# ZhaoyangLyu/Point_Diffusion_Refinement

Hardware: AMD Instinct MI355X
Metric: DDPM reverse steps/sec (T=1000, N=2048) (higher is better)
Workload: dtype f32; 1 GPU; BASELINE configs[1]: B=32/GPU, N=2048, 3072-pt mirrored condition, T=1000 DDPM reverse sampling, random-init dual-path PointNet++ (9.76 M params), cached condition step; global_batch=32, parallelism=dp1, launch=hipGraph replay, noise=device Philox, execution=fused channel-last HIP

## Files before the change

### include/pdr_hip.h

```cpp
#ifndef PDR_HIP_H
#define PDR_HIP_H

#include <stddef.h>
#include <stdint.h>

#ifdef __cplusplus
extern "C" {
#endif

#define PDR_OK 0
#define PDR_EINVAL (-1)
#define PDR_EUNSUPPORTED (-2)
#define PDR_ELAUNCH (-3)

typedef void *pdr_stream_t;

int pdr_version(void);
const char *pdr_last_error(void);
int pdr_set_option(const char *name, int value);
int pdr_get_option(const char *name, int *value);
const char *pdr_option_name(int index);

int pdr_opt_n_threads(int work_size);

// ... 142 lines not shown
int pdr_knn_build(const float *feats_y, int C, const float *x, const float *y,
                  const long long *idx, const float *d2, int B, int n1, int n2, int K,
                  float *out, int ldo, pdr_stream_t stream);
int pdr_attention_pool(const float *scores, int lds, const float *values, int ldv,
                       const float *vscale, const float *vshift, int v_relu, const int *counts,
                       int B, int npoint, int K, int D, float *out, pdr_stream_t stream);
int pdr_gather_add(const float *U, int ldu, int n_src, const float *V, const float *V0, int ldv,
                   const int *idx, const int *counts, const float *s1, const float *r1,
                   const float *s2, const float *r2, int B, int rows_per_batch, int K, int Cout,
                   float *Y, int ldy, float *partial, int relu_col0, int ycol0, int ycols,
                   pdr_stream_t stream);

int pdr_dedup_plan(const int *idx, const int *counts, int B, int m, int K, int *idx0, float *row_w,
                   unsigned char *tile_valid, int *tile_list, int *n_tiles, pdr_stream_t stream);
int pdr_dedup_prepare(const int *idx, const int *counts, const float *xyz, int B, int m, int K, int *perm, int *inv,
                      int *perm_rows, int *idx_s, int *counts_s, float *xyz_s, int *idx0, float *row_w,
                      unsigned char *tile_valid, int *tile_list, int *n_tiles, int *nvalid, int *probe_acc,
                      pdr_stream_t stream);
int pdr_dedup_probe(const int *counts, int B, int m, int K, int *probe_acc, pdr_stream_t stream);
int pdr_dedup_sort(const int *counts, int B, int m, int *perm, int *inv, int *perm_rows, pdr_stream_t stream);
int pdr_gather_add_tiles(const float *U, int ldu, int n_src, const float *V, const float *V0, int ldv,
                         const int *idx, const int *counts, const float *s1, const float *r1,
                         const float *s2, const float *r2, int B, int rows_per_batch, int K, int Cout,
                         float *Y, int ldy, float *partial, int relu_col0, int ycol0, int ycols,
                         const unsigned char *tile_valid, int partial_tpb, pdr_stream_t stream);
int pdr_gather_add_tiles_twin(const float *U, int ldu, int n_src, const float *V, const float *V0, int ldv,
                              const int *idx, const int *counts, int B, int rows_per_batch, int K, int Cout, float *Y,
                              int ldy, float *partial, int relu_col0, int ycol0, int ycols,
                              const unsigned char *tile_valid, int partial_tpb, const int *idx0, float *Yd, int ldyd,
                              const int *wrow0, float wmul, pdr_stream_t stream);
int pdr_weighted_moments(const float *Y, int ldy, int B, int rpb, int C, int relu_col0, const float *row_w,
                         float *partial, int ptpb, int tpb_full, const unsigned char *tile_valid,
                         pdr_stream_t stream);
int pdr_patch_rows(const float *V, int ldv, const float *vscale, const float *vshift, int v_relu,
                   const float *row_w, int B, int rpb, int D, float *out, int ldo, const int *out_rows,
                   pdr_stream_t stream);
int pdr_gather_rows(const float *src, const int *idx, int B, int n, int C, int m, float *out,
                    pdr_stream_t stream);


int pdr_reverse_update(float *x, const float *eps, int ld_eps, const float *z, const float *tab_a,
                       const float *tab_b, const float *tab_c, const long long *t_dev, long npoints,
                       int mode, pdr_stream_t stream);
int pdr_reverse_step(float *x, const float *eps, int ld_eps, const float *z, const float *tab_a,
                     const float *tab_b, const float *tab_c, long long *t_dev, const float *ts_table,
                     float *ts_out, unsigned long long *rng_state, int *ticket, long npoints, int mode,
                     int *probe_acc, int *probe_out, pdr_stream_t stream);
int pdr_embed_select(const float *table, int ldt, int T, const long long *t_dev, int B, int W, float *out, int ldo,
                     pdr_stream_t stream);
int pdr_embed_linear(const float *x, int ldx, const float *ts, int ts_stride, const float *freq, int half,
                     const float *W, const float *bias, int B, int K, int N, int act, float *out, int ldo,
                     pdr_stream_t stream);
typedef struct {
  const float *ptr;
  int C, ld;
} pdr_chain_seg_t;
typedef struct {
  const float *Wt;
  const float *bias;
  int ldw, Cin, Cout, main_cols;
  const float *gamma;
  const float *beta;
  int groups, Cn;
  float eps;
  int relu_pre, relu_post;
  const float *add;
  int add_ld;
  int reserved_;
} pdr_chain_layer_t;
typedef struct {
  int n_layers, n_seg;
  pdr_chain_seg_t seg[3];
  pdr_chain_layer_t layer[4];
  int residual, ldo;
  float *out;
  float *scratch;
  int *sync;
} pdr_point_chain_t;
int pdr_point_chain_plan(const pdr_point_chain_t *chain, int B, int n, long *out);
int pdr_point_chain(const pdr_point_chain_t *chain, int B, int n, pdr_stream_t stream);
int pdr_gather_rows2(const float *src0, int C0, const float *src1, int C1, const int *idx, int B, int n, int m,
                     float *out, pdr_stream_t stream);
int pdr_pad_rows(const float *src, long rows, int C, float *out, int ldo, pdr_stream_t stream);
int pdr_mark_time(unsigned long long *slot, pdr_stream_t stream);

#ifdef __cplusplus
}
#endif
#endif
```

### point_diffusion_refinement_amd/_lib.py

```python
import ctypes
import os

_HERE = os.path.dirname(os.path.abspath(__file__))
LIB_PATH = os.path.join(_HERE, "libpdr_hip.so")

PDR_OK, PDR_EINVAL, PDR_EUNSUPPORTED, PDR_ELAUNCH = 0, -1, -2, -3
_ERR = {PDR_EINVAL: "invalid argument", PDR_EUNSUPPORTED: "unsupported size", PDR_ELAUNCH: "kernel launch failed"}

_c = ctypes
_P, _I, _F, _Z = _c.c_void_p, _c.c_int, _c.c_float, _c.c_size_t

SIGNATURES = {
    "pdr_version": (_I, []),
    "pdr_last_error": (_c.c_char_p, []),
    "pdr_set_option": (_I, [_c.c_char_p, _I]),
    "pdr_get_option": (_I, [_c.c_char_p, _P]),
    "pdr_option_name": (_c.c_char_p, [_I]),
    "pdr_opt_n_threads": (_I, [_I]),
    "pdr_fps_workspace_bytes": (_Z, [_I, _I]),
    "pdr_furthest_point_sampling": (_I, [_P, _I, _I, _I, _P, _P, _P]),
    "pdr_gather_points": (_I, [_P, _P, _I, _I, _I, _I, _P, _P]),
    "pdr_gather_points_grad": (_I, [_P, _P, _I, _I, _I, _I, _P, _P]),
    "pdr_ball_query": (_I, [_P, _P, _I, _I, _I, _F, _I, _P, _P, _P]),
    "pdr_group_points": (_I, [_P, _P, _I, _I, _I, _I, _I, _P, _P]),
    "pdr_group_points_grad": (_I, [_P, _P, _I, _I, _I, _I, _I, _P, _P]),
    "pdr_three_nn": (_I, [_P, _P, _I, _I, _I, _P, _P, _P]),
    "pdr_three_interpolate": (_I, [_P, _P, _P, _I, _I, _I, _I, _P, _P]),
    "pdr_three_interpolate_grad": (_I, [_P, _P, _P, _I, _I, _I, _I, _P, _P]),
    "pdr_knn_points": (_I, [_P, _P, _I, _I, _I, _I, _P, _P, _P, _P]),
    "pdr_knn_points_ragged": (_I, [_P, _P, _P, _P, _I, _I, _I, _I, _P, _P, _P, _P]),
    "pdr_chamfer_nn": (_I, [_P, _P, _I, _I, _I, _P, _P, _P, _P, _P]),
    "pdr_chamfer_nn_ragged": (_I, [_P, _P, _P, _P, _I, _I, _I, _P, _P, _P, _P, _P]),
    "pdr_knn_group": (_I, [_P, _P, _I, _I, _I, _I, _P, _P, _P, _P]),
    "pdr_knn_points_grad": (_I, [_P, _P, _P, _P, _I, _I, _I, _I, _P, _P, _P]),
    "pdr_emd_workspace_bytes": (_Z, [_I, _I, _I]),
    "pdr_matchcost_workspace_bytes": (_Z, [_I, _I, _I]),
    "pdr_approxmatch": (_I, [_P, _P, _I, _I, _I, _P, _P, _P]),
    "pdr_matchcost": (_I, [_P, _P, _P, _I, _I, _I, _P, _P, _P]),
    "pdr_matchcost_grad": (_I, [_P, _P, _P, _P, _I, _I, _I, _P, _P, _P]),
    "pdr_emd_cost": (_I, [_P, _P, _I, _I, _I, _P, _P, _P]),
    "pdr_fused_layer_tile_rows": (_I, [_I, _I]),
    "pdr_fused_layer_variant": (_I, [_I, _I]),
    "pdr_fused_layer_plan": (_I, [_P, _c.c_long, _I, _P, _I, _I, _P, _I, _P]),
    "pdr_fused_layer": (_I, [_P, _c.c_long, _I, _P, _I, _P, _I, _P, _I, _P, _I, _P]),
    "pdr_fused_layer_pair": (_I, [_P, _c.c_long, _P, _c.c_long, _I, _P, _I, _P, _I, _P, _I, _P, _I, _P, _P, _I, _P]),
    "pdr_fused_layer_f16x3": (_I, [_P, _c.c_long, _I, _P, _I, _P, _I, _P, _I, _P, _I, _P]),
    "pdr_fused_layer_pool": (_I, [_P, _c.c_long, _I, _P, _I, _P, _I, _P, _I, _P, _P, _I, _P, _I, _P, _I, _P]),
    "pdr_fused_layer_pool_f16x3": (_I, [_P, _c.c_long, _I, _P, _I, _P, _I, _P, _I, _P, _P, _I, _P, _I, _P, _I, _P]),
    "pdr_gn_reduce": (_I, [_P, _I, _I, _I, _I, _c.c_double, _P, _I, _I, _P]),
    "pdr_apply_act": (_I, [_P, _c.c_long, _I, _P, _I, _P]),
    "pdr_act_colmax": (_I, [_P, _c.c_long, _I, _P, _P]),
    "pdr_gn_fold": (_I, [_P, _I, _I, _I, _c.c_double, _P, _I, _I, _I, _c.c_double, _I, _I, _I, _c.c_double, _F,
                         _P, _P, _P, _P, _P, _I, _P, _I, _P]),
    "pdr_gn_finalize": (_I, [_P, _I, _I, _I, _I, _c.c_double, _F, _P, _P, _P, _P, _P]),
    "pdr_group_build": (_I, [_P, _I, _P, _P, _P, _P, _I, _I, _I, _I, _I, _I, _I, _P, _I, _P]),
    "pdr_knn_build": (_I, [_P, _I, _P, _P, _P, _P, _I, _I, _I, _I, _P, _I, _P]),
    "pdr_attention_pool": (_I, [_P, _I, _P, _I, _P, _P, _I, _P, _I, _I, _I, _I, _P, _P]),
    "pdr_gather_rows": (_I, [_P, _P, _I, _I, _I, _I, _P, _P]),
    "pdr_reverse_update": (_I, [_P, _P, _I, _P, _P, _P, _P, _P, _c.c_long, _I, _P]),
    "pdr_reverse_step": (_I, [_P, _P, _I, _P, _P, _P, _P, _P, _P, _P, _P, _P, _c.c_long, _I, _P, _P, _P]),
    "pdr_embed_select": (_I, [_P, _I, _I, _P, _I, _I, _P, _I, _P]),
    "pdr_dedup_prepare": (_I, [_P, _P, _P, _I, _I, _I, _P, _P, _P, _P, _P, _P, _P, _P, _P, _P, _P, _P, _P, _P]),
    "pdr_dedup_probe": (_I, [_P, _I, _I, _I, _P, _P]),
    "pdr_gather_add_tiles_twin": (_I, [_P, _I, _I, _P, _P, _I, _P, _P, _I, _I, _I, _I, _P, _I, _P, _I, _I, _I, _P, _I,
                                       _P, _P, _I, _P, _F, _P]),
    "pdr_gather_rows2": (_I, [_P, _I, _P, _I, _P, _I, _I, _I, _P, _P]),
    "pdr_pad_rows": (_I, [_P, _c.c_long, _I, _P, _I, _P]),
    "pdr_mark_time": (_I, [_P, _P]),
    "pdr_embed_linear": (_I, [_P, _I, _P, _I, _P, _I, _P, _P, _I, _I, _I, _I, _P, _I, _P]),
    "pdr_gather_add": (_I, [_P, _I, _I, _P, _P, _I, _P, _P, _P, _P, _P, _P, _I, _I, _I, _I, _P, _I, _P, _I, _I, _I, _P]),
    "pdr_gather_add_tiles": (_I, [_P, _I, _I, _P, _P, _I, _P, _P, _P, _P, _P, _P, _I, _I, _I, _I, _P, _I, _P, _I, _I, _I,
                                  _P, _I, _P]),
    "pdr_dedup_plan": (_I, [_P, _P, _I, _I, _I, _P, _P, _P, _P, _P, _P]),
    "pdr_dedup_sort": (_I, [_P, _I, _I, _P, _P, _P, _P]),
    "pdr_weighted_moments": (_I, [_P, _I, _I, _I, _I, _I, _P, _P, _I, _I, _P, _P]),
    "pdr_patch_rows": (_I, [_P, _I, _P, _P, _I, _P, _I, _I, _I, _P, _I, _P, _P]),
    "pdr_point_chain_plan": (_I, [_P, _I, _I, _P]),
    "pdr_point_chain": (_I, [_P, _I, _I, _P]),
}


class Seg(_c.Structure):
    _fields_ = [("ptr", _P), ("C", _I), ("ld", _I), ("row_div", _I), ("gV", _P), ("gV0", _P), ("g_ldv", _I),
                ("g_nsrc", _I), ("g_zrow", _I), ("g_reserved", _I), ("g_r1", _P), ("g_r2", _P)]


class LayerIn(_c.Structure):
    _fields_ = [("n_seg", _I), ("seg", Seg * 4), ("scale", _P), ("shift", _P), ("add", _P), ("rseg", Seg),
                ("add_ld", _I), ("pre_relu", _I), ("post_relu", _I), ("rows_per_batch", _I), ("gidx", _P),
                ("gcnt", _P), ("gK", _I), ("ss_ld", _I), ("oadd", _P), ("oadd_ld", _I), ("oadd_div", _I), ("oadd_rows", _P),
                ("gs1", _P), ("gs2", _P), ("tile_list", _P), ("n_tiles", _P), ("out_rows", _P), ("partial_tpb", _I),
                ("wmul", _F), ("wrow0", _P), ("patch_values", _P), ("patch_w", _P), ("patch_ld", _I),
                ("walk_reverse", _I)]
class ChainSeg(_c.Structure):
    _fields_ = [("ptr", _P), ("C", _I), ("ld", _I)]


class ChainLayer(_c.Structure):
    _fields_ = [("Wt", _P), ("bias", _P), ("ldw", _I), ("Cin", _I), ("Cout", _I), ("main_cols", _I), ("gamma", _P),
                ("beta", _P), ("groups", _I), ("Cn", _I), ("eps", _F), ("relu_pre", _I), ("relu_post", _I), ("add", _P),
                ("add_ld", _I), ("reserved_", _I)]


class PointChain(_c.Structure):
    _fields_ = [("n_layers", _I), ("n_seg", _I), ("seg", ChainSeg * 3), ("layer", ChainLayer * 4), ("residual", _I),
                ("ldo", _I), ("out", _P), ("scratch", _P), ("sync", _P)]


_lib = None
ABI_VERSION = 200


def load():
    global _lib
    if _lib is None:
        if not os.path.exists(LIB_PATH):
            raise ImportError(
                "point_diffusion_refinement_amd: %s not found. Build it with "
                "`python -c 'import __graft_entry__ as g; g.build()'` or `make -C %s/csrc`. "
                "There is no CPU fallback." % (LIB_PATH, _HERE))
        lib = ctypes.CDLL(LIB_PATH)
        for name, (res, args) in SIGNATURES.items():
            fn = getattr(lib, name)
            fn.restype, fn.argtypes = res, args
        if lib.pdr_version() != ABI_VERSION:
            raise ImportError("point_diffusion_refinement_amd: %s is ABI %d, this binding needs %d -- rebuild it "
                              "(`make -C %s/csrc`)" % (LIB_PATH, lib.pdr_version(), ABI_VERSION, _HERE))
        _lib = lib
        _apply_env_options()
    return _lib


def set_option(name, value):
    check(load().pdr_set_option(name.encode(), int(value)), "set_option(%s=%r)" % (name, value))


def get_option(name):
    v = _c.c_int(0)
    check(load().pdr_get_option(name.encode(), _c.byref(v)), "get_option(%s)" % name)
    return v.value


def option_names():
    lib, out, i = load(), [], 0
    while True:
        n = lib.pdr_option_name(i)
        if n is None:
            return out
        out.append(n.decode())
        i += 1


def _apply_env_options():
    for item in filter(None, (t.strip() for t in os.environ.get("PDR_OPTIONS", "").split(","))):
        name, _, val = item.partition("=")
        set_option(name.strip(), int(val))
    for name in option_names():
        val = os.environ.get("PDR_" + name.upper())
        if val is not None and val.strip().lstrip("-").isdigit():
            set_option(name, int(val))


def check(rc, what):
    if rc != PDR_OK:
        detail = ""
        if rc == PDR_ELAUNCH:
            detail = ": " + (load().pdr_last_error() or b"").decode()
        raise RuntimeError("%s failed: %s%s" % (what, _ERR.get(rc, "code %d" % rc), detail))
```

### point_diffusion_refinement_amd/csrc/ball_query.hip

```cpp
#include "pdr_common.h"

namespace {

template <int NCH, bool RESIDENT>
__global__ __launch_bounds__(256) void ball_query_kernel(
    const float* __restrict__ new_xyz, const float* __restrict__ xyz, int n, int m,
    float radius2, int nsample, int qpw, int* __restrict__ idx,
    int* __restrict__ counts) {
  const int b = blockIdx.y;
  const int lane = threadIdx.x & 63;
  const int wave = __builtin_amdgcn_readfirstlane(threadIdx.x >> 6);
  const float* p = xyz + static_cast<size_t>(b) * n * 3;
  const float* q = new_xyz + static_cast<size_t>(b) * m * 3;
  int* oi = idx + static_cast<size_t>(b) * m * nsample;
  int* oc = counts + static_cast<size_t>(b) * m;

  const int nch = RESIDENT ? NCH : (n + 63) / 64;
  float px[NCH], py[NCH], pz[NCH];
  if constexpr (RESIDENT) {
    if constexpr (NCH <= 32) {
#pragma unroll
      for (int c = 0; c < NCH; ++c) {
        const int k = min(c * 64 + lane, n - 1);
        px[c] = p[k * 3 + 0];
        py[c] = p[k * 3 + 1];
        pz[c] = p[k * 3 + 2];
      }
#pragma unroll
      for (int c = 0; c < NCH; ++c) {
        const bool ok = c * 64 + lane < n;
        px[c] = ok ? px[c] : __builtin_inff();
        py[c] = ok ? py[c] : __builtin_inff();
        pz[c] = ok ? pz[c] : __builtin_inff();
      }
    } else {
#pragma unroll
      for (int c = 0; c < NCH; ++c) {
        const int k = c * 64 + lane;
        const bool ok = k < n;
        px[c] = ok ? p[k * 3 + 0] : __builtin_inff();
        py[c] = ok ? p[k * 3 + 1] : __builtin_inff();
        pz[c] = ok ? p[k * 3 + 2] : __builtin_inff();
      }
    }
    __builtin_amdgcn_s_waitcnt(0x0F70);
  }

  const int j0 = (blockIdx.x * 4 + wave) * qpw;
  const int jf = min(j0, m - 1);
  float nqx = q[jf * 3 + 0], nqy = q[jf * 3 + 1], nqz = q[jf * 3 + 2];
  for (int jj = 0; jj < qpw; ++jj) {
    const int j = j0 + jj;
    if (j >= m) break;
    const float qx = nqx, qy = nqy, qz = nqz;
    {
      const int jn = min(j + 1, m - 1);
      nqx = q[jn * 3 + 0], nqy = q[jn * 3 + 1], nqz = q[jn * 3 + 2];
    }
    int* row = oi + static_cast<size_t>(j) * nsample;
    int cnt = 0;
    int first = 0;
    auto scan = [&](int c, float x, float y, float z) {
      const float dx = qx - x, dy = qy - y, dz = qz - z;
      const float d2 = PDR_SUM3(dx, dy, dz);
      const bool hit = d2 < radius2;
      const unsigned long long mask = __ballot(hit);
      if (mask != 0ull) {
        if (cnt == 0) first = c * 64 + __builtin_ctzll(mask);
        const int pos = cnt + __builtin_amdgcn_mbcnt_hi(
                                  static_cast<unsigned>(mask >> 32),
                                  __builtin_amdgcn_mbcnt_lo(static_cast<unsigned>(mask), 0u));
        if (hit && pos < nsample) row[pos] = c * 64 + lane;
        cnt += __builtin_popcountll(mask);
      }
    };
    if constexpr (RESIDENT) {
#pragma unroll
      for (int c = 0; c < NCH; ++c) {
        if (cnt < nsample) scan(c, px[c], py[c], pz[c]);
      }
    } else {
      for (int c = 0; c < nch && cnt < nsample; ++c) {
        const int k = c * 64 + lane;
        const bool ok = k < n;
        const int kc = ok ? k : n - 1;
        const float x = p[kc * 3 + 0], y = p[kc * 3 + 1], z = p[kc * 3 + 2];
        scan(c, ok ? x : __builtin_inff(), ok ? y : __builtin_inff(), ok ? z : __builtin_inff());
      }
    }
    const int filled = cnt < nsample ? cnt : nsample;
    for (int l = filled + lane; l < nsample; l += 64) row[l] = first;
    if (lane == 0) oc[j] = filled;
  }
}

template <int NCH, bool RESIDENT>
int launch(const float* new_xyz, const float* xyz, int B, int n, int m, float radius2,
           int nsample, int* idx, int* counts, hipStream_t s) {
  int qpw = 16;
  while (qpw > 1 && static_cast<long long>(B) * ((m + 4 * qpw - 1) / (4 * qpw)) < 1024) qpw >>= 1;
  dim3 grid((m + 4 * qpw - 1) / (4 * qpw), B);
  hipLaunchKernelGGL((ball_query_kernel<NCH, RESIDENT>), grid, dim3(256), 0, s, new_xyz, xyz, n,
                     m, radius2, nsample, qpw, idx, counts);
  return pdr::check_launch();
}

}

extern "C" int pdr_ball_query(const float* new_xyz, const float* xyz, int B, int n, int m,
                              float radius, int nsample, int* idx, int* counts,
                              pdr_stream_t stream) {
  if (B < 0 || n <= 0 || m < 0 || nsample <= 0) return PDR_EINVAL;
  if (B == 0 || m == 0) return PDR_OK;
  if (!new_xyz || !xyz || !idx || !counts) return PDR_EINVAL;
  hipStream_t s = pdr::as_stream(stream);
  const float radius2 = radius * radius;
#define PDR_BQ_CASE(NCH) \
  if (n <= 64 * (NCH))   \
  return launch<NCH, true>(new_xyz, xyz, B, n, m, radius2, nsample, idx, counts, s)
  PDR_BQ_CASE(1);
  PDR_BQ_CASE(2);
  PDR_BQ_CASE(4);
  PDR_BQ_CASE(8);
  PDR_BQ_CASE(16);
  PDR_BQ_CASE(32);
  PDR_BQ_CASE(48);
  PDR_BQ_CASE(64);
#undef PDR_BQ_CASE
  return launch<1, false>(new_xyz, xyz, B, n, m, radius2, nsample, idx, counts, s);
}
```

### point_diffusion_refinement_amd/csrc/dedup.hip

```cpp
#include "pdr_common.h"

__global__ __launch_bounds__(256) void dedup_flags_kernel(const int* __restrict__ idx, const int* __restrict__ counts,
                                                          int K, long nq, int qpt, int* __restrict__ idx0,
                                                          float* __restrict__ row_w,
                                                          unsigned char* __restrict__ tile_valid) {
  const long q = static_cast<long>(blockIdx.x) * 256 + threadIdx.x;
  if (q >= nq) return;
  const int cnt = counts[q];
  idx0[q] = idx[q * K];
  int v = cnt > 1 ? 1 : 0;
  for (int off = 1; off < qpt; off <<= 1) v |= __shfl_xor(v, off, 64);
  const bool valid = v != 0;
  row_w[q] = valid ? 0.0f : static_cast<float>(K);
  if ((q & (qpt - 1)) == 0) tile_valid[q / qpt] = valid ? 1 : 0;
}

__global__ __launch_bounds__(1024) void dedup_compact_kernel(const unsigned char* __restrict__ tile_valid, int ntiles,
                                                            int* __restrict__ tile_list, int* __restrict__ n_tiles) {
  __shared__ int wtot[16];
  __shared__ int base_s;
  const int tid = threadIdx.x, lane = tid & 63, wave = tid >> 6;
  if (tid == 0) base_s = 0;
  __syncthreads();
  for (int i0 = 0; i0 < ntiles; i0 += 1024) {
// ... 2 lines not shown
    const unsigned long long bal = __ballot(valid);
    const int before = __builtin_popcountll(bal & ((1ull << lane) - 1ull));
    if (lane == 0) wtot[wave] = __builtin_popcountll(bal);
    __syncthreads();
    int woff = 0, tot = 0;
    for (int w = 0; w < 16; ++w) {
      woff += w < wave ? wtot[w] : 0;
      tot += wtot[w];
    }
    const int base = base_s;
    if (valid) tile_list[base + woff + before] = i;
    __syncthreads();
    if (tid == 0) base_s = base + tot;
    __syncthreads();
  }
  if (tid == 0) *n_tiles = base_s;
}

__global__ __launch_bounds__(1024) void dedup_sort_kernel(const int* __restrict__ counts, int m,
                                                         int* __restrict__ perm, int* __restrict__ inv,
                                                         int* __restrict__ perm_rows) {
  __shared__ int wtot[16];
  __shared__ int base_s;
  const int tid = threadIdx.x, lane = tid & 63, wave = tid >> 6;
  const int* cb = counts + static_cast<long>(blockIdx.x) * m;
  int* pb = perm + static_cast<long>(blockIdx.x) * m;
  int* ib = inv + static_cast<long>(blockIdx.x) * m;
  if (tid == 0) base_s = 0;
  __syncthreads();
  for (int pass = 0; pass < 2; ++pass) {
    for (int i0 = 0; i0 < m; i0 += 1024) {
      const int i = i0 + tid;
      const bool take = i < m && ((cb[i] > 1) == (pass == 0));
      const unsigned long long bal = __ballot(take);
      const int before = __builtin_popcountll(bal & ((1ull << lane) - 1ull));
      if (lane == 0) wtot[wave] = __builtin_popcountll(bal);
      __syncthreads();
      int woff = 0, tot = 0;
      for (int w = 0; w < 16; ++w) {
        woff += w < wave ? wtot[w] : 0;
        tot += wtot[w];
      }
      const int base = base_s;
      if (take) {
        const int j = base + woff + before;
        pb[j] = i;
        ib[i] = j;
        if (perm_rows) perm_rows[static_cast<long>(blockIdx.x) * m + j] = static_cast<int>(blockIdx.x) * m + i;
      }
      __syncthreads();
      if (tid == 0) base_s = base + tot;
      __syncthreads();
    }
  }
}

extern "C" int pdr_dedup_sort(const int* counts, int B, int m, int* perm, int* inv, int* perm_rows,
                              pdr_stream_t stream) {
  if (!counts || !perm || !inv || B < 0 || m <= 0 || static_cast<long>(B) * m >= (1L << 31)) return PDR_EINVAL;
  if (B == 0) return PDR_OK;
  hipLaunchKernelGGL(dedup_sort_kernel, dim3(B), dim3(1024), 0, pdr::as_stream(stream), counts, m, perm, inv, perm_rows);
  return pdr::check_launch();
}

extern "C" int pdr_dedup_plan(const int* idx, const int* counts, int B, int m, int K, int* idx0, float* row_w,
                              unsigned char* tile_valid, int* tile_list, int* n_tiles, pdr_stream_t stream) {
  if (!idx || !counts || !idx0 || !row_w || !tile_valid || !tile_list || !n_tiles || B < 0 || m <= 0) return PDR_EINVAL;
  if (!(K == 8 || K == 16 || K == 32) || (static_cast<long>(m) * K) % 128 != 0) return PDR_EINVAL;
  if (B == 0) return PDR_OK;
  const int qpt = 128 / K;
  const long ntiles = static_cast<long>(B) * m / qpt;
  if (ntiles >= (1L << 30)) return PDR_EINVAL;
  const long nq = static_cast<long>(B) * m;
  hipLaunchKernelGGL(dedup_flags_kernel, dim3(pdr::blocks_for(nq)), dim3(256), 0, pdr::as_stream(stream), idx, counts, K,
                     nq, qpt, idx0, row_w, tile_valid);
  hipLaunchKernelGGL(dedup_compact_kernel, dim3(1), dim3(1024), 0, pdr::as_stream(stream), tile_valid,
                     static_cast<int>(ntiles), tile_list, n_tiles);
  return pdr::check_launch();
}

constexpr int kMaxPrepareClouds = 1024;
constexpr int kMaxPrepareQueries = 4096;

__global__ __launch_bounds__(1024) void dedup_prepare_kernel(
    const int* __restrict__ idx, const int* __restrict__ counts, const float* __restrict__ xyz, int m, int K, int nB,
    int* __restrict__ perm, int* __restrict__ inv, int* __restrict__ perm_rows, int* __restrict__ idx_s,
    int* __restrict__ counts_s, float* __restrict__ xyz_s, int* __restrict__ idx0, float* __restrict__ row_w,
    unsigned char* __restrict__ tile_valid, int* __restrict__ tile_list, int* __restrict__ n_tiles,
    int* __restrict__ nvalid, int* __restrict__ probe_acc) {
  __shared__ int nreal_s[kMaxPrepareClouds];
  __shared__ int perm_s[kMaxPrepareQueries];
  __shared__ int wtot[16];
  __shared__ int base_s, prefix_s;
  const int tid = threadIdx.x, lane = tid & 63, wave = tid >> 6;
  const int b = blockIdx.x;
  const int qpt = 128 / K, tpb = m / qpt;
  if (tid == 0) base_s = 0;
  const bool vec = (m & 3) == 0 && (reinterpret_cast<uintptr_t>(counts) & 15) == 0;
  for (int bb = wave; bb <= b; bb += 16) {
    const int* cb = counts + static_cast<long>(bb) * m;
    int c = 0;
    if (vec) {
      const int4* c4 = reinterpret_cast<const int4*>(cb);
      const int n4 = m >> 2;
      for (int i0 = 0; i0 < n4; i0 += 64 * 8) {
        int4 v[8];
#pragma unroll
        for (int u = 0; u < 8; ++u) {
          const int i = i0 + 64 * u + lane;
          v[u] = c4[i < n4 ? i : 0];
        }
#pragma unroll
        for (int u = 0; u < 8; ++u) {
          const bool ok = i0 + 64 * u + lane < n4;
          c += ok ? (v[u].x > 1) + (v[u].y > 1) + (v[u].z > 1) + (v[u].w > 1) : 0;
        }
      }
    } else {
      for (int i = lane; i < m; i += 64) c += cb[i] > 1 ? 1 : 0;
    }
#pragma unroll
    for (int off = 32; off >= 1; off >>= 1) c += __shfl_xor(c, off, 64);
    if (lane == 0) nreal_s[bb] = c;
  }
  __syncthreads();
  if (tid == 0) {
    int p = 0;
    for (int bb = 0; bb < b; ++bb) p += (nreal_s[bb] + qpt - 1) / qpt;
    prefix_s = p;
  }
  const int nv = (nreal_s[b] + qpt - 1) / qpt;
  const int q0 = nv * qpt;
  const int* cb = counts + static_cast<long>(b) * m;
  int* pb = perm + static_cast<long>(b) * m;
  int* ib = inv + static_cast<long>(b) * m;
  for (int pass = 0; pass < 2; ++pass) {
    for (int i0 = 0; i0 < m; i0 += 1024) {
      const int i = i0 + tid;
      const bool take = i < m && ((cb[i] > 1) == (pass == 0));
      const unsigned long long bal = __ballot(take);
      const int before = __builtin_popcountll(bal & ((1ull << lane) - 1ull));
      if (lane == 0) wtot[wave] = __builtin_popcountll(bal);
      __syncthreads();
      int woff = 0, tot = 0;
      for (int w = 0; w < 16; ++w) {
        woff += w < wave ? wtot[w] : 0;
        tot += wtot[w];
      }
      const int base = base_s;
      if (take) {
        const int j = base + woff + before;
        perm_s[j] = i;
        pb[j] = i;
        ib[i] = j;
        if (perm_rows) perm_rows[static_cast<long>(b) * m + j] = b * m + i;
      }
      __syncthreads();
      if (tid == 0) base_s = base + tot;
      __syncthreads();
    }
  }
  for (int j = tid; j < m; j += 1024) {
    const int src = perm_s[j];
    const long qs = static_cast<long>(b) * m + src, qd = static_cast<long>(b) * m + j;
    counts_s[qd] = cb[src];
    idx0[qd] = idx[qs * K];
    row_w[qd] = j >= q0 ? static_cast<float>(K) : 0.0f;
    if (xyz) {
      const float x = xyz[qs * 3 + 0], y = xyz[qs * 3 + 1], z = xyz[qs * 3 + 2];
      xyz_s[qd * 3 + 0] = x;
      xyz_s[qd * 3 + 1] = y;
      xyz_s[qd * 3 + 2] = z;
    }
  }
  const int k4 = K / 4, ksh4 = __builtin_ctz(k4);
  const int npiece = m * k4;
  const int4* src4 = reinterpret_cast<const int4*>(idx + static_cast<long>(b) * m * K);
  int4* dst4 = reinterpret_cast<int4*>(idx_s + static_cast<long>(b) * m * K);
  for (int e0 = 0; e0 < npiece; e0 += 4096) {
    int4 v[4];
#pragma unroll
    for (int u = 0; u < 4; ++u) {
      const int e = min(e0 + 1024 * u + tid, npiece - 1);
      v[u] = src4[(perm_s[e >> ksh4] << ksh4) + (e & (k4 - 1))];
    }
#pragma unroll
    for (int u = 0; u < 4; ++u) {
      const int e = e0 + 1024 * u + tid;
      if (e < npiece) dst4[e] = v[u];
    }
  }
  const int prefix = prefix_s;
  for (int t = tid; t < tpb; t += 1024) {
    tile_valid[static_cast<long>(b) * tpb + t] = t < nv ? 1 : 0;
    if (t < nv) tile_list[prefix + t] = b * tpb + t;
  }
  if (tid == 0) {
    nvalid[b] = nv;
    nvalid[nB + b] = q0;
    if (b == nB - 1) *n_tiles = prefix + nv;
    if (probe_acc) {
      atomicAdd(&probe_acc[0], nv);
      atomicAdd(&probe_acc[1], tpb);
    }
  }
}

__global__ __launch_bounds__(256) void dedup_probe_kernel(const int* __restrict__ counts, int m, int K,
                                                          int* __restrict__ probe_acc) {
  __shared__ int tot;
  if (threadIdx.x == 0) tot = 0;
  __syncthreads();
  const int* cb = counts + static_cast<long>(blockIdx.x) * m;
  int c = 0;
  for (int i = threadIdx.x; i < m; i += 256) c += cb[i] > 1 ? 1 : 0;
#pragma unroll
  for (int off = 32; off >= 1; off >>= 1) c += __shfl_xor(c, off, 64);
  if ((threadIdx.x & 63) == 0 && c) atomicAdd(&tot, c);
  __syncthreads();
  if (threadIdx.x == 0) {
    const int qpt = 128 / K;
    atomicAdd(&probe_acc[0], (tot + qpt - 1) / qpt);
    atomicAdd(&probe_acc[1], m / qpt);
  }
}

extern "C" int pdr_dedup_prepare(const int* idx, const int* counts, const float* xyz, int B, int m, int K, int* perm,
                                 int* inv, int* perm_rows, int* idx_s, int* counts_s, float* xyz_s, int* idx0,
                                 float* row_w, unsigned char* tile_valid, int* tile_list, int* n_tiles, int* nvalid,
                                 int* probe_acc, pdr_stream_t stream) {
  if (!idx || !counts || !perm || !inv || !idx_s || !counts_s || (xyz && !xyz_s) || !idx0 || !row_w || !tile_valid ||
      !tile_list || !n_tiles || !nvalid || B < 0 || m <= 0)
    return PDR_EINVAL;
  if (!(K == 8 || K == 16 || K == 32) || (static_cast<long>(m) * K) % 128 != 0) return PDR_EINVAL;
  if (static_cast<long>(B) * m * K >= (1L << 31)) return PDR_EINVAL;
  if (B > kMaxPrepareClouds || m > kMaxPrepareQueries) return PDR_EUNSUPPORTED;
  if ((reinterpret_cast<uintptr_t>(idx) | reinterpret_cast<uintptr_t>(idx_s)) % 16 != 0) return PDR_EINVAL;
  if (B == 0) return PDR_OK;
  hipLaunchKernelGGL(dedup_prepare_kernel, dim3(B), dim3(1024), 0, pdr::as_stream(stream), idx, counts, xyz, m, K, B,
                     perm, inv, perm_rows, idx_s, counts_s, xyz_s, idx0, row_w, tile_valid, tile_list, n_tiles, nvalid,
                     probe_acc);
  return pdr::check_launch();
}

extern "C" int pdr_dedup_probe(const int* counts, int B, int m, int K, int* probe_acc, pdr_stream_t stream) {
  if (!counts || !probe_acc || B < 0 || m <= 0) return PDR_EINVAL;
  if (!(K == 8 || K == 16 || K == 32) || (static_cast<long>(m) * K) % 128 != 0) return PDR_EINVAL;
  if (B == 0) return PDR_OK;
  hipLaunchKernelGGL(dedup_probe_kernel, dim3(B), dim3(256), 0, pdr::as_stream(stream), counts, m, K, probe_acc);
  return pdr::check_launch();
}

__global__ __launch_bounds__(256) void weighted_moments_kernel(const float* __restrict__ Y, int ldy, int C, int rpb,
                                                               int tpbd, int nB, int relu_col0,
                                                               const float* __restrict__ row_w,
                                                               float* __restrict__ partial, int ptpb, int tpb_full,
                                                               const unsigned char* __restrict__ tile_valid) {
  const int nmom = nB * tpbd;
  const int cl = threadIdx.x & 63, sl = threadIdx.x >> 6;
  const int c = blockIdx.y * 64 + cl;
  if (static_cast<int>(blockIdx.x) >= nmom) {
    const int t0 = (static_cast<int>(blockIdx.x) - nmom) * 16;
    for (int k = sl; k < 16; k += 4) {
      const int t = t0 + k;
      if (t < nB * tpb_full && !tile_valid[t] && c < C) {
        const int b = t / tpb_full, tb = t - b * tpb_full;
        float* o = partial + ((static_cast<long>(b) * ptpb + tb) * C + c) * 2;
        o[0] = 0.0f;
        o[1] = 0.0f;
      }
    }
    return;
  }
  __shared__ float red[4][64][2];
  const int b = blockIdx.x / tpbd, j = blockIdx.x - b * tpbd;
  const int r0 = j * 128 + sl * 32, r1 = min(r0 + 32, rpb);
  float s1 = 0.0f, s2 = 0.0f;
  if (c < C) {
    const float lo = c >= relu_col0 ? 0.0f : -__builtin_inff();
    const float* yp = Y + (static_cast<long>(b) * rpb) * ldy + c;
    const float* wp = row_w + static_cast<long>(b) * rpb;
    float w[32];
    bool any = false;
#pragma unroll
    for (int k = 0; k < 32; ++k) {
      w[k] = r0 + k < r1 ? wp[min(r0 + k, rpb - 1)] : 0.0f;
      any = any || w[k] > 0.0f;
    }
    if (any) {
#pragma unroll
      for (int k0 = 0; k0 < 32; k0 += 16) {
        float y[16];
#pragma unroll
        for (int k = 0; k < 16; ++k) y[k] = yp[static_cast<long>(min(r0 + k0 + k, rpb - 1)) * ldy];
#pragma unroll
        for (int k = 0; k < 16; ++k) {
          const float f = fmaxf(y[k], lo);
          s1 = __builtin_fmaf(w[k0 + k], f, s1);
          s2 = __builtin_fmaf(w[k0 + k] * f, f, s2);
        }
      }
    }
  }
  red[sl][cl][0] = s1;
  red[sl][cl][1] = s2;
  __syncthreads();
  if (sl == 0 && c < C) {
    float* o = partial + ((static_cast<long>(b) * ptpb + tpb_full + j) * C + c) * 2;
    o[0] = (red[0][cl][0] + red[1][cl][0]) + (red[2][cl][0] + red[3][cl][0]);
    o[1] = (red[0][cl][1] + red[1][cl][1]) + (red[2][cl][1] + red[3][cl][1]);
  }
}

extern "C" int pdr_weighted_moments(const float* Y, int ldy, int B, int rpb, int C, int relu_col0, const float* row_w,
                                    float* partial, int ptpb, int tpb_full, const unsigned char* tile_valid,
                                    pdr_stream_t stream) {
  if (!Y || !row_w || !partial || !tile_valid || B < 0 || rpb <= 0 || C <= 0 || ldy < C || tpb_full <= 0) return PDR_EINVAL;
  const int tpbd = (rpb + 127) / 128;
  if (ptpb < tpb_full + tpbd) return PDR_EINVAL;
  if (B == 0) return PDR_OK;
  const long nz = (static_cast<long>(B) * tpb_full + 15) / 16;
  const dim3 grid(static_cast<unsigned>(static_cast<long>(B) * tpbd + nz), static_cast<unsigned>((C + 63) / 64));
  hipLaunchKernelGGL(weighted_moments_kernel, grid, dim3(256), 0, pdr::as_stream(stream), Y, ldy, C, rpb, tpbd, B,
                     relu_col0, row_w, partial, ptpb, tpb_full, tile_valid);
// ... 34 lines not shown
```

### point_diffusion_refinement_amd/csrc/fused_gather.hip

```cpp
#include "pdr_common.h"

namespace {

template <int LPP>
__global__ __launch_bounds__(256) void group_build_kernel(
    const float* __restrict__ feats, int Cs, int n, const float* __restrict__ xyz,
    const float* __restrict__ new_xyz, const int* __restrict__ idx, const int* __restrict__ counts,
    int m, int K, int patch_empty, int with_abs, int with_centre, long npos, int Cout, int ldo,
    float* __restrict__ out) {
  constexpr int GPB = 256 / LPP;
  const int lane = threadIdx.x % LPP;
  const long g0 = static_cast<long>(blockIdx.x) * GPB + threadIdx.x / LPP;
  const long ngroups = static_cast<long>(gridDim.x) * GPB;
  for (long p = g0; p < npos; p += ngroups) {
    const long bj = p / K;
    const int b = static_cast<int>(bj / m);
    const int a = idx[p];
    const bool empty = patch_empty && counts[bj] <= 0;
    const float* frow = feats + (static_cast<long>(b) * n + a) * Cs;
    float* orow = out + p * ldo;
    for (int c = lane; c < Cs; c += LPP) orow[c] = empty ? 0.0f : frow[c];
    if (lane < ldo - Cout) orow[Cout + lane] = 0.0f;
    if (lane < Cout - Cs) {
      const int g = lane;
// ... 113 lines not shown
    int cnt = K;
    if (counts) {
      cnt = counts[row];
      cnt = cnt < 1 ? 1 : cnt;
    }
    const float4* s4 = reinterpret_cast<const float4*>(scores + row * K * D) + lane;
    const float4* v4 = reinterpret_cast<const float4*>(values + row * K * D) + lane;
    float4 sv[NL], vv[NL];
#pragma unroll
    for (int i = 0; i < NL; ++i) {
      const bool ok = k0 + i * kstep < K;
      sv[i] = ok ? s4[i * 64] : make_float4(0, 0, 0, 0);
      vv[i] = ok ? v4[i * 64] : make_float4(0, 0, 0, 0);
    }
    float4 sc = make_float4(1, 1, 1, 1), shv = make_float4(0, 0, 0, 0);
    if (vscale) sc = *reinterpret_cast<const float4*>(vscale + static_cast<long>(b) * D + 4 * c4);
    if (vshift) shv = *reinterpret_cast<const float4*>(vshift + static_cast<long>(b) * D + 4 * c4);
    float m[4] = {-__builtin_inff(), -__builtin_inff(), -__builtin_inff(), -__builtin_inff()};
    float se[NL][4];
#pragma unroll
    for (int i = 0; i < NL; ++i) {
      const int k = k0 + i * kstep;
      const float e[4] = {sv[i].x, sv[i].y, sv[i].z, sv[i].w};
#pragma unroll
      for (int j = 0; j < 4; ++j) {
        se[i][j] = k >= K ? -__builtin_inff() : (k >= cnt ? -1e9f : e[j]) * 1.44269504088896340736f;
        m[j] = fmaxf(m[j], se[i][j]);
      }
    }
#pragma unroll
    for (int j = 0; j < 4; ++j)
      for (int off = D4; off < 64; off <<= 1) m[j] = fmaxf(m[j], __shfl_xor(m[j], off, 64));
    float l[4] = {0, 0, 0, 0}, acc[4] = {0, 0, 0, 0};
    const float sce[4] = {sc.x, sc.y, sc.z, sc.w}, she[4] = {shv.x, shv.y, shv.z, shv.w};
#pragma unroll
    for (int i = 0; i < NL; ++i) {
      const float ve[4] = {vv[i].x, vv[i].y, vv[i].z, vv[i].w};
#pragma unroll
      for (int j = 0; j < 4; ++j) {
        const float w = __builtin_amdgcn_exp2f(se[i][j] - m[j]);
        const float val = fmaxf(__builtin_fmaf(ve[j], sce[j], she[j]), lo);
        l[j] += w;
        acc[j] = __builtin_fmaf(val, w, acc[j]);
      }
    }
#pragma unroll
    for (int j = 0; j < 4; ++j)
      for (int off = D4; off < 64; off <<= 1) {
        l[j] += __shfl_xor(l[j], off, 64);
        acc[j] += __shfl_xor(acc[j], off, 64);
      }
    if (lane < D4)
      *reinterpret_cast<float4*>(out + row * D + 4 * c4) =
          make_float4(acc[0] / l[0], acc[1] / l[1], acc[2] / l[2], acc[3] / l[3]);
  }
}

__global__ __launch_bounds__(256) void gather_rows_cl_kernel(const float* __restrict__ src, int n,
                                                             int C, const int* __restrict__ idx,
                                                             int m, long total,
                                                             float* __restrict__ out) {
  const long e = static_cast<long>(blockIdx.x) * 256 + threadIdx.x;
  if (e >= total) return;
  const long bj = e / C;
  const int c = static_cast<int>(e - bj * C);
  const int b = static_cast<int>(bj / m);
  out[e] = src[(static_cast<long>(b) * n + idx[bj]) * C + c];
}

__global__ __launch_bounds__(256) void gather_rows2_cl_kernel(const float* __restrict__ src0, int C0,
                                                              const float* __restrict__ src1, int C1, int n,
                                                              const int* __restrict__ idx, int m, long total,
                                                              float* __restrict__ out) {
  const long e = static_cast<long>(blockIdx.x) * 256 + threadIdx.x;
  if (e >= total) return;
  const int C = C0 + C1;
  const long bj = e / C;
  const int c = static_cast<int>(e - bj * C);
  const int b = static_cast<int>(bj / m);
  const long row = static_cast<long>(b) * n + idx[bj];
  out[e] = c < C0 ? src0[row * C0 + c] : src1[row * C1 + (c - C0)];
}

__global__ __launch_bounds__(256) void pad_rows_kernel(const float* __restrict__ src, int C, int ldo, long total,
                                                       float* __restrict__ out) {
  const long e = static_cast<long>(blockIdx.x) * 256 + threadIdx.x;
  if (e >= total) return;
  const long r = e / ldo;
  const int c = static_cast<int>(e - r * ldo);
  out[e] = c < C ? src[r * C + c] : 0.0f;
}

}

extern "C" int pdr_group_build(const float* feats, int Cs, const float* xyz, const float* new_xyz,
                               const int* idx, const int* counts, int B, int n, int m, int K,
                               int patch_empty, int with_abs, int with_centre, float* out, int ldo,
                               pdr_stream_t stream) {
  if (B < 0 || n <= 0 || m < 0 || K <= 0 || Cs < 0) return PDR_EINVAL;
  if (B == 0 || m == 0) return PDR_OK;
  if (!xyz || !new_xyz || !idx || !out || (Cs > 0 && !feats) || (patch_empty && !counts))
    return PDR_EINVAL;
  const int Cout = Cs + 3 + (with_abs ? 3 : 0) + (with_centre ? 3 : 0);
  if (ldo < Cout || ldo - Cout > 8) return PDR_EINVAL;
  const long npos = static_cast<long>(B) * m * K;
  hipStream_t s = pdr::as_stream(stream);
#define PDR_GB(LPP)                                                                                 \
  do {                                                                                              \
    const long nblk = (npos + 256 / LPP - 1) / (256 / LPP);                                         \
    hipLaunchKernelGGL(group_build_kernel<LPP>, dim3(static_cast<unsigned>(nblk < 32768 ? nblk : 32768)), \
                       dim3(256), 0, s, feats, Cs, n, xyz, new_xyz, idx, counts, m, K, patch_empty, \
                       with_abs, with_centre, npos, Cout, ldo, out);                                \
  } while (0)
  if (Cout <= 16) PDR_GB(16);
  else if (Cout <= 48) PDR_GB(32);
  else PDR_GB(64);
#undef PDR_GB
  return pdr::check_launch();
}

extern "C" int pdr_knn_build(const float* feats_y, int C, const float* x, const float* y,
                             const long long* idx, const float* d2, int B, int n1, int n2, int K,
                             float* out, int ldo, pdr_stream_t stream) {
  if (B < 0 || n1 < 0 || n2 <= 0 || K <= 0 || C < 0) return PDR_EINVAL;
  if (B == 0 || n1 == 0) return PDR_OK;
  if (!x || !y || !idx || !d2 || !out || (C > 0 && !feats_y)) return PDR_EINVAL;
  const int Cout = C + 11;
  if (ldo < Cout || ldo - Cout > 8) return PDR_EINVAL;
  const long npos = static_cast<long>(B) * n1 * K;
  hipStream_t s = pdr::as_stream(stream);
#define PDR_KB(LPP)                                                                                 \
  do {                                                                                              \
    const long nblk = (npos + 256 / LPP - 1) / (256 / LPP);                                         \
    hipLaunchKernelGGL(knn_build_kernel<LPP>, dim3(static_cast<unsigned>(nblk < 32768 ? nblk : 32768)), \
                       dim3(256), 0, s, feats_y, C, n2, x, y, idx, d2, n1, K, npos, Cout, ldo, out); \
  } while (0)
  if (Cout <= 16) PDR_KB(16);
  else if (Cout <= 48) PDR_KB(32);
  else PDR_KB(64);
#undef PDR_KB
  return pdr::check_launch();
}

extern "C" int pdr_attention_pool(const float* scores, int lds, const float* values, int ldv,
                                  const float* vscale, const float* vshift, int v_relu,
                                  const int* counts, int B, int npoint, int K, int D, float* out,
                                  pdr_stream_t stream) {
  if (B < 0 || npoint < 0 || K <= 0 || D <= 0) return PDR_EINVAL;
  if (B == 0 || npoint == 0) return PDR_OK;
  if (!scores || !values || !out) return PDR_EINVAL;
  const long rows = static_cast<long>(B) * npoint;
  if (D % 4 || lds % 4 || ldv % 4) return PDR_EUNSUPPORTED;
  {
    const int D4 = D / 4;
    const long per_query = static_cast<long>(K) * D4;
    const int kstep = D4 <= 64 ? 64 / (D4 ? D4 : 1) : 0;
    if (lds == D && ldv == D && D4 <= 64 && (D4 & (D4 - 1)) == 0 && per_query <= 512 && kstep > 0) {
      const int nl = static_cast<int>((K + kstep - 1) / kstep);
      long blocks = (rows + 3) / 4;
      if (blocks > 256L * 16) blocks = 256L * 16;
      const dim3 grid(static_cast<unsigned>(blocks));
      hipStream_t st = pdr::as_stream(stream);
#define PDR_AP(NL)                                                                                      \
  hipLaunchKernelGGL(attention_pool_wave_kernel<NL>, grid, dim3(256), 0, st, scores, values, vscale,    \
                     vshift, v_relu, counts, K, D, npoint, rows, out)
      if (nl <= 1) PDR_AP(1);
      else if (nl <= 2) PDR_AP(2);
      else if (nl <= 4) PDR_AP(4);
      else PDR_AP(8);
#undef PDR_AP
      return pdr::check_launch();
    }
  }
  hipLaunchKernelGGL(attention_pool_kernel, dim3(pdr::blocks_for(rows * (D / 4))), dim3(256), 0,
                     pdr::as_stream(stream), scores, lds, values, ldv, vscale, vshift, v_relu, counts, K,
                     D, npoint, rows, out);
  return pdr::check_launch();
}

extern "C" int pdr_gather_rows2(const float* src0, int C0, const float* src1, int C1, const int* idx, int B, int n,
                                int m, float* out, pdr_stream_t stream) {
  if (B < 0 || n <= 0 || C0 <= 0 || C1 <= 0 || m < 0) return PDR_EINVAL;
  if (B == 0 || m == 0) return PDR_OK;
  if (!src0 || !src1 || !idx || !out) return PDR_EINVAL;
  const long total = static_cast<long>(B) * m * (C0 + C1);
  hipLaunchKernelGGL(gather_rows2_cl_kernel, dim3(pdr::blocks_for(total)), dim3(256), 0, pdr::as_stream(stream), src0,
                     C0, src1, C1, n, idx, m, total, out);
  return pdr::check_launch();
}

extern "C" int pdr_pad_rows(const float* src, long rows, int C, float* out, int ldo, pdr_stream_t stream) {
  if (rows < 0 || C <= 0 || ldo < C) return PDR_EINVAL;
  if (rows == 0) return PDR_OK;
  if (!src || !out) return PDR_EINVAL;
  const long total = rows * ldo;
  hipLaunchKernelGGL(pad_rows_kernel, dim3(pdr::blocks_for(total)), dim3(256), 0, pdr::as_stream(stream), src, C, ldo,
                     total, out);
  return pdr::check_launch();
}

extern "C" int pdr_gather_rows(const float* src, const int* idx, int B, int n, int C, int m,
                               float* out, pdr_stream_t stream) {
  if (B < 0 || n <= 0 || C <= 0 || m < 0) return PDR_EINVAL;
  if (B == 0 || m == 0) return PDR_OK;
  if (!src || !idx || !out) return PDR_EINVAL;
  const long total = static_cast<long>(B) * m * C;
  hipLaunchKernelGGL(gather_rows_cl_kernel, dim3(pdr::blocks_for(total)), dim3(256), 0,
                     pdr::as_stream(stream), src, n, C, idx, m, total, out);
  return pdr::check_launch();
}

template <int LPR, bool KPOW2, bool HAS_S>
__global__ __launch_bounds__(256) void gather_add_kernel(
    const float* __restrict__ U, int ldu, int n_src, const float* __restrict__ V,
    const float* __restrict__ V0, int ldv, const int* __restrict__ idx, const int* __restrict__ counts,
    const float* __restrict__ s1, const float* __restrict__ r1, const float* __restrict__ s2,
    const float* __restrict__ r2, int rows_per_batch_, int K_, int Cout, float* __restrict__ Y_, int ldy_,
    float* __restrict__ partial, int relu_col0, int ycol0_, int ycol1_,
    const unsigned char* __restrict__ tile_valid, int partial_tpb, pdr::GatherTwin tw) {
  constexpr int TM = 128;
  const bool twin = static_cast<int>(blockIdx.x) >= tw.n_main && tw.n_main > 0;
  const int rows_per_batch = twin ? rows_per_batch_ / K_ : rows_per_batch_;
  const int K = twin ? 1 : K_;
  const int* __restrict__ idx_e = twin ? tw.idx0 : idx;
  float* __restrict__ Y = twin ? tw.Y : Y_;
  const int ldy = twin ? tw.ldy : ldy_;
  const int ycol0 = twin ? 0 : ycol0_, ycol1 = twin ? ((Cout + 3) & ~3) : ycol1_;
  constexpr int RPI = 64 / LPR;
  constexpr int DEPTH = 32 / RPI < 4 ? 32 / RPI : 4;
  constexpr int CW = 4 * LPR;
  __shared__ float red[4][CW][2];
  const int lane = threadIdx.x & 63, wave = threadIdx.x >> 6;
  const int sub = lane / LPR, cl = lane % LPR;
  const int tpb = (rows_per_batch + TM - 1) / TM;
  const int n_main = tw.n_main > 0 ? tw.n_main : static_cast<int>(gridDim.x);
  const int bid = twin ? static_cast<int>(blockIdx.x) - n_main : pdr::xcd_contiguous(blockIdx.x, n_main);
  const int b = bid / tpb, tb = bid - b * tpb;
  if (!twin && tile_valid && !tile_valid[bid]) return;
  const int tpb_main = (rows_per_batch_ + TM - 1) / TM;
  const long prow = static_cast<long>(b) * (partial_tpb > 0 ? partial_tpb : tpb) + (twin ? tpb_main : 0) + tb;
  const long row0 = static_cast<long>(b) * rows_per_batch + static_cast<long>(tb) * TM;
  const int nvalid = min(TM, rows_per_batch - tb * TM);
  const int wlo = twin ? min(max(tw.wrow0[b] - tb * TM, 0), TM) : 0;
  const float wmul = twin ? tw.wmul : 1.0f;
  const float* Ub = U + static_cast<long>(b) * n_src * ldu;
  const int wr0 = wave * 32;
  const int myr = min(wr0 + (lane & 31), nvalid - 1);
  const long myp = row0 + myr;
  const int my_idx = idx_e[myp];
  const int my_empty = (counts && counts[myp / K] <= 0) ? 1 : 0;
  const float my_s1 = s1 ? s1[myp] : 0.0f;
  const float my_s2 = s2 ? s2[myp] : 0.0f;
  const int nrows = max(0, min(32, nvalid - wr0));

  constexpr bool has_s = HAS_S;
  const bool has_em = counts != nullptr;
  const int ksh = KPOW2 ? __builtin_ctz(K) : -1;
  const long qbase = (row0 + wr0) / K;
  const float* Vq = V + qbase * ldv;
  const long v0d = has_em ? V0 - V : 0;
  for (int c0 = static_cast<int>(blockIdx.y) * CW; c0 < Cout; c0 += CW * static_cast<int>(gridDim.y)) {
    const int c = c0 + 4 * cl;
    const bool cok = c < Cout;
    const int cc = cok ? c : 0;
    float4 q1 = make_float4(0, 0, 0, 0), q2 = make_float4(0, 0, 0, 0);
    if (cok && r1) q1 = *reinterpret_cast<const float4*>(r1 + c);
    if (cok && r2) q2 = *reinterpret_cast<const float4*>(r2 + c);
    float lo[4];
#pragma unroll
    for (int j = 0; j < 4; ++j) lo[j] = (c + j >= relu_col0) ? 0.0f : -__builtin_inff();
    const bool ywin = Y && c >= ycol0 && c < ycol1;
    float a1[4] = {0, 0, 0, 0}, a2[4] = {0, 0, 0, 0};
    for (int r = 0; r < nrows; r += DEPTH * RPI) {
      float4 u[DEPTH], v[DEPTH];
      float t1[DEPTH], t2[DEPTH];
      int em[DEPTH], rr[DEPTH];
#pragma unroll
      for (int k = 0; k < DEPTH; ++k) {
        rr[k] = r + k * RPI + sub;
        const int rc = min(rr[k], nrows - 1);
// ... 162 lines not shown
```

### point_diffusion_refinement_amd/csrc/fused_layer.hip

```cpp
#include "layer_tiles.h"

#include <cstdlib>

namespace {

typedef float f32x16 __attribute__((ext_vector_type(16)));

using pdr::PoolArgs;

template <int RT, int CT, int WR, int WC, int KC, bool RADD, bool VEC, bool GATH, bool POOL = false, int KS = 1>
__global__ __launch_bounds__(256, 2) void fused_layer_kernel(
    pdr_layer_in_t in, int Cin, const float* __restrict__ Wt, int ldw,
    const float* __restrict__ bias, int Cout, float* __restrict__ Y, int ldy,
    float* __restrict__ partial, int relu_col0, int n_row_tiles, PoolArgs pool = PoolArgs()) {
  static_assert(WR * WC * KS == 4, "4 waves per workgroup");
  static_assert(KS == 1 || !POOL, "pooled epilogue: no K split");
  constexpr int TM = WR * RT * 32, TN = WC * CT * 32;
  constexpr int APT = TM * KC / 256;
  constexpr int RSTEP = 256 / KC;
  constexpr int C4 = KC / 4;
  constexpr int VSTEP = 256 / C4;
  constexpr int APT4 = TM / VSTEP;
  constexpr int TN4 = TN / 4;
  constexpr int WPT4 = (KC * TN4 + 255) / 256;
// ... 339 lines not shown
      const int col = n0 + cl;
      const bool colok = col < Cout;
      const float bv = bias_r[j];
      const bool relu_stat = col >= relu_col0;
      float s1 = 0.0f, s2 = 0.0f;
      float* ybase = Y + row0 * ldy + col;
      if (colok && in.oadd) {
        const int osh = __builtin_ctz(in.oadd_div);
        const float* ob = in.oadd + col;
#pragma unroll
        for (int i = 0; i < RT; ++i) {
#pragma unroll
          for (int r = 0; r < 16; ++r) {
            const int rl = min((wr * RT + i) * 32 + (r & 3) + 8 * (r >> 2) + 4 * hi, nvalid - 1);
            const long oq = (row0 + rl) >> osh;
            acc[i][j][r] += ob[(in.oadd_rows ? static_cast<long>(in.oadd_rows[oq]) : oq) * in.oadd_ld];
          }
        }
      }
      if (colok) {
        if (rows_full) {
#pragma unroll
          for (int i = 0; i < RT; ++i) {
#pragma unroll
            for (int r = 0; r < 16; ++r) {
              const int rl = (wr * RT + i) * 32 + (r & 3) + 8 * (r >> 2) + 4 * hi;
              const float y = acc[i][j][r] + bv;
              ybase[rl * ldy] = y;
              const float f = relu_stat ? fmaxf(y, 0.0f) : y;
              s1 += f;
              s2 = __builtin_fmaf(f, f, s2);
            }
          }
        } else {
#pragma unroll
          for (int i = 0; i < RT; ++i) {
#pragma unroll
            for (int r = 0; r < 16; ++r) {
              const int rl = (wr * RT + i) * 32 + (r & 3) + 8 * (r >> 2) + 4 * hi;
              const float y = acc[i][j][r] + bv;
              if (rl < nvalid) {
                ybase[rl * ldy] = y;
                if (rl >= wlo) {
                  const float f = relu_stat ? fmaxf(y, 0.0f) : y;
                  s1 += f;
                  s2 = __builtin_fmaf(f, f, s2);
                }
              }
            }
          }
        }
      }
      if (partial) {
        s1 += __shfl_xor(s1, 32, 64);
        s2 += __shfl_xor(s2, 32, 64);
        if (in.wrow0) {
          s1 *= in.wmul;
          s2 *= in.wmul;
        }
        if (hi == 0) {
          red[wr][cl][0] = s1;
          red[wr][cl][1] = s2;
        }
      }
    }
    if (partial) {
      __syncthreads();
      if (tid < TN && n0 + tid < Cout) {
        float s1 = 0.0f, s2 = 0.0f;
#pragma unroll
        for (int w = 0; w < WR; ++w) {
          s1 += red[w][tid][0];
          s2 += red[w][tid][1];
        }
        const long prow = static_cast<long>(b) * (in.partial_tpb > 0 ? in.partial_tpb : tpb) + tb;
        float* o = partial + (prow * Cout + n0 + tid) * 2;
        o[0] = s1;
        o[1] = s2;
      }
    }
  }
}

__global__ __launch_bounds__(256) void fused_layer_thin_kernel(const float* __restrict__ X, int ldx, int shift,
                                                               int Cin, const float* __restrict__ Wt, int ldw,
                                                               const float* __restrict__ bias, int Cout,
                                                               float* __restrict__ Y, int ldy, long P, int qshift) {
  constexpr int kThinIters = 8;
  const int ql = 1 << qshift;
  const int cq = threadIdx.x & (ql - 1), rl = threadIdx.x >> qshift;
  const int c0 = 4 * (static_cast<int>(blockIdx.y) * ql + cq);
  if (c0 >= Cout) return;
  const int rpp = 256 >> qshift;
  float4 w[4];
  float b4[4];
#pragma unroll
  for (int k = 0; k < 4; ++k)
    w[k] = k < Cin ? *reinterpret_cast<const float4*>(Wt + static_cast<long>(k) * ldw + c0) : make_float4(0, 0, 0, 0);
#pragma unroll
  for (int j = 0; j < 4; ++j) b4[j] = (bias && c0 + j < Cout) ? bias[c0 + j] : 0.0f;
  const long r0 = static_cast<long>(blockIdx.x) * (rpp * kThinIters) + rl;
  float4 xr[kThinIters];
#pragma unroll
  for (int it = 0; it < kThinIters; ++it) {
    const long row = r0 + static_cast<long>(it) * rpp;
    xr[it] = *reinterpret_cast<const float4*>(X + ((row < P ? row : P - 1) >> shift) * ldx);
  }
#pragma unroll
  for (int it = 0; it < kThinIters; ++it) {
    const long row = r0 + static_cast<long>(it) * rpp;
    if (row < P) {
      const float4 x = xr[it];
      const float xs[4] = {x.x, x.y, x.z, x.w};
      float acc[4] = {b4[0], b4[1], b4[2], b4[3]};
#pragma unroll
      for (int o = 0; o < 4; ++o) {
        const int k = ((o & 1) << 1) | (o >> 1);
        if (k < Cin) {
          acc[0] = __builtin_fmaf(xs[k], w[k].x, acc[0]);
          acc[1] = __builtin_fmaf(xs[k], w[k].y, acc[1]);
          acc[2] = __builtin_fmaf(xs[k], w[k].z, acc[2]);
          acc[3] = __builtin_fmaf(xs[k], w[k].w, acc[3]);
        }
      }
      *reinterpret_cast<float4*>(Y + row * ldy + c0) = make_float4(acc[0], acc[1], acc[2], acc[3]);
    }
  }
}

using pdr::LayerSource;
using pdr::Tile;

inline bool narrow_kc32() { return pdr::option(pdr::OPT_NARROW_KC32) != 0; }
inline int pick_tile(int rows_per_batch, int Cout) {
  if (narrow_kc32() && rows_per_batch >= 128 && Cout <= 32) return 7;
  if (narrow_kc32() && rows_per_batch >= 128 && Cout <= 64) return 8;
  if (rows_per_batch >= 256 && Cout <= 32) return 0;
  if (rows_per_batch >= 256 && Cout <= 64) return 1;
  if (rows_per_batch >= 128 && Cout <= 96) return 2;
  if (rows_per_batch >= 128 && Cout > 128 && Cout <= 160) return 3;
  if (rows_per_batch >= 128) return 4;
  if (rows_per_batch >= 64) return 5;
  return 6;
}
}

extern "C" int pdr_fused_layer_tile_rows(int rows_per_batch, int Cout) {
  if (rows_per_batch <= 0 || Cout <= 0) return 0;
  return pdr::tile_tm(pick_tile(rows_per_batch, Cout));
}

extern "C" int pdr_fused_layer_variant(int rows_per_batch, int Cout) {
  if (rows_per_batch <= 0 || Cout <= 0) return -1;
  return pick_tile(rows_per_batch, Cout);
}

namespace {
enum class Family {
  Thin,
  DeepSplitK,
  Deep,
  Ws,
  Uniform
};

struct LayerPlan {
  Family family;
  int id, tm;
  LayerSource src;
  bool vec;
  bool ws;
  bool thin;
  long ntiles;
  int ncol;
  int deep;
  int deep_tn;
};

bool deep_chunks() { return pdr::option(pdr::OPT_DEEP_CHUNKS) != 0; }

bool use_ws_kernels() { return pdr::option(pdr::OPT_FUSED_WS) != 0; }

int plan_layer(const pdr_layer_in_t* in, long P, int Cin, const float* Wt, int ldw, int Cout, const float* Y,
               int ldy, bool has_partial, LayerPlan* pl) {
  if (!in || !Wt || P < 0 || Cin <= 0 || Cout <= 0 || in->n_seg < 1 || in->n_seg > 4 || ldw < Cout ||
      (Y && ldy < Cout))
    return PDR_EINVAL;
  if (ldw % 4 != 0 || reinterpret_cast<uintptr_t>(Wt) % 16 != 0) return PDR_EINVAL;
  int ctot = 0;
  for (int s = 0; s < in->n_seg; ++s) {
    if (!in->seg[s].ptr || in->seg[s].C <= 0 || in->seg[s].row_div < 1) return PDR_EINVAL;
    if (in->seg[s].row_div & (in->seg[s].row_div - 1)) return PDR_EUNSUPPORTED;
    ctot += in->seg[s].C;
  }
  if (ctot != Cin || in->rows_per_batch <= 0 || P % in->rows_per_batch != 0) return PDR_EINVAL;
  if (in->oadd && (in->oadd_div < 1 || (in->oadd_div & (in->oadd_div - 1)) || in->oadd_ld < Cout))
    return PDR_EINVAL;
  if (in->ss_ld != 0 && in->ss_ld < Cin) return PDR_EINVAL;
  const int id = pick_tile(in->rows_per_batch, Cout), tm = pdr::tile_tm(id);
  for (int sg = 0; sg < in->n_seg; ++sg) {
    const int d = in->seg[sg].row_div;
    if (in->rows_per_batch % d != 0 || (in->rows_per_batch > tm && tm % d != 0)) return PDR_EUNSUPPORTED;
  }
  const long nb = P / in->rows_per_batch;
  if (in->partial_tpb > 0 && in->partial_tpb < (in->rows_per_batch + tm - 1) / tm) return PDR_EINVAL;
  pl->id = id;
  pl->tm = tm;
  pl->ntiles = nb * ((in->rows_per_batch + tm - 1) / tm);
  pl->ncol = (Cout + pdr::tile_tn(id) - 1) / pdr::tile_tn(id);
  const LayerSource src = pdr::layer_source(*in);
// ... 38 lines not shown
             !in->pre_relu && !in->post_relu && !in->oadd && Y && ldy % 4 == 0 &&
             reinterpret_cast<uintptr_t>(Y) % 16 == 0 && ldw >= ((Cout + 3) & ~3) && ldy >= ((Cout + 3) & ~3) &&
             P < (1L << 31);
  if (src.knn_marked && !pl->ws) return PDR_EUNSUPPORTED;
  if (in->tile_list && (!in->n_tiles || !pl->ws || tm != 128)) return PDR_EUNSUPPORTED;
  pl->family = pl->thin && !has_partial && !in->tile_list ? Family::Thin
               : split_k                                   ? Family::DeepSplitK
               : pl->deep                                  ? Family::Deep
               : pl->ws                                    ? Family::Ws
                                                           : Family::Uniform;
  return PDR_OK;
}

struct LayerArgs {
  hipStream_t s; const pdr_layer_in_t& in; int Cin; const float* Wt; int ldw; const float* bias; int Cout;
  float* Y; int ldy; float* partial; int relu_col0, n_row_tiles; PoolArgs pool;
};

template <class T, bool RADD, bool VEC, bool GATH, bool POOL = false, int KS = 1>
void launch_k(dim3 grid, const LayerArgs& a) {
  hipLaunchKernelGGL((fused_layer_kernel<T::RT, T::CT, T::WR, T::WC, T::KC, RADD, VEC, GATH, POOL, KS>), grid,
                     dim3(256), 0, a.s, a.in, a.Cin, a.Wt, a.ldw, a.bias, a.Cout, a.Y, a.ldy, a.partial, a.relu_col0,
                     a.n_row_tiles, a.pool);
}

template <class T>
void launch_form(dim3 grid, const LayerArgs& a, const LayerPlan& pl) {
  if (pl.src.radd) {
    if (pl.src.gath) launch_k<T, true, true, true>(grid, a);
    else if (pl.vec) launch_k<T, true, true, false>(grid, a);
    else launch_k<T, true, false, false>(grid, a);
  } else {
    if (pl.src.gath) launch_k<T, false, true, true>(grid, a);
    else if (pl.vec) launch_k<T, false, true, false>(grid, a);
    else launch_k<T, false, false, false>(grid, a);
  }
}

template <class T, int KS = 1>
void launch_plain(dim3 grid, const LayerArgs& a, bool radd) {
  if (radd) launch_k<T, true, true, false, false, KS>(grid, a);
  else launch_k<T, false, true, false, false, KS>(grid, a);
}

dim3 uniform_grid(long ntiles, int ncol) {
  const long cap = (256L * 6 + ncol - 1) / ncol;
  return dim3(static_cast<unsigned>(ntiles > cap ? cap : ntiles), static_cast<unsigned>(ncol));
}
}

extern "C" int pdr_fused_layer_plan(const pdr_layer_in_t* in, long P, int Cin, const float* Wt, int ldw, int Cout,
                                    const float* Y, int ldy, int* out) {
  if (!out) return PDR_EINVAL;
  LayerPlan pl;
  const int rc = plan_layer(in, P, Cin, Wt, ldw, Cout, Y, ldy, true, &pl);
  if (rc != PDR_OK) return rc;
  out[0] = pl.family == Family::Ws;
  out[1] = pl.id;
  out[2] = pl.src.radd;
  out[3] = pl.src.gath ? (pl.src.knn_marked ? 2 : 1) : 0;
  out[4] = pl.vec;
  out[5] = 0;
  out[6] = pl.thin;
  out[7] = pl.deep ? 128 : 0;
  return PDR_OK;
}

extern "C" int pdr_fused_layer(const pdr_layer_in_t* in, long P, int Cin, const float* Wt, int ldw,
                               const float* bias, int Cout, float* Y, int ldy, float* partial,
                               int relu_col0, pdr_stream_t stream) {
  if (!Y) return PDR_EINVAL;
  LayerPlan pl;
  const int prc = plan_layer(in, P, Cin, Wt, ldw, Cout, Y, ldy, partial != nullptr, &pl);
  if (prc != PDR_OK) return prc;
  if (P == 0) return PDR_OK;
  hipStream_t s = pdr::as_stream(stream);
  const int nt = static_cast<int>(pl.ntiles);
  const LayerArgs a{s, *in, Cin, Wt, ldw, bias, Cout, Y, ldy, partial, relu_col0, nt, PoolArgs()};
  auto deep_grid = [&] {
    return dim3(static_cast<unsigned>(pl.ntiles), static_cast<unsigned>((Cout + pl.deep_tn - 1) / pl.deep_tn));
  };
  switch (pl.family) {
    case Family::Thin: {
      const int c4n = (Cout + 3) / 4;
      int qshift = 3;
      while (qshift < 6 && (1 << qshift) < c4n) ++qshift;
      const int ql = 1 << qshift, rows_per_block = (256 >> qshift) * 8;
      const dim3 tgrid(static_cast<unsigned>((P + rows_per_block - 1) / rows_per_block),
                       static_cast<unsigned>((c4n + ql - 1) / ql));
      hipLaunchKernelGGL(fused_layer_thin_kernel, tgrid, dim3(256), 0, s, in->seg[0].ptr, in->seg[0].ld,
                         __builtin_ctz(in->seg[0].row_div), Cin, Wt, ldw, bias, Cout, Y, ldy, P, qshift);
      break;
    }
    case Family::DeepSplitK:
      if (pl.deep == 6) launch_plain<Tile<1, 1, 1, 1, 128>, 4>(deep_grid(), a, pl.src.radd);
      else launch_plain<Tile<1, 1, 2, 1, 128>, 2>(deep_grid(), a, pl.src.radd);
      break;
    case Family::Deep:
      if (pl.deep == 6) launch_form<Tile<1, 1, 1, 4, 128>>(uniform_grid(pl.ntiles, pl.ncol), a, pl);
      else if (pl.deep == 5) launch_plain<Tile<1, 1, 2, 2, 128>>(deep_grid(), a, pl.src.radd);
      else launch_plain<Tile<2, 1, 2, 2, 128>>(deep_grid(), a, pl.src.radd);
      break;
    case Family::Ws:
      pdr::launch_fused_layer_ws(pl.id, pl.src, *in, Cin, Wt, ldw, bias, Cout, Y, ldy, partial, relu_col0, nt, pl.ncol,
                                 s);
      break;
    case Family::Uniform:
      pdr::with_tile(pl.id, [&](auto t) { launch_form<decltype(t)>(uniform_grid(pl.ntiles, pl.ncol), a, pl); });
      break;
  }
  return pdr::check_launch();
}

extern "C" int pdr_fused_layer_pair(const pdr_layer_in_t* in, long P, const pdr_layer_in_t* in2, long P2, int Cin,
                                    const float* Wt, int ldw, const float* bias, int Cout, float* Y, int ldy,
                                    float* Y2, int ldy2, float* partial, float* partial2, int relu_col0,
                                    pdr_stream_t stream) {
  if (!Y || !Y2 || !in || !in2) return PDR_EINVAL;
  LayerPlan pl, pl2;
  int rc = plan_layer(in, P, Cin, Wt, ldw, Cout, Y, ldy, partial != nullptr, &pl);
  if (rc != PDR_OK) return rc;
  rc = plan_layer(in2, P2, Cin, Wt, ldw, Cout, Y2, ldy2, partial2 != nullptr, &pl2);
  if (rc != PDR_OK) return rc;
  if (P == 0 || P2 == 0) return PDR_EUNSUPPORTED;
  if ((partial == nullptr) != (partial2 == nullptr)) return PDR_EINVAL;
  if (!in->tile_list || !pl.ws || !pdr::tile_has_pair(pl.id) || !pl.vec || !pl2.vec || pl.src.radd || pl2.src.radd ||
      pl2.src.gath || pl.src.knn_marked || in2->tile_list)
    return PDR_EUNSUPPORTED;
  const int tpb2 = (in2->rows_per_batch + pl.tm - 1) / pl.tm;
  if (in2->partial_tpb > 0 && in2->partial_tpb < tpb2) return PDR_EINVAL;
  for (int sg = 0; sg < in2->n_seg; ++sg)
    if (in2->seg[sg].row_div != 1) return PDR_EUNSUPPORTED;
  if (in2->gidx || !pdr::fused_layer_ws_supported(pl.id, pl2.src, *in2, Cin)) return PDR_EUNSUPPORTED;
  pdr::WsTwin tw;
  tw.in[1] = *in2;
  tw.Y[1] = Y2;
  tw.partial[1] = partial2;
  tw.ldy[1] = ldy2;
  tw.n_row_tiles[1] = static_cast<int>((P2 / in2->rows_per_batch) * tpb2);
  tw.gx = 0;
  pdr::launch_fused_layer_ws_pair(pl.id, pl.src.gath, *in, Cin, Wt, ldw, bias, Cout, Y, ldy, partial, relu_col0,
                                  static_cast<int>(pl.ntiles), pl.ncol, tw, pdr::as_stream(stream));
  return pdr::check_launch();
}

extern "C" int pdr_fused_layer_f16x3(const pdr_layer_in_t* in, long P, int Cin, const void* Wp, int nchunks,
                                     const float* bias, int Cout, float* Y, int ldy, float* partial,
                                     int relu_col0, pdr_stream_t stream) {
  if (!Y || !Wp || nchunks <= 0 || reinterpret_cast<uintptr_t>(Wp) % 16 != 0) return PDR_EINVAL;
  LayerPlan pl;
  const int prc = plan_layer(in, P, Cin, reinterpret_cast<const float*>(Wp), (Cout + 3) & ~3, Cout, Y, ldy,
                             partial != nullptr, &pl);
  if (prc != PDR_OK) return prc;
  if (P == 0) return PDR_OK;
  if (!pl.ws || !pdr::tile_has_split(pl.id)) return PDR_EUNSUPPORTED;
  int nch = 0;
  for (int s = 0; s < in->n_seg; ++s) nch += (in->seg[s].C + 31) / 32;
  if (nch != nchunks) return PDR_EINVAL;
  pdr::launch_fused_layer_ws(pl.id, pl.src, *in, Cin, reinterpret_cast<const float*>(Wp), nchunks, bias, Cout, Y, ldy,
                             partial, relu_col0, static_cast<int>(pl.ntiles), pl.ncol, pdr::as_stream(stream), true);
  return pdr::check_launch();
}

namespace {
bool pool_patch_args_ok(const pdr_layer_in_t& in, int D, const float* out, int ldo) {
  if (!in.patch_values) return true;
  return in.patch_w != nullptr && in.patch_ld >= D && D % 4 == 0 && in.patch_ld % 4 == 0 && ldo % 4 == 0 &&
         reinterpret_cast<uintptr_t>(in.patch_values) % 16 == 0 && reinterpret_cast<uintptr_t>(out) % 16 == 0;
}

struct PoolPlan {
  int id, tm, ncol, nch;
  long ntiles;
  bool vec;
};
int plan_pool(const pdr_layer_in_t* in, long P, int Cin, bool weights_ok, int D, const float* values, int ldv, int K,
              const float* out, int ldo, PoolPlan* pp) {
  if (!in || !weights_ok || !values || !out || P <= 0 || Cin <= 0 || D <= 0 || in->n_seg < 1 || in->n_seg > 4 ||
      ldv < D || ldo < D)
    return PDR_EINVAL;
  if (!pool_patch_args_ok(*in, D, out, ldo)) return PDR_EINVAL;
  if (!(K == 8 || K == 16 || K == 32)) return PDR_EUNSUPPORTED;
  if (in->rseg.ptr || in->oadd) return PDR_EUNSUPPORTED;
  int ctot = 0;
  pp->nch = 0;
  pp->vec = true;
  for (int s = 0; s < in->n_seg; ++s) {
    const pdr_seg_t& g = in->seg[s];
    if (!g.ptr || g.C <= 0 || g.row_div != 1 || g.gV) return PDR_EUNSUPPORTED;
    pp->vec = pp->vec && reinterpret_cast<uintptr_t>(g.ptr) % 16 == 0 && g.ld % 4 == 0 && g.ld >= ((g.C + 3) & ~3);
    ctot += g.C;
    pp->nch += (g.C + 31) / 32;
  }
// ... 56 lines not shown
```

### point_diffusion_refinement_amd/csrc/neighbors.hip

```cpp
#include <cstdlib>

#include "pdr_common.h"

namespace {

constexpr int kTile = 1024;

enum DistModel { kSum3 = 0, kAcc3 = 1 };

__device__ __forceinline__ int cloud_len(const int64_t* __restrict__ len, int b, int n) {
  if (!len) return n;
  const int64_t v = len[b];
  return v < 0 ? 0 : (v > n ? n : static_cast<int>(v));
}

template <int K, int MODEL, typename IdxT, bool KNN_PAD, bool RAGGED = false>
__global__ __launch_bounds__(256) void nn_search_kernel(const float* __restrict__ queries,
                                                        const float* __restrict__ cloud, int nq,
                                                        int nc, int Kout,
                                                        float* __restrict__ dists,
                                                        IdxT* __restrict__ idx,
                                                        float* __restrict__ nn,
                                                        float* __restrict__ wgt = nullptr,
                                                        const int64_t* __restrict__ len_q = nullptr,
                                                        const int64_t* __restrict__ len_c = nullptr) {
  static_assert(KNN_PAD || !RAGGED, "the ragged search pads with (0, -1)");
  __shared__ float4 tile[kTile];
  const int b = blockIdx.y;
  const int j = blockIdx.x * 256 + threadIdx.x;
  const bool active = j < nq;
  const int nqe = RAGGED ? cloud_len(len_q, b, nq) : nq;
  const int nce = !RAGGED ? nc : (static_cast<int>(blockIdx.x) * 256 < nqe ? cloud_len(len_c, b, nc) : 0);
  const bool searching = RAGGED ? j < nqe : active;
  const float* q = queries + (static_cast<size_t>(b) * nq + (active ? j : 0)) * 3;
  const float* c = cloud + static_cast<size_t>(b) * nc * 3;
  const float qx = q[0], qy = q[1], qz = q[2];

  float bd[K];
  int bi[K];
#pragma unroll
  for (int t = 0; t < K; ++t) {
    bd[t] = __builtin_inff();
    bi[t] = KNN_PAD ? -1 : 0;
  }

  for (int k0 = 0; k0 < nce; k0 += kTile) {
    const int kn = (nce - k0) < kTile ? (nce - k0) : kTile;
    __syncthreads();
    for (int t = threadIdx.x; t < kn; t += 256) {
      const float* s = c + static_cast<size_t>(k0 + t) * 3;
      tile[t] = make_float4(s[0], s[1], s[2], 0.0f);
    }
    __syncthreads();
    if (searching) {
      for (int t = 0; t < kn; ++t) {
        const float4 pt = tile[t];
        const float dx = qx - pt.x, dy = qy - pt.y, dz = qz - pt.z;
        const float d = MODEL == kSum3 ? PDR_SUM3(dx, dy, dz) : PDR_ACC3(dx, dy, dz);
        if (d < bd[K - 1]) {
          const int k = k0 + t;
#pragma unroll
          for (int s = K - 1; s >= 1; --s) {
            const bool shift = bd[s - 1] > d;
            const bool here = bd[s] > d;
            bd[s] = shift ? bd[s - 1] : (here ? d : bd[s]);
            bi[s] = shift ? bi[s - 1] : (here ? k : bi[s]);
          }
          if (bd[0] > d) {
            bd[0] = d;
            bi[0] = k;
          }
        }
      }
    }
  }
  if (!active) return;
  float* od = dists + (static_cast<size_t>(b) * nq + j) * Kout;
  IdxT* oi = idx + (static_cast<size_t>(b) * nq + j) * Kout;
  if (wgt) {
    float* ow = wgt + (static_cast<size_t>(b) * nq + j) * Kout;
    float norm = 0.0f;
#pragma unroll
    for (int t = 0; t < K; ++t)
      if (t < Kout) norm += 1.0f / ((KNN_PAD && bi[t] < 0 ? 0.0f : bd[t]) + 1e-8f);
#pragma unroll
    for (int t = 0; t < K; ++t)
      if (t < Kout) ow[t] = (1.0f / ((KNN_PAD && bi[t] < 0 ? 0.0f : bd[t]) + 1e-8f)) / norm;
  }
#pragma unroll
  for (int t = 0; t < K; ++t) {
    if (t < Kout) {
      const bool empty = KNN_PAD && bi[t] < 0;
      od[t] = empty ? 0.0f : bd[t];
      oi[t] = static_cast<IdxT>(bi[t]);
      if (nn) {
        float* on = nn + ((static_cast<size_t>(b) * nq + j) * Kout + t) * 3;
        const int a = empty ? 0 : bi[t];
        on[0] = empty ? 0.0f : c[a * 3 + 0];
        on[1] = empty ? 0.0f : c[a * 3 + 1];
        on[2] = empty ? 0.0f : c[a * 3 + 2];
      }
    }
  }
}

template <int NCH, typename IdxT, bool RAGGED = false>
__global__ __launch_bounds__(256) void knn_wave_kernel(const float* __restrict__ queries,
                                                       const float* __restrict__ cloud, int nq, int nc, int K,
                                                       int qpw, float* __restrict__ dists, IdxT* __restrict__ idx,
                                                       float* __restrict__ nn, float* __restrict__ wgt,
                                                       const int64_t* __restrict__ len_q = nullptr,
                                                       const int64_t* __restrict__ len_c = nullptr) {
  __shared__ unsigned long long cand[4][64];
  __shared__ float outd[4][8];
  __shared__ int outi[4][8];
  __shared__ float outr[4][8];
  const int b = blockIdx.y;
  const int lane = threadIdx.x & 63;
  const int wave = __builtin_amdgcn_readfirstlane(threadIdx.x >> 6);
  const float* c = cloud + static_cast<size_t>(b) * nc * 3;
  const float* q = queries + static_cast<size_t>(b) * nq * 3;
  const int nqe = RAGGED ? cloud_len(len_q, b, nq) : nq;
  const int nce = RAGGED ? cloud_len(len_c, b, nc) : nc;
  float px[NCH], py[NCH], pz[NCH];
#pragma unroll
  for (int ch = 0; ch < NCH; ++ch) {
    const int k = min(ch * 64 + lane, nc - 1);
    px[ch] = c[k * 3 + 0];
    py[ch] = c[k * 3 + 1];
    pz[ch] = c[k * 3 + 2];
  }
#pragma unroll
  for (int ch = 0; ch < NCH; ++ch) {
    const bool ok = ch * 64 + lane < nce;
    px[ch] = ok ? px[ch] : __builtin_inff();
    py[ch] = ok ? py[ch] : __builtin_inff();
    pz[ch] = ok ? pz[ch] : __builtin_inff();
  }
  const int j0 = (blockIdx.x * 4 + wave) * qpw;
  __builtin_amdgcn_s_waitcnt(0x0F70);
  const int jf = min(j0, nq - 1);
  float nqx = q[jf * 3 + 0], nqy = q[jf * 3 + 1], nqz = q[jf * 3 + 2];
  for (int jj = 0; jj < qpw; ++jj) {
    const int j = j0 + jj;
    if (j >= nq) break;
    const float qx = nqx, qy = nqy, qz = nqz;
    {
      const int jn = min(j + 1, nq - 1);
      nqx = q[jn * 3 + 0], nqy = q[jn * 3 + 1], nqz = q[jn * 3 + 2];
    }
    if (RAGGED && j >= nqe) {
      if (lane < K) {
        const size_t o = (static_cast<size_t>(b) * nq + j) * K + lane;
        dists[o] = 0.0f;
        idx[o] = static_cast<IdxT>(-1);
        if (nn) nn[o * 3 + 0] = nn[o * 3 + 1] = nn[o * 3 + 2] = 0.0f;
      }
      continue;
    }
    float d[NCH];
    float m = __builtin_inff();
    if constexpr (NCH % 2 == 0) {
      typedef float f2 __attribute__((ext_vector_type(2)));
      const f2 qx2 = {qx, qx}, qy2 = {qy, qy}, qz2 = {qz, qz};
#pragma unroll
      for (int ch = 0; ch < NCH; ch += 2) {
        const f2 dx = qx2 - f2{px[ch], px[ch + 1]}, dy = qy2 - f2{py[ch], py[ch + 1]},
                 dz = qz2 - f2{pz[ch], pz[ch + 1]};
        const f2 dd = __builtin_elementwise_fma(dz, dz, __builtin_elementwise_fma(dy, dy, dx * dx));
        d[ch] = dd.x;
        d[ch + 1] = dd.y;
        m = fminf(m, fminf(dd.x, dd.y));
      }
    } else {
#pragma unroll
      for (int ch = 0; ch < NCH; ++ch) {
        const float dx = qx - px[ch], dy = qy - py[ch], dz = qz - pz[ch];
        d[ch] = PDR_ACC3(dx, dy, dz);
        m = fminf(m, d[ch]);
      }
    }
    unsigned g = __float_as_uint(m);
    {
      unsigned o = __builtin_amdgcn_update_dpp(0u, g, 0xB1, 0xf, 0xf, false);
      g = o < g ? o : g;
      o = __builtin_amdgcn_update_dpp(0u, g, 0x4E, 0xf, 0xf, false);
      g = o < g ? o : g;
      o = __builtin_amdgcn_update_dpp(0u, g, 0x141, 0xf, 0xf, false);
      g = o < g ? o : g;
    }
    const unsigned T = pdr::wave_max_u32(g);
    int base = 0;
#pragma unroll
    for (int ch = 0; ch < NCH; ++ch) {
      const unsigned bits = __float_as_uint(d[ch]);
      const bool hit = bits <= T && (!RAGGED || ch * 64 + lane < nce);
      const unsigned long long mask = __ballot(hit);
      if (mask != 0ull) {
        const int pos = base + __builtin_amdgcn_mbcnt_hi(static_cast<unsigned>(mask >> 32),
                                                         __builtin_amdgcn_mbcnt_lo(static_cast<unsigned>(mask), 0u));
        if (hit && pos < 64) cand[wave][pos] = pdr::u64_from(bits, static_cast<unsigned>(ch * 64 + lane));
        base += __builtin_popcountll(mask);
      }
    }
    __builtin_amdgcn_wave_barrier();
    if (base >= K && base <= 64) {
      const unsigned long long key = lane < base ? cand[wave][lane] : ~0ull;
      const unsigned klo = static_cast<unsigned>(key), khi = static_cast<unsigned>(key >> 32);
      int rank = 0;
      for (int r = 0; r < base; ++r) {
        const unsigned long long kr =
            pdr::u64_from(__builtin_amdgcn_readlane(khi, r), __builtin_amdgcn_readlane(klo, r));
        rank += kr < key ? 1 : 0;
      }
      if (lane < base && rank < K) {
        outd[wave][rank] = __uint_as_float(khi);
        outi[wave][rank] = static_cast<int>(klo);
      }
    } else {
      unsigned long long last = 0ull;
      for (int r = 0; r < K; ++r) {
        unsigned long long best = ~0ull;
#pragma unroll
        for (int ch = 0; ch < NCH; ++ch) {
          const unsigned long long key =
              ch * 64 + lane < nce ? pdr::u64_from(__float_as_uint(d[ch]), static_cast<unsigned>(ch * 64 + lane))
                                  : ~0ull;
          if ((r == 0 || key > last) && key < best) best = key;
        }
        best = ~pdr::wave_max_u64(~best);
        if (lane == 0) {
          outd[wave][r] = __uint_as_float(static_cast<unsigned>(best >> 32));
          outi[wave][r] = static_cast<int>(static_cast<unsigned>(best));
        }
        last = best;
      }
    }
    __builtin_amdgcn_wave_barrier();
    if (lane < K) {
      const bool empty = RAGGED && static_cast<unsigned>(outi[wave][lane]) >= static_cast<unsigned>(nce);
      const float dk = empty ? 0.0f : outd[wave][lane];
      const int ik = empty ? -1 : outi[wave][lane];
      const size_t o = (static_cast<size_t>(b) * nq + j) * K + lane;
      dists[o] = dk;
      idx[o] = static_cast<IdxT>(ik);
      if (nn) {
        const int a = empty ? 0 : ik;
        nn[o * 3 + 0] = empty ? 0.0f : c[a * 3 + 0];
        nn[o * 3 + 1] = empty ? 0.0f : c[a * 3 + 1];
        nn[o * 3 + 2] = empty ? 0.0f : c[a * 3 + 2];
      }
      if (wgt) {
        const float rk = 1.0f / (dk + 1e-8f);
        outr[wave][lane] = rk;
        __builtin_amdgcn_wave_barrier();
        float norm = 0.0f;
        for (int t = 0; t < K; ++t) norm += outr[wave][t];
        wgt[o] = rk / norm;
      }
    }
    __builtin_amdgcn_wave_barrier();
  }
}

template <typename IdxT, bool RAGGED = false>
bool launch_knn_wave(const float* x, const float* y, int B, int n1, int n2, int K, float* dists, IdxT* idx, float* nn,
                     float* wgt, hipStream_t s, const int64_t* len1 = nullptr, const int64_t* len2 = nullptr) {
  const bool on = pdr::option(pdr::OPT_KNN_WAVE) != 0;
  if (!on || K > 8 || n2 < 64 || n2 > 1024) return false;
  int qpw = 16;
  while (qpw > 1 && static_cast<long long>(B) * ((n1 + 4 * qpw - 1) / (4 * qpw)) < 1024) qpw >>= 1;
  const dim3 grid((n1 + 4 * qpw - 1) / (4 * qpw), B);
#define PDR_KW(NCH)                                                                                                  \
  hipLaunchKernelGGL((knn_wave_kernel<NCH, IdxT, RAGGED>), grid, dim3(256), 0, s, x, y, n1, n2, K, qpw, dists, idx, nn, \
                     wgt, len1, len2)
  if (n2 <= 64) PDR_KW(1);
  else if (n2 <= 128) PDR_KW(2);
  else if (n2 <= 256) PDR_KW(4);
  else if (n2 <= 512) PDR_KW(8);
  else PDR_KW(16);
#undef PDR_KW
  return true;
}

typedef float f32x2 __attribute__((ext_vector_type(2)));

template <int QP, typename IdxT, bool RAGGED = false>
__global__ __launch_bounds__(256) void nn1_kernel(const float* __restrict__ xa, const float* __restrict__ xb,
                                                  int na, int nb, float* __restrict__ da,
                                                  IdxT* __restrict__ ia, float* __restrict__ db,
                                                  IdxT* __restrict__ ib,
                                                  const int64_t* __restrict__ len_a = nullptr,
                                                  const int64_t* __restrict__ len_b = nullptr, int pad_idx = -1) {
  constexpr int CH = 8;
  constexpr int NQ = 2 * QP;
  __shared__ float4 tile[kTile];
  const int dir = blockIdx.z;
  const float* queries = dir ? xb : xa;
  const float* cloud = dir ? xa : xb;
  const int nq = dir ? nb : na, nc = dir ? na : nb;
  float* dists = dir ? db : da;
  IdxT* idx = dir ? ib : ia;
  if (static_cast<int>(blockIdx.x) * 256 * NQ >= nq) return;
  const int b = blockIdx.y;
  const float* c = cloud + static_cast<size_t>(b) * nc * 3;
  const int q0 = blockIdx.x * 256 * NQ + threadIdx.x;
  const int nqe = RAGGED ? cloud_len(dir ? len_b : len_a, b, nq) : nq;
  const int nce =
      !RAGGED ? nc : (static_cast<int>(blockIdx.x) * 256 * NQ < nqe ? cloud_len(dir ? len_a : len_b, b, nc) : 0);
  f32x2 qx[QP], qy[QP], qz[QP], best[QP];
  int bchunk[NQ];
#pragma unroll
  for (int p = 0; p < QP; ++p) {
#pragma unroll
    for (int h = 0; h < 2; ++h) {
      const int j = min(q0 + 256 * (2 * p + h), nq - 1);
      const float* q = queries + (static_cast<size_t>(b) * nq + j) * 3;
      qx[p][h] = q[0];
      qy[p][h] = q[1];
      qz[p][h] = q[2];
      bchunk[2 * p + h] = 0;
    }
    best[p] = f32x2{__builtin_inff(), __builtin_inff()};
  }
  for (int k0 = 0; k0 < nce; k0 += kTile) {
    const int kn = (nce - k0) < kTile ? (nce - k0) : kTile;
    const int kpad = (kn + CH - 1) / CH * CH;
    __syncthreads();
    for (int t = threadIdx.x; t < kpad; t += 256) {
      const float* s = c + static_cast<size_t>(k0 + min(t, kn - 1)) * 3;
      tile[t] = t < kn ? make_float4(s[0], s[1], s[2], 0.0f)
                       : make_float4(__builtin_inff(), __builtin_inff(), __builtin_inff(), 0.0f);
    }
    __syncthreads();
    for (int t0 = 0; t0 < kpad; t0 += CH) {
      f32x2 cm[QP];
#pragma unroll
      for (int p = 0; p < QP; ++p) cm[p] = f32x2{__builtin_inff(), __builtin_inff()};
#pragma unroll
      for (int u = 0; u < CH; ++u) {
        const float4 pt = tile[t0 + u];
#pragma unroll
        for (int p = 0; p < QP; ++p) {
          const f32x2 dx = qx[p] - pt.x, dy = qy[p] - pt.y, dz = qz[p] - pt.z;
// ... 67 lines not shown
    constexpr int QPB = 256 * 2 * PDR_NN1_QP;
    hipLaunchKernelGGL((nn1_kernel<PDR_NN1_QP, int64_t, RAGGED>), dim3((n1 + QPB - 1) / QPB, B, 1), dim3(256), 0, s, x,
                       y, n1, n2, dists, idx, static_cast<float*>(nullptr), static_cast<int64_t*>(nullptr), len1, len2,
                       -1);
    return pdr::check_launch();
  }
  if (K == 1) return launch_knn<1, RAGGED>(x, y, len1, len2, B, n1, n2, K, dists, idx, nn, s);
  if (K <= n2 && launch_knn_wave<int64_t, RAGGED>(x, y, B, n1, n2, K, dists, idx, nn, nullptr, s, len1, len2))
    return pdr::check_launch();
  if (K <= 4) return launch_knn<4, RAGGED>(x, y, len1, len2, B, n1, n2, K, dists, idx, nn, s);
  if (K <= 8) return launch_knn<8, RAGGED>(x, y, len1, len2, B, n1, n2, K, dists, idx, nn, s);
  if (K <= 16) return launch_knn<16, RAGGED>(x, y, len1, len2, B, n1, n2, K, dists, idx, nn, s);
  return launch_knn<32, RAGGED>(x, y, len1, len2, B, n1, n2, K, dists, idx, nn, s);
}

template <bool RAGGED>
int chamfer_nn(const float* x, const float* y, const int64_t* len1, const int64_t* len2, int B, int n1, int n2,
               float* dist_xy, int64_t* idx_xy, float* dist_yx, int64_t* idx_yx, pdr_stream_t stream) {
  if (B < 0 || n1 <= 0 || n2 <= 0) return PDR_EINVAL;
  if (B == 0) return PDR_OK;
  if (!x || !y || !dist_xy || !idx_xy || !dist_yx || !idx_yx) return PDR_EINVAL;
  const int nmax = n1 > n2 ? n1 : n2;
  constexpr int QPB = 256 * 2 * PDR_NN1_QP;
  hipLaunchKernelGGL((nn1_kernel<PDR_NN1_QP, int64_t, RAGGED>), dim3((nmax + QPB - 1) / QPB, B, 2), dim3(256), 0,
                     pdr::as_stream(stream), x, y, n1, n2, dist_xy, idx_xy, dist_yx, idx_yx, len1, len2, 0);
  return pdr::check_launch();
}

}

extern "C" int pdr_three_nn(const float* unknown, const float* known, int B, int n, int m,
                            float* dist2, int* idx, pdr_stream_t stream) {
  if (B < 0 || n < 0 || m < 0) return PDR_EINVAL;
  if (B == 0 || n == 0) return PDR_OK;
  if (!unknown || !dist2 || !idx || (m > 0 && !known)) return PDR_EINVAL;
  dim3 grid((n + 255) / 256, B);
  hipLaunchKernelGGL((nn_search_kernel<3, kSum3, int, false>), grid, dim3(256), 0,
                     pdr::as_stream(stream), unknown, known, n, m, 3, dist2, idx,
                     static_cast<float*>(nullptr));
  return pdr::check_launch();
}

extern "C" int pdr_knn_points(const float* x, const float* y, int B, int n1, int n2, int K,
                              float* dists, int64_t* idx, float* nn, pdr_stream_t stream) {
  return knn_points<false>(x, y, nullptr, nullptr, B, n1, n2, K, dists, idx, nn, stream);
}

extern "C" int pdr_knn_points_ragged(const float* x, const float* y, const int64_t* lengths1, const int64_t* lengths2,
                                     int B, int n1, int n2, int K, float* dists, int64_t* idx, float* nn,
                                     pdr_stream_t stream) {
  if (!lengths1 && !lengths2) return knn_points<false>(x, y, nullptr, nullptr, B, n1, n2, K, dists, idx, nn, stream);
  return knn_points<true>(x, y, lengths1, lengths2, B, n1, n2, K, dists, idx, nn, stream);
}

extern "C" int pdr_chamfer_nn(const float* x, const float* y, int B, int n1, int n2, float* dist_xy,
                              int64_t* idx_xy, float* dist_yx, int64_t* idx_yx, pdr_stream_t stream) {
  return chamfer_nn<false>(x, y, nullptr, nullptr, B, n1, n2, dist_xy, idx_xy, dist_yx, idx_yx, stream);
}

extern "C" int pdr_chamfer_nn_ragged(const float* x, const float* y, const int64_t* lengths1, const int64_t* lengths2,
                                     int B, int n1, int n2, float* dist_xy, int64_t* idx_xy, float* dist_yx,
                                     int64_t* idx_yx, pdr_stream_t stream) {
  if (!lengths1 && !lengths2)
    return chamfer_nn<false>(x, y, nullptr, nullptr, B, n1, n2, dist_xy, idx_xy, dist_yx, idx_yx, stream);
  return chamfer_nn<true>(x, y, lengths1, lengths2, B, n1, n2, dist_xy, idx_xy, dist_yx, idx_yx, stream);
}

extern "C" int pdr_knn_group(const float* x, const float* y, int B, int n1, int n2, int K, float* dists,
                             int* idx, float* weights, pdr_stream_t stream) {
  if (B < 0 || n1 < 0 || n2 <= 0 || K <= 0 || K > n2) return PDR_EINVAL;
  if (K > 16) return PDR_EUNSUPPORTED;
  if (B == 0 || n1 == 0) return PDR_OK;
  if (!x || !y || !dists || !idx || !weights) return PDR_EINVAL;
  hipStream_t s = pdr::as_stream(stream);
  if (launch_knn_wave<int>(x, y, B, n1, n2, K, dists, idx, nullptr, weights, s)) return pdr::check_launch();
  const dim3 grid((n1 + 255) / 256, B);
#define PDR_KG(KK)                                                                                      \
  hipLaunchKernelGGL((nn_search_kernel<KK, kAcc3, int, false>), grid, dim3(256), 0, s, x, y, n1, n2, K,  \
                     dists, idx, static_cast<float*>(nullptr), weights)
  if (K <= 4) PDR_KG(4);
  else if (K <= 8) PDR_KG(8);
  else PDR_KG(16);
#undef PDR_KG
  return pdr::check_launch();
}

namespace {
__global__ __launch_bounds__(256) void knn_grad_kernel(const float* __restrict__ x,
                                                       const float* __restrict__ y,
                                                       const int64_t* __restrict__ idx,
                                                       const float* __restrict__ gd, int n1, int n2, int K,
                                                       float* __restrict__ gx, float* __restrict__ gy) {
  const int b = blockIdx.y;
  const int j = blockIdx.x * 256 + threadIdx.x;
  if (j >= n1) return;
  const float* q = x + (static_cast<size_t>(b) * n1 + j) * 3;
  const float* p = y + static_cast<size_t>(b) * n2 * 3;
  float* gp = gy + static_cast<size_t>(b) * n2 * 3;
  const float qx = q[0], qy = q[1], qz = q[2];
  float ax = 0.0f, ay = 0.0f, az = 0.0f;
  for (int t = 0; t < K; ++t) {
    const int64_t k = idx[(static_cast<size_t>(b) * n1 + j) * K + t];
    if (k < 0) continue;
    const float g = 2.0f * gd[(static_cast<size_t>(b) * n1 + j) * K + t];
    const float dx = g * (qx - p[k * 3 + 0]);
    const float dy = g * (qy - p[k * 3 + 1]);
    const float dz = g * (qz - p[k * 3 + 2]);
    ax += dx;
    ay += dy;
    az += dz;
    atomicAdd(gp + k * 3 + 0, -dx);
    atomicAdd(gp + k * 3 + 1, -dy);
    atomicAdd(gp + k * 3 + 2, -dz);
  }
  float* o = gx + (static_cast<size_t>(b) * n1 + j) * 3;
  o[0] = ax;
  o[1] = ay;
  o[2] = az;
}
}

extern "C" int pdr_knn_points_grad(const float* x, const float* y, const int64_t* idx,
                                   const float* grad_dists, int B, int n1, int n2, int K, float* grad_x,
                                   float* grad_y, pdr_stream_t stream) {
  if (B < 0 || n1 < 0 || n2 < 0 || K <= 0) return PDR_EINVAL;
  if (B == 0) return PDR_OK;
  hipStream_t s = pdr::as_stream(stream);
  if (n2 > 0) {
    if (!grad_y) return PDR_EINVAL;
    if (hipMemsetAsync(grad_y, 0, sizeof(float) * static_cast<size_t>(B) * n2 * 3, s) != hipSuccess)
      return PDR_ELAUNCH;
  }
  if (n1 == 0) return PDR_OK;
  if (!x || !idx || !grad_dists || !grad_x || (n2 > 0 && !y)) return PDR_EINVAL;
  hipLaunchKernelGGL(knn_grad_kernel, dim3((n1 + 255) / 256, B), dim3(256), 0, s, x, y, idx, grad_dists, n1, n2,
                     K, grad_x, grad_y);
  return pdr::check_launch();
}
```

### point_diffusion_refinement_amd/csrc/pdr_common.h

```cpp
#pragma once
#include <hip/hip_runtime.h>
#include <stdint.h>

#include "../../include/pdr_hip.h"

#define PDR_SUM3(a, b, c) __builtin_fmaf((c), (c), __builtin_fmaf((a), (a), (b) * (b)))
#define PDR_ACC3(a, b, c) __builtin_fmaf((c), (c), __builtin_fmaf((b), (b), (a) * (a)))

#define PDR_WAVE 64

namespace pdr {

void set_last_error(hipError_t e);

inline int check_launch() {
  hipError_t e = hipGetLastError();
  if (e != hipSuccess) {
    set_last_error(e);
    return PDR_ELAUNCH;
  }
  return PDR_OK;
}

inline hipStream_t as_stream(pdr_stream_t s) { return reinterpret_cast<hipStream_t>(s); }

inline unsigned blocks_for(long total) { return static_cast<unsigned>((total + 255) / 256); }

enum Opt {
  OPT_FUSED_WS, OPT_NARROW_KC32, OPT_FPS_WAVE, OPT_FPS_LEAN, OPT_KNN_WAVE, OPT_GN_FOLD_SMALL, OPT_WS_NARROW3,
  OPT_WS_XCD_ORDER, OPT_DEEP_CHUNKS, OPT_DEEP_KS, OPT_DEEP_JOBS32, OPT_DEEP_JOBS64, OPT_COUNT
};
int option(Opt o);

struct PoolArgs {
  const float* values;
  const float* vscale;
  const float* vshift;
  const int* counts;
  float* out;
  int ldv, ldo, K, v_relu;
};

struct GatherTwin {
  const int* idx0;
  float* Y;
  const int* wrow0;
  int ldy, n_main;
  float wmul;
};

struct WsTwin {
  pdr_layer_in_t in[2];
  float* Y[2];
  float* partial[2];
  int ldy[2], n_row_tiles[2];
  int gx;
};

template <int CTRL>
__device__ __forceinline__ unsigned dpp_u32(unsigned v) {
  return __builtin_amdgcn_update_dpp(0u, v, CTRL, 0xf, 0xf, false);
}

__device__ __forceinline__ unsigned long long u64_from(unsigned hi, unsigned lo) {
  return (static_cast<unsigned long long>(hi) << 32) | lo;
}

template <int CTRL>
__device__ __forceinline__ unsigned long long dpp_max_step_u64(unsigned long long v) {
  const unsigned lo = dpp_u32<CTRL>(static_cast<unsigned>(v));
  const unsigned hi = dpp_u32<CTRL>(static_cast<unsigned>(v >> 32));
  const unsigned long long o = u64_from(hi, lo);
  return o > v ? o : v;
}

__device__ __forceinline__ unsigned long long wave_max_u64(unsigned long long v) {
  v = dpp_max_step_u64<0x111>(v);
  v = dpp_max_step_u64<0x112>(v);
  v = dpp_max_step_u64<0x114>(v);
  v = dpp_max_step_u64<0x118>(v);
  v = dpp_max_step_u64<0x142>(v);
  v = dpp_max_step_u64<0x143>(v);
  const unsigned lo = __builtin_amdgcn_readlane(static_cast<unsigned>(v), 63);
  const unsigned hi = __builtin_amdgcn_readlane(static_cast<unsigned>(v >> 32), 63);
  return u64_from(hi, lo);
}

template <int CTRL>
__device__ __forceinline__ unsigned dpp_max_step_u32(unsigned v) {
  const unsigned o = dpp_u32<CTRL>(v);
  return o > v ? o : v;
}
__device__ __forceinline__ unsigned wave_max_u32(unsigned v) {
  v = dpp_max_step_u32<0x111>(v);
  v = dpp_max_step_u32<0x112>(v);
  v = dpp_max_step_u32<0x114>(v);
  v = dpp_max_step_u32<0x118>(v);
  v = dpp_max_step_u32<0x142>(v);
  v = dpp_max_step_u32<0x143>(v);
  return __builtin_amdgcn_readlane(v, 63);
}

__device__ __forceinline__ float wave_sum_f32(float v) {
#pragma unroll
  for (int off = 32; off >= 1; off >>= 1) v += __shfl_xor(v, off, 64);
  return v;
}

__device__ __forceinline__ int lane_id() { return threadIdx.x & 63; }

__device__ __forceinline__ unsigned bitrev(unsigned v, int bits) {
  return bits == 0 ? 0u : (__brev(v) >> (32 - bits));
}

__device__ __forceinline__ int xcd_contiguous(int bid, int nb) {
// ... 8 lines not shown
```

### point_diffusion_refinement_amd/pointnet2/fused_network.py

```python
import contextlib
import ctypes
from collections import namedtuple

import torch
import torch.nn as nn
import torch.nn.functional as F

from .. import _lib
from ..pointnet2_ops import _ext
from ..pointnet2_ops.attention import MyGroupNorm
from .models.pointnet2_ssg_sem import calc_t_emb


USE_SPLIT_FIRST = True
SPLIT_QUERY_CONV = True
FUSE_SCORE_POOL = True
FUSE_CONDITION_BRANCH = True
USE_VIRTUAL_FIRST = True
USE_VIRTUAL_KNN = True
GATHER_RES = 4096
GATHER_RES_KNN = True
NATIVE_EMBED = True
STEP_TABLE = True
FUSE_GLOBAL_PNET = True
# ... 112 lines not shown
            seg.fill(li.seg[i])
        li.scale = self.scale.data_ptr() if self.scale is not None else None
        li.shift = self.shift.data_ptr() if self.shift is not None else None
        li.add = self.add.data_ptr() if self.add is not None else None
        li.add_ld = self.add_ld if self.add is not None else 0
        if self.radd is not None:
            self.radd.fill(li.rseg)
        li.pre_relu, li.post_relu, li.rows_per_batch = int(self.pre_relu), int(self.post_relu), self.rpb
        li.ss_ld = self.ss_ld
        if self.oadd is not None:
            li.oadd, li.oadd_ld, li.oadd_div = self.oadd[0].data_ptr(), self.oadd[0].shape[1], self.oadd[1]
            if self.oadd_rows is not None:
                li.oadd_rows = self.oadd_rows.data_ptr()
        if self.gidx is not None:
            li.gidx = self.gidx.data_ptr()
            li.gcnt = self.gcnt.data_ptr() if self.gcnt is not None else None
            li.gK = self.gK
            if self.gs1 is not None:
                li.gs1, li.gs2 = self.gs1.data_ptr(), self.gs2.data_ptr()
        li.partial_tpb = partial_tpb
        if self.dd is not None:
            li.tile_list, li.n_tiles = self.dd.tile_list.data_ptr(), self.dd.n_tiles.data_ptr()
            li.partial_tpb = partial_tpb or self.dd.ptpb
        if weighted and self.wrow0 is not None:
            li.wrow0, li.wmul = self.wrow0.data_ptr(), self.wmul
        if self.patch is not None:
            Vd, w = self.patch
            li.patch_values, li.patch_ld, li.patch_w = Vd.data_ptr(), Vd.shape[1], w.data_ptr()
        li.walk_reverse = self.walk()
        return li


_NET_DEDUP = [True]
_PROBE = [None]


def _dedup_on():
    return DEDUP and _NET_DEDUP[0]


def _probe_ptr():
    return _PROBE[0].data_ptr() if _PROBE[0] is not None else None


class Dedup:

    def __init__(self, idx, counts, B, m, K, prepared=None):
        dev = idx.device
        self.B, self.m, self.K = B, m, K
        self.tpb, self.tpbd = m * K // 128, (m + 127) // 128
        self.ptpb = self.tpb + self.tpbd
        nt = B * self.tpb
        self.idx0 = torch.empty((B, m), dtype=torch.int32, device=dev)
        self.row_w = torch.empty((B * m,), dtype=torch.float32, device=dev)
        self.tile_valid = torch.empty((nt,), dtype=torch.uint8, device=dev)
        self.tile_list = torch.empty((nt,), dtype=torch.int32, device=dev)
        self.n_tiles = torch.empty((1,), dtype=torch.int32, device=dev)
        self.nvalid = None
        if prepared is not None:
            prepared(self)
            return
        _lib.check(_lib.load().pdr_dedup_plan(idx.data_ptr(), counts.data_ptr(), B, m, K, self.idx0.data_ptr(),
                                              self.row_w.data_ptr(), self.tile_valid.data_ptr(),
                                              self.tile_list.data_ptr(), self.n_tiles.data_ptr(), _stream()),
                   "dedup_plan")
        nv = self.tile_valid.view(B, self.tpb).sum(1, dtype=torch.int32)
        self.nvalid = torch.stack([nv, nv * (128 // K)]).contiguous()
        if _PROBE[0] is not None:
            _PROBE[0][0:1] += self.n_tiles
            _PROBE[0][1:2] += nt

    @property
    def wrow0(self):
        return self.nvalid[1]

    def moments(self, Yd, C, relu_col0, partial):
        _lib.check(_lib.load().pdr_weighted_moments(Yd.data_ptr(), Yd.shape[1], self.B, self.m, C, relu_col0,
                                                    self.row_w.data_ptr(), partial.data_ptr(), self.ptpb, self.tpb,
                                                    self.tile_valid.data_ptr(), _stream()), "weighted_moments")


class SortedQueries:

    def __init__(self, idx, counts, new_xyz):
        B, m, K = idx.shape
        dev = idx.device
        lib = _lib.load()
        self.perm = torch.empty((B, m), dtype=torch.int32, device=dev)
        self.inv = torch.empty((B, m), dtype=torch.int32, device=dev)
        self.perm_rows = torch.empty((B, m), dtype=torch.int32, device=dev)
        self.plan = None
        if FUSED_PLAN and K in (8, 16, 32) and (m * K) % 128 == 0 and B <= 1024 and m <= 4096:
            new_xyz = new_xyz.contiguous()
            self.idx = torch.empty_like(idx)
            self.counts = torch.empty_like(counts)
            self.xyz = torch.empty_like(new_xyz)
            nvalid = torch.empty((2, B), dtype=torch.int32, device=dev)

            def prepared(dd):
                _lib.check(lib.pdr_dedup_prepare(
                    idx.data_ptr(), counts.data_ptr(), new_xyz.data_ptr(), B, m, K, self.perm.data_ptr(),
                    self.inv.data_ptr(), self.perm_rows.data_ptr(), self.idx.data_ptr(), self.counts.data_ptr(),
                    self.xyz.data_ptr(), dd.idx0.data_ptr(), dd.row_w.data_ptr(), dd.tile_valid.data_ptr(),
                    dd.tile_list.data_ptr(), dd.n_tiles.data_ptr(), nvalid.data_ptr(), _probe_ptr(), _stream()),
                    "dedup_prepare")
                dd.nvalid = nvalid
            self.plan = Dedup(self.idx, self.counts, B, m, K, prepared=prepared)
            return
        _lib.check(lib.pdr_dedup_sort(counts.data_ptr(), B, m, self.perm.data_ptr(), self.inv.data_ptr(),
                                      self.perm_rows.data_ptr(), _stream()), "dedup_sort")
        self.idx = gather_rows(idx.view(torch.float32), self.perm).view(torch.int32)
        self.counts = gather_rows(counts.view(B, m, 1).view(torch.float32), self.perm).view(torch.int32).view(B, m)
        self.xyz = gather_rows(new_xyz.contiguous(), self.perm)
        if K in (8, 16, 32) and (m * K) % 128 == 0:
            self.plan = Dedup(self.idx, self.counts, B, m, K)


Window = namedtuple("Window", "partial col0 C tpb mult sub", defaults=(1.0, None))


class Stats(namedtuple("Stats", "partial tpb sub", defaults=(None,))):
    __slots__ = ()

    def window(self, col0, C, mult=1.0):
        return Window(self.partial, col0, C, self.tpb, mult, self.sub)


class LayerOut:
    __slots__ = ("Y", "stats", "folded", "twin", "dd")

    def __init__(self, Y, stats, folded=None, twin=None, dd=None):
        self.Y, self.stats, self.folded, self.twin, self.dd = Y, stats, folded, twin, dd

    def __iter__(self):
        return iter((self.Y, self.stats.partial, self.stats.tpb))


Values = namedtuple("Values", "V scale shift twin")
Injected = namedtuple("Injected", "t off ld")
QueryTables = namedtuple("QueryTables", "V2 order", defaults=(None,))
Head = namedtuple("Head", "B m K counts first folded sq rows query q_ahead", defaults=(None,) * 5)
Prepared = namedtuple("Prepared", "head values event", defaults=(None,))


def _ready(x):
    return lambda: x


def act_from(lo, C, P, B, rpb, **kw):
    a = Act([Seg(lo.Y, 0, C, lo.Y.shape[1])], P, B, rpb, **kw)
    if lo.dd is not None:
        a.dd = lo.dd
        a.twin = _twin_act([Seg(lo.twin, 0, C, lo.twin.shape[1])], lo.dd, B, **kw)
    return a


def _twin_act(segs, dd, B, **kw):
    tw = Act(segs, dd.B * dd.m, B, dd.m, **kw)
    if TWIN_STATS:
        tw.wrow0, tw.wmul = dd.wrow0, float(dd.K)
    return tw


class FirstOut:

    def __init__(self, Y=None, stats=None, U=None, V2=None, ld=0, has_v0=False, idx=None, counts=None, K=0, nsrc=0,
                 zrow=-1, Yres=None, res_col0=0, res_cols=0, s1=None, s2=None, r1=None, r2=None, materialise=None):
        self.Y, self.stats, self.U, self.V2, self.ld, self.has_v0 = Y, stats, U, V2, ld, has_v0
        self.idx, self.counts, self.K, self.nsrc, self.zrow = idx, counts, K, nsrc, zrow
        self.Yres, self.res_col0, self.res_cols = Yres, res_col0, res_cols
        self.s1, self.s2, self.r1, self.r2 = s1, s2, r1, r2
        self.materialise = materialise
        self.dd, self.deg = None, None

    @property
    def virtual(self):
        return self.Y is None

    def seg(self, col0, C):
        if not self.virtual:
            return Seg(self.Y, col0, C, self.Y.shape[1])
        if self.Yres is not None and col0 >= self.res_col0 and col0 + C <= self.res_col0 + self.res_cols:
            return Seg(self.Yres, col0 - self.res_col0, C, self.Yres.shape[1])
        kNN = self.s1 is not None
        g = Gather(V=(self.V2, col0), V0=(self.V2, self.ld + col0) if self.has_v0 else None, ldv=self.V2.shape[1],
                   nsrc=self.nsrc, zrow=self.zrow, r1=(self.r1, col0) if kNN else None,
                   r2=(self.r2, col0) if kNN else None)
        return Seg(self.U, col0, C, self.U.shape[1], 1, g)

    def attach(self, act):
        if self.virtual:
            act.gidx, act.gcnt, act.gK = self.idx, self.counts, self.K
            act.gs1, act.gs2, act.first = self.s1, self.s2, self
        if self.dd is not None:
            dd, Yd = self.dd, self.deg
            if act.twin is None:
                if len(act.segs) != 1 or not act.segs[0].gathered:
                    raise NotImplementedError("deduplicated block: one gathered source per layer")
                sg = act.segs[0]
                tw = _twin_act([Seg(Yd, sg.off, sg.C, Yd.shape[1])], dd, act.B)
                for k in Act._SHARED:
                    object.__setattr__(tw, k, getattr(act, k))
                act.dd, act.twin = dd, tw
            if act.radd is not None and act.radd.gathered:
                act.twin.radd = Seg(Yd, act.radd.off, act.radd.C, Yd.shape[1])
        return act


def _pad4(c):
    return (c + 3) // 4 * 4


Padded = namedtuple("Padded", "src padded stream event")
_XYZ4 = {}
_GEOM = {}
_WALK = {}


def _new_forward():
    _XYZ4.clear()
    _GEOM.clear()
    _WALK.clear()


class Geom:
    __slots__ = ("tensor", "sorted", "probed")

    def __init__(self, tensor):
        self.tensor, self.sorted, self.probed = tensor, None, False


def _geom(idx, create=False):
    e = _GEOM.get(id(idx))
    if e is None and create:
        e = _GEOM[id(idx)] = Geom(idx)
    return e


def xyz4(t):
    if t.shape[-1] % 4 == 0:
        return t
    key = (t.data_ptr(), tuple(t.shape))
    hit = _XYZ4.get(key)
    if hit is None:
        C = t.shape[-1]
        stream = ev = None
        if t.is_cuda and t.dtype == torch.float32 and t.is_contiguous():
            padded = torch.empty(t.shape[:-1] + (_pad4(C),), dtype=torch.float32, device=t.device)
            _lib.check(_lib.load().pdr_pad_rows(t.data_ptr(), t.numel() // C, C, padded.data_ptr(), _pad4(C),
                                                _stream()), "pad_rows")
        else:
            padded = torch.nn.functional.pad(t, (0, -C % 4)).contiguous()
        if t.is_cuda:
            cur = torch.cuda.current_stream(t.device)
            stream, ev = cur.cuda_stream, torch.cuda.Event()
            ev.record(cur)
        hit = _XYZ4[key] = Padded(t, padded, stream, ev)
    elif hit.event is not None:
        cur = torch.cuda.current_stream(t.device)
        if cur.cuda_stream != hit.stream:
            cur.wait_event(hit.event)
    return hit.padded


def plain(t2d, B, rows_per_batch, row_div=1, C=None):
    rows, ld = t2d.shape
    C = ld if C is None else C
    return Act([Seg(t2d, 0, C, ld, row_div)], rows * row_div, B, rows_per_batch)


class Conv:

    def __init__(self, convs):
        convs = [c for c in convs if c is not None]
        ws = [c.weight.detach().reshape(c.weight.shape[0], -1) for c in convs]
        wt = torch.cat(ws, 0).t().contiguous()
        self.Cin, self.Cout = wt.shape
        dev = wt.device
        self.ldw = _pad4(self.Cout)
        self.Wt = torch.zeros((self.Cin, self.ldw), dtype=torch.float32, device=dev)
        self.Wt[:, :self.Cout] = wt
        self.bias = torch.cat([c.bias.detach() if c.bias is not None else torch.zeros(w.shape[0], device=dev)
                               for c, w in zip(convs, ws)]).contiguous()
        self.widths = [w.shape[0] for w in ws]
        self.f16x3 = {}
        self.pair_ok = {}

    def f16x3_image(self, seg_widths, TN):
        key = tuple(seg_widths) + (TN,)
        if key not in self.f16x3:
            self.f16x3[key] = pack_f16x3(self.Wt, self.Cout, key[:-1], TN)
        return self.f16x3[key]


SIDE_TABLES = True
FPS_STREAM = True
_PAR = {"stream": None}


def _on_aux(fn):
    aux = _PAR["stream"]
    if aux is None:
        return None
    main = torch.cuda.current_stream()
    ev = torch.cuda.Event()
    ev.record(main)
    aux.wait_event(ev)
    with torch.cuda.stream(aux):
        result = fn()
        done = torch.cuda.Event()
        done.record(aux)

    def join():
        main.wait_event(done)
        return result
    return join


@contextlib.contextmanager
def _single_stream():
    saved, _PAR["stream"] = _PAR["stream"], None
    try:
        yield
    finally:
        _PAR["stream"] = saved


_PRECISION = ["f32"]
SPLIT_VARIANTS = (4, 5, 8)
SPLIT_MIN_CIN = 64


def _apply_lab_opts():
    spec = __import__("os").environ.get("PDR_FUSED_OPTS", "")
    for item in filter(None, (t.strip() for t in spec.split(","))):
        name, _, val = item.partition("=")
        cur = globals().get(name)
        if name.startswith("_") or not isinstance(cur, (bool, int)):
            raise ValueError("PDR_FUSED_OPTS: unknown option %r" % name)
        globals()[name] = (val.lower() in ("1", "true", "on")) if isinstance(cur, bool) else int(val)


_apply_lab_opts()


def pack_f16x3(Wt, Cout, seg_widths, TN=128):
    KC = 32
    W = Wt[:, :Cout].float()
    half = torch.float16
    hi = W.to(half)
    if not bool(torch.isfinite(hi).all()):
        raise ValueError("split-f16 arithmetic: a weight is not finite or exceeds the f16 range (65504); use "
                         "precision='f32' for this network")
    lo = (W - hi.float()).to(half)
    chunks, k = [], 0
    for C in seg_widths:
        for ks in range(0, C, KC):
            chunks.append((k + ks, min(KC, C - ks)))
        k += C
    assert k == W.shape[0]
    ncb = (Cout + TN - 1) // TN
    img = torch.zeros((ncb, len(chunks), 2, TN, KC), dtype=half, device=Wt.device)
    for cb in range(ncb):
        n0 = cb * TN
        nn_ = min(TN, Cout - n0)
        for ci, (k0, km) in enumerate(chunks):
            img[cb, ci, 0, :nn_, :km] = hi[k0:k0 + km, n0:n0 + nn_].t()
            img[cb, ci, 1, :nn_, :km] = lo[k0:k0 + km, n0:n0 + nn_].t()
    img = img.view(ncb, len(chunks), 2, TN, 4, 8)
    n = torch.arange(TN, device=Wt.device)
    pos = torch.arange(4, device=Wt.device)[None, :] ^ ((n >> 2) & 3)[:, None]
    img = img.gather(4, pos[None, None, None, :, :, None].expand_as(img)).contiguous()
    return img.view(torch.int16).reshape(-1), len(chunks)


def _launch_split(lib, act, conv, li, y_ptr, ldy, partial_ptr, relu_col0, tiny_exact=True):
    if _PRECISION[0] != "split_f16" or conv.Cin < SPLIT_MIN_CIN:
        return False
    if torch.is_tensor(partial_ptr):
# ... 674 lines not shown
        self.device = a.device
        self._dense = None

    def dense(self):
        if self._dense is None:
            self._dense = torch.cat(self.parts, dim=2)
        return self._dense


def feature_segments(feats_cl):
    parts = feats_cl.parts if isinstance(feats_cl, Cat) else (feats_cl,)
    return [Seg(xyz4(t), 0, t.shape[2], _pad4(t.shape[2])) for t in parts]


def gather_rows(src_cl, idx):
    if isinstance(src_cl, Cat):
        a, b = src_cl.parts
        B, n, C = src_cl.shape
        m = idx.shape[1]
        out = torch.empty((B, m, C), dtype=torch.float32, device=a.device)
        _lib.check(_lib.load().pdr_gather_rows2(a.data_ptr(), a.shape[2], b.data_ptr(), b.shape[2], idx.data_ptr(), B, n,
                                                m, out.data_ptr(), _stream()), "gather_rows2")
        return out
    B, n, C = src_cl.shape
    m = idx.shape[1]
    out = torch.empty((B, m, C), dtype=torch.float32, device=src_cl.device)
    _lib.check(_lib.load().pdr_gather_rows(src_cl.data_ptr(), idx.data_ptr(), B, n, C, m, out.data_ptr(),
                                           _stream()), "gather_rows")
    return out


class FusedGroupedBlock:

    def __init__(self, grouper, mlp, att, bank):
        if grouper.neighbor_def != 'radius' or not grouper.use_xyz:
            raise NotImplementedError("fused path: radius neighbourhoods with xyz channels")
        self.radius, self.nsample = grouper.radius, grouper.nsample
        self.with_abs, self.with_centre = grouper.include_abs_coordinate, grouper.include_center_coordinate
        self.att = FusedAttention(att)
        self.mlp = FusedMlp(mlp, bank, extra_convs=[self.att.key_conv])
        self.split = None
        self.static_U = None
        self.dedup = False
        self._t128 = {}

    _WS_ON = []

    @staticmethod
    def _ws_kernels_on():
        if not FusedGroupedBlock._WS_ON:
            li = _lib.LayerIn()
            li.n_seg = 1
            li.seg[0].ptr, li.seg[0].C, li.seg[0].ld, li.seg[0].row_div = 0x1000, 64, 64, 1
            li.rows_per_batch = 8192
            plan = (ctypes.c_int * 8)()
            rc = _lib.load().pdr_fused_layer_plan(ctypes.byref(li), 8192, 64, 0x1000, 64, 64, 0x1000, 64, plan)
            FusedGroupedBlock._WS_ON.append(rc == 0 and plan[0] == 1)
        return FusedGroupedBlock._WS_ON[0]

    def _tiles_128(self, rpb):
        if rpb not in self._t128:
            tr = _lib.load().pdr_fused_layer_tile_rows
            couts = [c.Cout for c in self.mlp.rest] + [self.att.v.Cout, self.att.w1.Cout, self.att.w2.Cout]
            self._t128[rpb] = all(tr(rpb, c) == 128 for c in couts)
        return self._t128[rpb]

    def _plan(self, idx, counts, B, m, K, sq=None):
        if not self._eligible(idx, m, K):
            return None
        return sq.plan if (sq is not None and sq.idx is idx) else None

    def _shape_ok(self, idx, m, K):
        return (self.dedup and USE_SPLIT_FIRST and USE_VIRTUAL_FIRST and SPLIT_QUERY_CONV and
                K in (8, 16, 32) and m >= DEDUP_MIN_QUERIES and (m * K) % 128 == 0 and idx.dtype == torch.int32 and
                self._ws_kernels_on() and self._tiles_128(m * K))

    def _eligible(self, idx, m, K):
        return _dedup_on() and self._shape_ok(idx, m, K)

    def _sorted(self, idx):
        e = _geom(idx)
        return e.sorted if (e is not None and _dedup_on() and self.dedup) else None

    def plan_ahead(self, neigh, new_xyz):
        idx, counts = neigh
        B, m, K = idx.shape
        e = _geom(idx, create=True)
        if self._eligible(idx, m, K):
            if e.sorted is None:
                e.sorted = SortedQueries(idx, counts, new_xyz)
        elif _PROBE[0] is not None and self._shape_ok(idx, m, K) and not e.probed:
            _lib.check(_lib.load().pdr_dedup_probe(counts.data_ptr(), B, m, K, _probe_ptr(), _stream()), "dedup_probe")
            e.probed = True
        return neigh

    def side_tables(self, neigh, new_xyz, has_v0):
        sq = self._sorted(neigh[0])
        return QueryTables(self.split.query_tables(sq.xyz if sq is not None else new_xyz, has_v0=has_v0), sq)

    def _make_split(self, Cs):
        if self.split is None:
            self.split = SplitFirstConv(self.mlp.first, Cs, 'ball', self.with_abs, self.with_centre)
        return self.split

    @staticmethod
    def _in_place(K):
        return QUERIES_IN_PLACE and SPLIT_QUERY_CONV and K in (32, 64)

    def prepare_static_source(self, src_xyz, src_feats_cl):
        if not USE_SPLIT_FIRST:
            return
        U = self._make_split(src_feats_cl.shape[2]).source_table(src_feats_cl, src_xyz)
        if self.static_U is U:
            pass
        elif self.static_U is not None and self.static_U.shape == U.shape:
            self.static_U.copy_(U)
        else:
            self.static_U = U

    def neighbours(self, src_xyz, new_xyz):
        return _ext.ball_query(new_xyz, src_xyz, self.radius, self.nsample)

    @staticmethod
    def _ordered(query_feats_cl, sq, rows):
        return gather_rows(query_feats_cl, sq.perm) if (sq is not None and rows is None) else query_feats_cl

    def _head(self, src_xyz, src_feats_cl, new_xyz, subset, neigh, tables, U=None, query=None, q_ahead=None):
        B, m, _ = new_xyz.shape
        K = self.nsample
        idx, counts = neigh if neigh is not None else self.neighbours(src_xyz, new_xyz)
        sq, rows = self._sorted(idx), None
        if sq is not None:
            idx, counts, new_xyz = sq.idx, sq.counts, sq.xyz
            rows = sq.perm_rows if self._in_place(K) else None
        if query is not None:
            query = self._ordered(query, sq, rows)
            if q_ahead is not None and not (sq is None or rows is not None):
                q_ahead = None
            if q_ahead is None and QUERY_CONV_AHEAD and SPLIT_QUERY_CONV:
                qf = query.reshape(B * m, -1)
                q_ahead = _on_aux(lambda: self.att.query_conv(qf, B, m))
        first, folded = self._make_split(src_feats_cl.shape[2])(
            src_feats_cl, src_xyz, new_xyz, idx, None if subset else counts, K, self.mlp.extra_col0,
            virtual=USE_VIRTUAL_FIRST, U=U if U is not None else self.static_U,
            V2=tables.V2 if (tables is not None and tables.order is sq) else None,
            dd=self._plan(idx, counts, B, m, K, sq), **self.mlp.first_conv_args(m * K))
        return Head(B, m, K, counts, first, folded, sq, rows, query, q_ahead)

    def _values(self, hd, bank):
        h, _ = self.mlp.after_first(hd.first, hd.B * hd.m * hd.K, hd.B, hd.m * hd.K, bank, folded=hd.folded)
        return self.att.values(h, hd.B, hd.m, hd.K)

    def _pool(self, hd, query_feats_cl, values, q_ahead=None):
        out = self.att(query_feats_cl.reshape(hd.B * hd.m, -1), hd.first, self.mlp.extra_col0, hd.counts, hd.B, hd.m,
                       hd.K, values, sorted_q=hd.sq, query_rows=hd.rows, q_ahead=q_ahead)
        return out.view(hd.B, hd.m, -1)

    def prepare(self, src_xyz, src_feats_cl, new_xyz, bank, subset, neigh=None, V2=None):
        if USE_SPLIT_FIRST:
            hd = self._head(src_xyz, src_feats_cl, new_xyz, subset, neigh, V2)
            return Prepared(hd, _ready(self._values(hd, bank)))
        B, m, _ = new_xyz.shape
        idx, counts = neigh if neigh is not None else self.neighbours(src_xyz, new_xyz)
        K = self.nsample
        dense_feats = src_feats_cl.dense() if isinstance(src_feats_cl, Cat) else src_feats_cl
        G, Cg = group_build(dense_feats, src_xyz, new_xyz, idx, counts, not subset, self.with_abs, self.with_centre)
        h, first = self.mlp(plain(G, B, m * K, C=Cg), bank)
        return Prepared(Head(B, m, K, counts, first), _ready(self.att.values(h, B, m, K)))

    def finish(self, prep, query_feats_cl):
        hd = prep.head
        return self._pool(hd, self._ordered(query_feats_cl, hd.sq, hd.rows), prep.values)

    def __call__(self, src_xyz, src_feats_cl, new_xyz, query_feats_cl, bank, subset, neigh=None, V2=None, U=None,
                 q_ahead=None):
# ... 396 lines not shown
                l_xyz.append(gather_rows(l_xyz[i], sel))
                ev_fps[i] = event(fps_s)

        def transfer_level(lv, tables_for):
            with torch.cuda.stream(side):
                for blk in ([self.enc_map[lv]] if lv < nlev else []) + [self.dec_map[lv]]:
                    if fm_key(lv, blk) not in fm_neigh:
                        fm_neigh[fm_key(lv, blk)] = blk.plan_ahead(blk.neighbours(l_uvw[lv], l_xyz[lv]), l_xyz[lv])
                    if side_tables_on and blk.split is not None and blk in tables_for:
                        tables[id(blk)] = blk.side_tables(fm_neigh[fm_key(lv, blk)], l_xyz[lv], True)
                ev_fm[lv] = event(side)

        def group_level(i):
            sa = self.sa[i]
            if not fps_on:
                sample_level(i)
            with torch.cuda.stream(side):
                if fps_on:
                    side.wait_event(ev_fps[i])
                sa_neigh[i] = sa.plan_ahead(sa.neighbours(l_xyz[i], l_xyz[i + 1]), l_xyz[i + 1])
                xyz4(l_xyz[i + 1])
                if side_tables_on and sa.split is not None:
                    tables[id(sa)] = sa.side_tables(sa_neigh[i], l_xyz[i + 1], False)
                ev_sa[i] = event(side)

        with torch.cuda.stream(fps_s):
            mark("fps:begin")
        if fps_on:
            sample_level(0)
        transfer_level(0, (self.enc_map[0], self.dec_map[0]) if hoist0_main else (self.enc_map[0],))
        with torch.cuda.stream(side):
            mark("side:first_ball_query_done")
        if fps_on:
            for i in range(1, nlev):
                sample_level(i)

        mark("main:before_embeddings", detail=True)
        self._embeddings(ts, label)
        mark("main:embeddings_done")
        ev_emb = event(main)

        def transfer(blk, l, cl, query, V2=None, q_ahead=None):
            prep = prepared.get(id(blk))
            if prep is not None:
                if prep.event is not None:
                    main.wait_event(prep.event)
                return blk.finish(prep, query)
            return blk(l_uvw[l], cl[l], l_xyz[l], query, bank, subset=False, neigh=fm_neigh[fm_key(l, blk)], V2=V2,
                       q_ahead=q_ahead)

        prepared = {}
        hoist = AHEAD_DECODER_MAPS and USE_SPLIT_FIRST and self.two_streams
        hoisted = [False]
        hoist_enc = AHEAD_ENCODER_MAPS and hoist and (_dedup_on() or AHEAD_ENCODER_MAPS_WHOLE)

        def hoist_map(blk, cl, l):
            if tables.get(id(blk)) is None:
                return
            with torch.cuda.stream(side):
                if not hoisted[0]:
                    side.wait_event(ev_emb)
                    hoisted[0] = True
                with _single_stream():
                    prep = blk.prepare(l_uvw[l], cl[l], l_xyz[l], bank, subset=False, neigh=fm_neigh[fm_key(l, blk)],
                                       V2=tables[id(blk)])
                prepared[id(blk)] = prep._replace(event=event(side))

        def geometry_tail():
            with torch.cuda.stream(side):
                mark("side:encoder_geometry_done")
                if side_tables_on:
                    if self.dec_map[0].split is not None and id(self.dec_map[0]) not in tables:
                        tables[id(self.dec_map[0])] = self.dec_map[0].side_tables(fm_neigh[fm_key(0, self.dec_map[0])],
                                                                                  l_xyz[0], True)
                    for i in range(-1, -(len(self.fp) + 1), -1):
                        fp = self.fp[i]
                        if fp.split is not None:
                            tables[id(fp)] = QueryTables(fp.split.query_tables(l_xyz[i - 1], has_v0=False))
                for i in range(-1, -(len(self.fp) + 1), -1):
                    knn[i] = _ext.knn_group(l_xyz[i - 1], l_xyz[i], self.fp[i].K)
                mark("side:knn_done")
                return event(side)

        for k in range(nlev):
            group_level(k)
            lv = k + 1
            transfer_level(lv, (self.enc_map[lv],) if lv < nlev else (self.dec_map[lv],))
            if lv < nlev and hoist_enc:
                hoist_map(self.enc_map[lv], enc_cl, lv)
        if side_tables_on:
            with torch.cuda.stream(side):
                for l in range(1, nlev):
                    blk = self.dec_map[l]
                    if blk.split is not None and id(blk) not in tables:
                        tables[id(blk)] = blk.side_tables(fm_neigh[fm_key(l, blk)], l_xyz[l], True)
        ev_knn = geometry_tail()
        if hoist:
            for l in range(nlev, 0 if hoist0_main else -1, -1):
                hoist_map(self.dec_map[l], dec_cl, l)

        def table_early(split, Cm, early_feats, src_xyz):
            aux = _PAR["stream"]
            if not (SPLIT_SOURCE_TABLES and USE_SPLIT_FIRST and aux is not None) or early_feats.shape[2] % 4 != 0:
                return None
            aux.wait_event(event(main))
            with torch.cuda.stream(aux):
                part = split.source_table_early(Cm, early_feats, src_xyz)
                return part, event(aux)

        def table_late(split, pending, late_feats):
            if pending is None:
                return None
            main.wait_event(pending[1])
            return split.source_table_late(late_feats, pending[0])

        q0 = None
        if QUERY_CONV_AHEAD and SPLIT_QUERY_CONV and QUERIES_IN_PLACE and USE_SPLIT_FIRST and _PAR["stream"] is not None:
            q0 = _ready(self.enc_map[0].att.query_conv(feat0.reshape(B * N, -1), B, N))
        main.wait_event(ev_fm[0])
        mark("main:after_wait_first_ball_query")
        l_feat = [feat0]
        for i, sa in enumerate(self.sa):
            if i > 0:
                main.wait_event(ev_fm[i])
            Cm = self.enc_map[i].att.D
            pend = table_early(sa._make_split(Cm + l_feat[i].shape[2]), Cm, l_feat[i], l_xyz[i]) if i > 0 else None
            mapped = transfer(self.enc_map[i], i, enc_cl, l_feat[i], V2=tables.get(id(self.enc_map[i])),
                              q_ahead=q0 if i == 0 else None)
            mark("main:enc_map%d_done" % i)
            if i == 0 and hoist0_main and hoist and tables.get(id(self.dec_map[0])) is not None:
                with _single_stream():
                    prepared[id(self.dec_map[0])] = self.dec_map[0].prepare(
                        l_uvw[0], dec_cl[0], l_xyz[0], bank, subset=False, neigh=fm_neigh[fm_key(0, self.dec_map[0])],
                        V2=tables.get(id(self.dec_map[0])))
            sa_in = Cat(mapped, l_feat[i]) if USE_SPLIT_FIRST else torch.cat([mapped, l_feat[i]], dim=2)
            U_ahead = table_late(sa.split, pend, mapped)
            if i == 0 and SA0_TABLE_AHEAD and USE_SPLIT_FIRST and hoist0_main and _PAR["stream"] is not None:
                U_ahead = sa._make_split(sa_in.shape[2]).source_table(sa_in, l_xyz[i])
            main.wait_event(ev_sa[i])
            mark("main:after_wait_sa%d_geometry" % i)
            centre = gather_rows(sa_in, sels[i])
            l_feat.append(sa(l_xyz[i], sa_in, l_xyz[i + 1], centre, bank, subset=True, neigh=sa_neigh[i],
                             V2=tables.get(id(sa)), U=U_ahead))
            mark("main:sa%d_done" % i)
        main.wait_event(ev_knn)
        for i in range(-1, -(len(self.fp) + 1), -1):
            Cm = self.dec_map[i].att.D
            pend = table_early(self.fp[i]._make_split(Cm + l_feat[i].shape[2]), Cm, l_feat[i], l_xyz[i]) \
                if USE_SPLIT_FIRST else None
            mapped = transfer(self.dec_map[i], i % (nlev + 1), dec_cl, l_feat[i], V2=tables.get(id(self.dec_map[i])))
            fp_in = Cat(mapped, l_feat[i]) if USE_SPLIT_FIRST else torch.cat([mapped, l_feat[i]], dim=2)
            mark("main:dec_map%d_done" % (i % (nlev + 1)))
            l_feat[i - 1] = self.fp[i](l_xyz[i - 1], l_xyz[i], l_feat[i - 1], fp_in, bank, knn=knn[i],
                                       V2=tables.get(id(self.fp[i])), U=table_late(self.fp[i].split, pend, mapped))
            mark("main:fp%d_done" % (i % (nlev + 1)))
        mapped = transfer(self.dec_map[0], 0, dec_cl, l_feat[0], V2=tables.get(id(self.dec_map[0])))
        Cm, Cf = mapped.shape[2], l_feat[0].shape[2]
        head_in = Act([Seg(mapped, 0, Cm, Cm), Seg(l_feat[0], 0, Cf, Cf), Seg(xyz4(xyz), 0, 3, 4)], B * N, B, N)
        lo = run_layer(head_in, self.head1, fold=FoldReq(self.head_norm, self.head1.Cout, N))
        out = run_layer(act_from(lo, self.head1.Cout, B * N, B, N, scale=lo.folded[0], shift=lo.folded[1],
                                 post_relu=True), self.head2).Y
        mark("main:head_done")
        eps = out.view(B, N, out.shape[1])[:, :, :self.head2.Cout]
        return eps if self.return_strided_eps else eps.contiguous()

    __call__ = forward

    def reset_cond_features(self):
        self.net.reset_cond_features()
        self._synced = False
        self._label_key = None

    def parameters(self):
        return self.net.parameters()
```

### point_diffusion_refinement_amd/pointnet2_ops/_ext.py

```python
import torch

from .. import _lib


def _stream():
    return torch.cuda.current_stream().cuda_stream


def _req(t, name, dtype):
    if not isinstance(t, torch.Tensor):
        raise TypeError("%s must be a torch.Tensor" % name)
    if not t.is_cuda:
        raise RuntimeError("%s: CPU not supported" % name)
    if not t.is_contiguous():
        raise RuntimeError("%s must be a contiguous tensor" % name)
    if t.dtype != dtype:
        raise RuntimeError("%s must be a %s tensor" % (name, "float" if dtype == torch.float32 else "int"))


def _req_xyz(t, name):
    if t.dim() != 3 or t.shape[2] != 3:
        raise RuntimeError("%s must have shape (B, N, 3), got %s" % (name, tuple(t.shape)))


def _same_device(*ts):
    d = ts[0].device
    for t in ts[1:]:
        if t.device != d:
            raise RuntimeError("all tensors must live on the same device")


def furthest_point_sampling(points, nsamples):
    _req(points, "points", torch.float32)
    _req_xyz(points, "points")
    B, N, _ = points.shape
    lib = _lib.load()
    out = torch.empty((B, nsamples), dtype=torch.int32, device=points.device)
    ws = lib.pdr_fps_workspace_bytes(B, N)
    temp = torch.empty((ws // 4,), dtype=torch.float32, device=points.device) if ws else None
    with torch.cuda.device(points.device):
        _lib.check(lib.pdr_furthest_point_sampling(points.data_ptr(), B, N, int(nsamples),
                                                   temp.data_ptr() if temp is not None else None,
                                                   out.data_ptr(), _stream()), "furthest_point_sampling")
    return out


def gather_points(points, idx):
    _req(points, "points", torch.float32)
    _req(idx, "idx", torch.int32)
    _same_device(points, idx)
    B, C, N = points.shape
    m = idx.shape[1]
    out = torch.empty((B, C, m), dtype=torch.float32, device=points.device)
    with torch.cuda.device(points.device):
        _lib.check(_lib.load().pdr_gather_points(points.data_ptr(), idx.data_ptr(), B, C, N, m,
                                                 out.data_ptr(), _stream()), "gather_points")
    return out


def gather_points_grad(grad_out, idx, n):
    _req(grad_out, "grad_out", torch.float32)
    _req(idx, "idx", torch.int32)
    _same_device(grad_out, idx)
    B, C, m = grad_out.shape
    out = torch.empty((B, C, n), dtype=torch.float32, device=grad_out.device)
    with torch.cuda.device(grad_out.device):
        _lib.check(_lib.load().pdr_gather_points_grad(grad_out.data_ptr(), idx.data_ptr(), B, C, int(n), m,
                                                      out.data_ptr(), _stream()), "gather_points_grad")
    return out


def ball_query(new_xyz, xyz, radius, nsample):
    _req(new_xyz, "new_xyz", torch.float32)
    _req(xyz, "xyz", torch.float32)
    _req_xyz(new_xyz, "new_xyz")
    _req_xyz(xyz, "xyz")
    _same_device(new_xyz, xyz)
    if new_xyz.shape[0] != xyz.shape[0]:
        raise RuntimeError("new_xyz and xyz must have the same batch size")
    B, m, _ = new_xyz.shape
    n = xyz.shape[1]
    idx = torch.empty((B, m, nsample), dtype=torch.int32, device=xyz.device)
    counts = torch.empty((B, m), dtype=torch.int32, device=xyz.device)
    with torch.cuda.device(xyz.device):
        _lib.check(_lib.load().pdr_ball_query(new_xyz.data_ptr(), xyz.data_ptr(), B, n, m, float(radius),
                                              int(nsample), idx.data_ptr(), counts.data_ptr(), _stream()),
                   "ball_query")
    return idx, counts


def group_points(points, idx):
    _req(points, "points", torch.float32)
    _req(idx, "idx", torch.int32)
    _same_device(points, idx)
    B, C, N = points.shape
    _, npnt, ns = idx.shape
    out = torch.empty((B, C, npnt, ns), dtype=torch.float32, device=points.device)
    with torch.cuda.device(points.device):
        _lib.check(_lib.load().pdr_group_points(points.data_ptr(), idx.data_ptr(), B, C, N, npnt, ns,
                                                out.data_ptr(), _stream()), "group_points")
    return out


def group_points_grad(grad_out, idx, n):
    _req(grad_out, "grad_out", torch.float32)
    _req(idx, "idx", torch.int32)
    _same_device(grad_out, idx)
    B, C, npnt, ns = grad_out.shape
    out = torch.empty((B, C, n), dtype=torch.float32, device=grad_out.device)
    with torch.cuda.device(grad_out.device):
        _lib.check(_lib.load().pdr_group_points_grad(grad_out.data_ptr(), idx.data_ptr(), B, C, int(n), npnt, ns,
                                                     out.data_ptr(), _stream()), "group_points_grad")
    return out


def three_nn(unknowns, knows):
    _req(unknowns, "unknowns", torch.float32)
    _req(knows, "knows", torch.float32)
    _req_xyz(unknowns, "unknowns")
    _req_xyz(knows, "knows")
    _same_device(unknowns, knows)
    B, n, _ = unknowns.shape
    m = knows.shape[1]
    dist2 = torch.empty((B, n, 3), dtype=torch.float32, device=unknowns.device)
    idx = torch.empty((B, n, 3), dtype=torch.int32, device=unknowns.device)
    with torch.cuda.device(unknowns.device):
        _lib.check(_lib.load().pdr_three_nn(unknowns.data_ptr(), knows.data_ptr(), B, n, m, dist2.data_ptr(),
                                            idx.data_ptr(), _stream()), "three_nn")
    return [dist2, idx]


def three_interpolate(points, idx, weight):
    _req(points, "points", torch.float32)
    _req(idx, "idx", torch.int32)
    _req(weight, "weight", torch.float32)
    _same_device(points, idx, weight)
    B, C, m = points.shape
    n = idx.shape[1]
    out = torch.empty((B, C, n), dtype=torch.float32, device=points.device)
    with torch.cuda.device(points.device):
        _lib.check(_lib.load().pdr_three_interpolate(points.data_ptr(), idx.data_ptr(), weight.data_ptr(), B, C, m,
                                                     n, out.data_ptr(), _stream()), "three_interpolate")
    return out


def three_interpolate_grad(grad_out, idx, weight, m):
    _req(grad_out, "grad_out", torch.float32)
    _req(idx, "idx", torch.int32)
    _req(weight, "weight", torch.float32)
    _same_device(grad_out, idx, weight)
    B, C, n = grad_out.shape
    out = torch.empty((B, C, m), dtype=torch.float32, device=grad_out.device)
    with torch.cuda.device(grad_out.device):
        _lib.check(_lib.load().pdr_three_interpolate_grad(grad_out.data_ptr(), idx.data_ptr(), weight.data_ptr(), B,
                                                          C, n, int(m), out.data_ptr(), _stream()),
                   "three_interpolate_grad")
    return out


def _req_lengths(t, name, cloud):
    if t is None:
        return
    _req(t, name, torch.int64)
    if t.dim() != 1 or t.shape[0] != cloud.shape[0]:
        raise RuntimeError("%s must have shape (B,) = (%d,), got %s" % (name, cloud.shape[0], tuple(t.shape)))
    _same_device(cloud, t)


def _ptr(t):
    return t.data_ptr() if t is not None else None


def _knn_forward(p1, p2, K, return_nn, lengths1=None, lengths2=None):
    B, n1, _ = p1.shape
    n2 = p2.shape[1]
    dists = torch.empty((B, n1, K), dtype=torch.float32, device=p1.device)
    idx = torch.empty((B, n1, K), dtype=torch.int64, device=p1.device)
    nn = torch.empty((B, n1, K, 3), dtype=torch.float32, device=p1.device) if return_nn else None
    with torch.cuda.device(p1.device):
        if lengths1 is None and lengths2 is None:
            rc = _lib.load().pdr_knn_points(p1.data_ptr(), p2.data_ptr(), B, n1, n2, int(K), dists.data_ptr(),
                                            idx.data_ptr(), _ptr(nn), _stream())
        else:
            rc = _lib.load().pdr_knn_points_ragged(p1.data_ptr(), p2.data_ptr(), _ptr(lengths1), _ptr(lengths2), B,
                                                   n1, n2, int(K), dists.data_ptr(), idx.data_ptr(), _ptr(nn),
                                                   _stream())
        _lib.check(rc, "knn_points")
    return dists, idx, nn


def chamfer_nn(x, y, x_lengths=None, y_lengths=None):
    _req(x, "x", torch.float32)
    _req(y, "y", torch.float32)
    _same_device(x, y)
    if x.shape[2] != 3 or y.shape[2] != 3 or x.shape[0] != y.shape[0]:
        raise RuntimeError("chamfer_nn: (B,n,3) clouds with equal batch size")
    _req_lengths(x_lengths, "x_lengths", x)
    _req_lengths(y_lengths, "y_lengths", y)
    B, n1, _ = x.shape
    n2 = y.shape[1]
    dx = torch.empty((B, n1), dtype=torch.float32, device=x.device)
    dy = torch.empty((B, n2), dtype=torch.float32, device=x.device)
    ix = torch.empty((B, n1), dtype=torch.int64, device=x.device)
    iy = torch.empty((B, n2), dtype=torch.int64, device=x.device)
    with torch.cuda.device(x.device):
        if x_lengths is None and y_lengths is None:
            rc = _lib.load().pdr_chamfer_nn(x.data_ptr(), y.data_ptr(), B, n1, n2, dx.data_ptr(), ix.data_ptr(),
                                            dy.data_ptr(), iy.data_ptr(), _stream())
        else:
            rc = _lib.load().pdr_chamfer_nn_ragged(x.data_ptr(), y.data_ptr(), _ptr(x_lengths), _ptr(y_lengths), B,
                                                   n1, n2, dx.data_ptr(), ix.data_ptr(), dy.data_ptr(),
                                                   iy.data_ptr(), _stream())
        _lib.check(rc, "chamfer_nn")
    return dx, ix, dy, iy


def knn_group(x, y, K):
    _req(x, "x", torch.float32)
    _req(y, "y", torch.float32)
    _same_device(x, y)
    if x.dim() != 3 or y.dim() != 3 or x.shape[2] != 3 or y.shape[2] != 3 or x.shape[0] != y.shape[0]:
        raise RuntimeError("knn_group: x (B,n1,3) and y (B,n2,3) with equal batch size required, got %s and %s"
                           % (tuple(x.shape), tuple(y.shape)))
    B, n1, _ = x.shape
    n2 = y.shape[1]
    K = int(K)
    if K > min(n2, 16):
        d, i, _ = knn_points(x, y, K)
        w = 1.0 / (d + 1e-8)
        w = w / w.sum(dim=2, keepdim=True)
        return d, i.clamp(min=0).to(torch.int32), w
    d = torch.empty((B, n1, K), dtype=torch.float32, device=x.device)
    w = torch.empty((B, n1, K), dtype=torch.float32, device=x.device)
    i = torch.empty((B, n1, K), dtype=torch.int32, device=x.device)
    with torch.cuda.device(x.device):
        _lib.check(_lib.load().pdr_knn_group(x.data_ptr(), y.data_ptr(), B, n1, n2, int(K), d.data_ptr(),
                                             i.data_ptr(), w.data_ptr(), _stream()), "knn_group")
    return d, i, w


class _KnnDists(torch.autograd.Function):

    @staticmethod
    def forward(ctx, p1, p2, K, lengths1=None, lengths2=None):
        dists, idx, _ = _knn_forward(p1, p2, K, False, lengths1, lengths2)
        ctx.save_for_backward(p1, p2, idx)
        ctx.mark_non_differentiable(idx)
        return dists, idx

    @staticmethod
    def backward(ctx, grad_dists, _grad_idx):
        p1, p2, idx = ctx.saved_tensors
        B, n1, _ = p1.shape
        n2, K = p2.shape[1], idx.shape[2]
        g = grad_dists.contiguous().float()
        g1 = torch.empty_like(p1)
        g2 = torch.empty_like(p2)
        with torch.cuda.device(p1.device):
            _lib.check(_lib.load().pdr_knn_points_grad(p1.data_ptr(), p2.data_ptr(), idx.data_ptr(), g.data_ptr(), B,
                                                       n1, n2, K, g1.data_ptr(), g2.data_ptr(), _stream()),
                       "knn_points_grad")
        return g1, g2, None, None, None


def knn_points(p1, p2, K, return_nn=False, lengths1=None, lengths2=None):
    _req(p1, "p1", torch.float32)
    _req(p2, "p2", torch.float32)
    _same_device(p1, p2)
    if p1.shape[2] != 3 or p2.shape[2] != 3:
        raise RuntimeError("knn_points: only D=3 is built")
    _req_lengths(lengths1, "lengths1", p1)
    _req_lengths(lengths2, "lengths2", p2)
    if torch.is_grad_enabled() and (p1.requires_grad or p2.requires_grad):
        dists, idx = _KnnDists.apply(p1, p2, int(K), lengths1, lengths2)
        nn = None
        if return_nn:
            B, n1, _ = p1.shape
            safe = idx.clamp(min=0).reshape(B, n1 * int(K), 1).expand(-1, -1, 3)
            nn = p2.gather(1, safe).reshape(B, n1, int(K), 3) * (idx >= 0).unsqueeze(-1)
        return dists, idx, nn
    return _knn_forward(p1, p2, K, return_nn, lengths1, lengths2)
```

Baseline: 6012 cloud-steps/s.

## Batch per-level geometry kernels into multi-job grouped launches

Adds multi-job kernels for ball query, dedup prepare/probe, thin linear layers, kNN grouping and row padding. Each kernel takes a job table and maps blocks to jobs through a prefix search. The Python geometry stage is restructured to collect all levels' queries and launch them together on the side stream, replacing many small per-level launches. The goal is lower launch count and better GPU fill from tiny kernels, at the cost of heavier argument structs, runtime switch dispatch and a more complex scheduling path.

```diff
diff --git a/include/pdr_hip.h b/include/pdr_hip.h
--- a/include/pdr_hip.h
+++ b/include/pdr_hip.h
@@ -248,6 +248,66 @@
 int pdr_gather_rows2(const float *src0, int C0, const float *src1, int C1, const int *idx, int B, int n, int m,
                      float *out, pdr_stream_t stream);
 int pdr_pad_rows(const float *src, long rows, int C, float *out, int ldo, pdr_stream_t stream);
+#define PDR_MAX_JOBS 8
+typedef struct {
+  const float *new_xyz;
+  const float *xyz;
+  int n, m;
+  float radius;
+  int nsample;
+  int *idx;
+  int *counts;
+} pdr_ball_job_t;
+int pdr_ball_query_multi(const pdr_ball_job_t *jobs, int njobs, int B, pdr_stream_t stream);
+typedef struct {
+  const int *idx;
+  const int *counts;
+  const float *xyz;
+  int m, K;
+  int *perm, *inv, *perm_rows, *idx_s, *counts_s;
+  float *xyz_s;
+  int ld_xyz_s;
+  int probe_only;
+  int *idx0;
+  float *row_w;
+  unsigned char *tile_valid;
+  int *tile_list, *n_tiles, *nvalid;
+} pdr_prepare_job_t;
+int pdr_dedup_prepare_multi(const pdr_prepare_job_t *jobs, int njobs, int B, int *probe_acc, pdr_stream_t stream);
+int pdr_dedup_prepare_ld(const int *idx, const int *counts, const float *xyz, int B, int m, int K, int *perm, int *inv,
+                         int *perm_rows, int *idx_s, int *counts_s, float *xyz_s, int ld_xyz_s, int *idx0, float *row_w,
+                         unsigned char *tile_valid, int *tile_list, int *n_tiles, int *nvalid, int *probe_acc,
+                         pdr_stream_t stream);
+typedef struct {
+  const float *X;
+  int ldx, row_div;
+  long rows;
+  int Cin;
+  const float *Wt;
+  int ldw;
+  const float *bias;
+  int Cout;
+  float *Y;
+  int ldy;
+} pdr_thin_job_t;
+int pdr_thin_multi(const pdr_thin_job_t *jobs, int njobs, pdr_stream_t stream);
+typedef struct {
+  const float *x;
+  const float *y;
+  int n1, n2, K;
+  float *dists;
+  int *idx;
+  float *weights;
+} pdr_knn_job_t;
+int pdr_knn_group_multi(const pdr_knn_job_t *jobs, int njobs, int B, pdr_stream_t stream);
+typedef struct {
+  const float *src;
+  long rows;
+  int C;
+  float *out;
+  int ldo;
+} pdr_pad_job_t;
+int pdr_pad_rows_multi(const pdr_pad_job_t *jobs, int njobs, pdr_stream_t stream);
 int pdr_mark_time(unsigned long long *slot, pdr_stream_t stream);
 
 #ifdef __cplusplus
diff --git a/point_diffusion_refinement_amd/_lib.py b/point_diffusion_refinement_amd/_lib.py
--- a/point_diffusion_refinement_amd/_lib.py
+++ b/point_diffusion_refinement_amd/_lib.py
@@ -75,6 +75,12 @@
     "pdr_dedup_sort": (_I, [_P, _I, _I, _P, _P, _P, _P]),
     "pdr_weighted_moments": (_I, [_P, _I, _I, _I, _I, _I, _P, _P, _I, _I, _P, _P]),
     "pdr_patch_rows": (_I, [_P, _I, _P, _P, _I, _P, _I, _I, _I, _P, _I, _P, _P]),
+    "pdr_ball_query_multi": (_I, [_P, _I, _I, _P]),
+    "pdr_dedup_prepare_multi": (_I, [_P, _I, _I, _P, _P]),
+    "pdr_dedup_prepare_ld": (_I, [_P, _P, _P, _I, _I, _I, _P, _P, _P, _P, _P, _P, _I, _P, _P, _P, _P, _P, _P, _P, _P]),
+    "pdr_thin_multi": (_I, [_P, _I, _P]),
+    "pdr_knn_group_multi": (_I, [_P, _I, _I, _P]),
+    "pdr_pad_rows_multi": (_I, [_P, _I, _P]),
     "pdr_point_chain_plan": (_I, [_P, _I, _I, _P]),
     "pdr_point_chain": (_I, [_P, _I, _I, _P]),
 }
@@ -105,6 +111,37 @@
 class PointChain(_c.Structure):
     _fields_ = [("n_layers", _I), ("n_seg", _I), ("seg", ChainSeg * 3), ("layer", ChainLayer * 4), ("residual", _I),
                 ("ldo", _I), ("out", _P), ("scratch", _P), ("sync", _P)]
+
+
+MAX_JOBS = 8
+
+
+class BallJob(_c.Structure):
+    _fields_ = [("new_xyz", _P), ("xyz", _P), ("n", _I), ("m", _I), ("radius", _F), ("nsample", _I), ("idx", _P),
+                ("counts", _P)]
+
+
+class PrepareJob(_c.Structure):
+    _fields_ = [("idx", _P), ("counts", _P), ("xyz", _P), ("m", _I), ("K", _I), ("perm", _P), ("inv", _P),
+                ("perm_rows", _P), ("idx_s", _P), ("counts_s", _P), ("xyz_s", _P), ("ld_xyz_s", _I), ("probe_only", _I),
+                ("idx0", _P), ("row_w", _P), ("tile_valid", _P), ("tile_list", _P), ("n_tiles", _P), ("nvalid", _P)]
+
+
+class ThinJob(_c.Structure):
+    _fields_ = [("X", _P), ("ldx", _I), ("row_div", _I), ("rows", _c.c_long), ("Cin", _I), ("Wt", _P), ("ldw", _I),
+                ("bias", _P), ("Cout", _I), ("Y", _P), ("ldy", _I)]
+
+
+class KnnJob(_c.Structure):
+    _fields_ = [("x", _P), ("y", _P), ("n1", _I), ("n2", _I), ("K", _I), ("dists", _P), ("idx", _P), ("weights", _P)]
+
+
+class PadJob(_c.Structure):
+    _fields_ = [("src", _P), ("rows", _c.c_long), ("C", _I), ("out", _P), ("ldo", _I)]
+
+
+def job_array(jobs):
+    return (type(jobs[0]) * len(jobs))(*jobs)
 
 
 _lib = None
diff --git a/point_diffusion_refinement_amd/csrc/ball_query.hip b/point_diffusion_refinement_amd/csrc/ball_query.hip
--- a/point_diffusion_refinement_amd/csrc/ball_query.hip
+++ b/point_diffusion_refinement_amd/csrc/ball_query.hip
@@ -3,11 +3,10 @@
 namespace {
 
 template <int NCH, bool RESIDENT>
-__global__ __launch_bounds__(256) void ball_query_kernel(
+__device__ __forceinline__ void ball_query_body(
     const float* __restrict__ new_xyz, const float* __restrict__ xyz, int n, int m,
     float radius2, int nsample, int qpw, int* __restrict__ idx,
-    int* __restrict__ counts) {
-  const int b = blockIdx.y;
+    int* __restrict__ counts, int bx, int b) {
   const int lane = threadIdx.x & 63;
   const int wave = __builtin_amdgcn_readfirstlane(threadIdx.x >> 6);
   const float* p = xyz + static_cast<size_t>(b) * n * 3;
@@ -46,7 +45,7 @@
     __builtin_amdgcn_s_waitcnt(0x0F70);
   }
 
-  const int j0 = (blockIdx.x * 4 + wave) * qpw;
+  const int j0 = (bx * 4 + wave) * qpw;
   const int jf = min(j0, m - 1);
   float nqx = q[jf * 3 + 0], nqy = q[jf * 3 + 1], nqz = q[jf * 3 + 2];
   for (int jj = 0; jj < qpw; ++jj) {
@@ -95,6 +94,48 @@
 }
 
 template <int NCH, bool RESIDENT>
+__global__ __launch_bounds__(256) void ball_query_kernel(
+    const float* __restrict__ new_xyz, const float* __restrict__ xyz, int n, int m,
+    float radius2, int nsample, int qpw, int* __restrict__ idx,
+    int* __restrict__ counts) {
+  ball_query_body<NCH, RESIDENT>(new_xyz, xyz, n, m, radius2, nsample, qpw, idx, counts, blockIdx.x, blockIdx.y);
+}
+
+struct BallJob {
+  const float* new_xyz;
+  const float* xyz;
+  int* idx;
+  int* counts;
+  int n, m, nsample, gx, nch;
+  float radius2;
+};
+struct BallMulti {
+  pdr::JobPrefix pre;
+  BallJob job[PDR_MAX_JOBS];
+  int qpw;
+};
+
+__global__ __launch_bounds__(256) void ball_query_multi_kernel(const BallMulti a) {
+  const int j = pdr::find_job(a.pre, blockIdx.x);
+  const BallJob& J = a.job[j];
+  const int local = static_cast<int>(blockIdx.x - a.pre.first[j]);
+  const int b = local / J.gx, bx = local - b * J.gx;
+#define PDR_BQM(NCH)                                                                                              \
+  case NCH:                                                                                                       \
+    ball_query_body<NCH, true>(J.new_xyz, J.xyz, J.n, J.m, J.radius2, J.nsample, a.qpw, J.idx, J.counts, bx, b);  \
+    break
+  switch (J.nch) {
+    PDR_BQM(1);
+    PDR_BQM(2);
+    PDR_BQM(4);
+    PDR_BQM(8);
+    default:
+    PDR_BQM(16);
+  }
+#undef PDR_BQM
+}
+
+template <int NCH, bool RESIDENT>
 int launch(const float* new_xyz, const float* xyz, int B, int n, int m, float radius2,
            int nsample, int* idx, int* counts, hipStream_t s) {
   int qpw = 16;
@@ -129,3 +170,38 @@
 #undef PDR_BQ_CASE
   return launch<1, false>(new_xyz, xyz, B, n, m, radius2, nsample, idx, counts, s);
 }
+
+extern "C" int pdr_ball_query_multi(const pdr_ball_job_t* jobs, int njobs, int B, pdr_stream_t stream) {
+  if (!jobs || njobs < 1 || njobs > PDR_MAX_JOBS || B < 0) return PDR_EINVAL;
+  for (int j = 0; j < njobs; ++j) {
+    const pdr_ball_job_t& q = jobs[j];
+    if (q.n <= 0 || q.n > 1024 || q.m <= 0 || q.nsample <= 0 || !q.new_xyz || !q.xyz || !q.idx || !q.counts)
+      return PDR_EINVAL;
+    if (static_cast<long>(B) * q.m * q.nsample >= (1L << 31)) return PDR_EINVAL;
+  }
+  if (B == 0) return PDR_OK;
+  BallMulti a;
+  long wgs[PDR_MAX_JOBS];
+  int qpw = 32;
+  long tot;
+  do {
+    qpw >>= 1;
+    tot = 0;
+    for (int j = 0; j < njobs; ++j) tot += static_cast<long>(B) * ((jobs[j].m + 4 * qpw - 1) / (4 * qpw));
+  } while (qpw > 1 && tot < 1024);
+  a.qpw = qpw;
+  for (int j = 0; j < njobs; ++j) {
+    const pdr_ball_job_t& q = jobs[j];
+    BallJob& J = a.job[j];
+    J.new_xyz = q.new_xyz, J.xyz = q.xyz, J.idx = q.idx, J.counts = q.counts;
+    J.n = q.n, J.m = q.m, J.nsample = q.nsample;
+    J.gx = (q.m + 4 * qpw - 1) / (4 * qpw);
+    J.nch = q.n <= 64 ? 1 : q.n <= 128 ? 2 : q.n <= 256 ? 4 : q.n <= 512 ? 8 : 16;
+    J.radius2 = q.radius * q.radius;
+    wgs[j] = static_cast<long>(B) * J.gx;
+  }
+  for (int j = njobs; j < PDR_MAX_JOBS; ++j) a.job[j] = a.job[0];
+  if (!pdr::fill_prefix(&a.pre, wgs, njobs)) return PDR_EINVAL;
+  hipLaunchKernelGGL(ball_query_multi_kernel, dim3(a.pre.first[njobs]), dim3(256), 0, pdr::as_stream(stream), a);
+  return pdr::check_launch();
+}
diff --git a/point_diffusion_refinement_amd/csrc/dedup.hip b/point_diffusion_refinement_amd/csrc/dedup.hip
--- a/point_diffusion_refinement_amd/csrc/dedup.hip
+++ b/point_diffusion_refinement_amd/csrc/dedup.hip
@@ -108,10 +108,10 @@
 constexpr int kMaxPrepareClouds = 1024;
 constexpr int kMaxPrepareQueries = 4096;
 
-__global__ __launch_bounds__(1024) void dedup_prepare_kernel(
-    const int* __restrict__ idx, const int* __restrict__ counts, const float* __restrict__ xyz, int m, int K, int nB,
-    int* __restrict__ perm, int* __restrict__ inv, int* __restrict__ perm_rows, int* __restrict__ idx_s,
-    int* __restrict__ counts_s, float* __restrict__ xyz_s, int* __restrict__ idx0, float* __restrict__ row_w,
+__device__ __forceinline__ void dedup_prepare_body(
+    int b, const int* __restrict__ idx, const int* __restrict__ counts, const float* __restrict__ xyz, int m, int K,
+    int nB, int* __restrict__ perm, int* __restrict__ inv, int* __restrict__ perm_rows, int* __restrict__ idx_s,
+    int* __restrict__ counts_s, float* __restrict__ xyz_s, int ld_s, int* __restrict__ idx0, float* __restrict__ row_w,
     unsigned char* __restrict__ tile_valid, int* __restrict__ tile_list, int* __restrict__ n_tiles,
     int* __restrict__ nvalid, int* __restrict__ probe_acc) {
   __shared__ int nreal_s[kMaxPrepareClouds];
@@ -119,7 +119,6 @@
   __shared__ int wtot[16];
   __shared__ int base_s, prefix_s;
   const int tid = threadIdx.x, lane = tid & 63, wave = tid >> 6;
-  const int b = blockIdx.x;
   const int qpt = 128 / K, tpb = m / qpt;
   if (tid == 0) base_s = 0;
   const bool vec = (m & 3) == 0 && (reinterpret_cast<uintptr_t>(counts) & 15) == 0;
@@ -194,9 +193,10 @@
     row_w[qd] = j >= q0 ? static_cast<float>(K) : 0.0f;
     if (xyz) {
       const float x = xyz[qs * 3 + 0], y = xyz[qs * 3 + 1], z = xyz[qs * 3 + 2];
-      xyz_s[qd * 3 + 0] = x;
-      xyz_s[qd * 3 + 1] = y;
-      xyz_s[qd * 3 + 2] = z;
+      xyz_s[qd * ld_s + 0] = x;
+      xyz_s[qd * ld_s + 1] = y;
+      xyz_s[qd * ld_s + 2] = z;
+      if (ld_s == 4) xyz_s[qd * 4 + 3] = 0.0f;
     }
   }
   const int k4 = K / 4, ksh4 = __builtin_ctz(k4);
@@ -232,14 +232,25 @@
   }
 }
 
-__global__ __launch_bounds__(256) void dedup_probe_kernel(const int* __restrict__ counts, int m, int K,
-                                                          int* __restrict__ probe_acc) {
+__global__ __launch_bounds__(1024) void dedup_prepare_kernel(
+    const int* __restrict__ idx, const int* __restrict__ counts, const float* __restrict__ xyz, int m, int K, int nB,
+    int* __restrict__ perm, int* __restrict__ inv, int* __restrict__ perm_rows, int* __restrict__ idx_s,
+    int* __restrict__ counts_s, float* __restrict__ xyz_s, int ld_s, int* __restrict__ idx0, float* __restrict__ row_w,
+    unsigned char* __restrict__ tile_valid, int* __restrict__ tile_list, int* __restrict__ n_tiles,
+    int* __restrict__ nvalid, int* __restrict__ probe_acc) {
+  dedup_prepare_body(blockIdx.x, idx, counts, xyz, m, K, nB, perm, inv, perm_rows, idx_s, counts_s, xyz_s, ld_s, idx0,
+                     row_w, tile_valid, tile_list, n_tiles, nvalid, probe_acc);
+}
+
+template <int NT>
+__device__ __forceinline__ void dedup_probe_body(int b, const int* __restrict__ counts, int m, int K,
+                                                 int* __restrict__ probe_acc) {
   __shared__ int tot;
   if (threadIdx.x == 0) tot = 0;
   __syncthreads();
-  const int* cb = counts + static_cast<long>(blockIdx.x) * m;
+  const int* cb = counts + static_cast<long>(b) * m;
   int c = 0;
-  for (int i = threadIdx.x; i < m; i += 256) c += cb[i] > 1 ? 1 : 0;
+  for (int i = threadIdx.x; i < m; i += NT) c += cb[i] > 1 ? 1 : 0;
 #pragma unroll
   for (int off = 32; off >= 1; off >>= 1) c += __shfl_xor(c, off, 64);
   if ((threadIdx.x & 63) == 0 && c) atomicAdd(&tot, c);
@@ -251,21 +262,89 @@
   }
 }
 
+__global__ __launch_bounds__(256) void dedup_probe_kernel(const int* __restrict__ counts, int m, int K,
+                                                          int* __restrict__ probe_acc) {
+  dedup_probe_body<256>(blockIdx.x, counts, m, K, probe_acc);
+}
+
+struct PrepareMulti {
+  pdr::JobPrefix pre;
+  pdr_prepare_job_t job[PDR_MAX_JOBS];
+  int nB;
+  int* probe_acc;
+};
+
+__global__ __launch_bounds__(1024) void dedup_prepare_multi_kernel(const PrepareMulti a) {
+  const int j = pdr::find_job(a.pre, blockIdx.x);
+  const pdr_prepare_job_t& J = a.job[j];
+  const int b = static_cast<int>(blockIdx.x - a.pre.first[j]);
+  if (J.probe_only)
+    dedup_probe_body<1024>(b, J.counts, J.m, J.K, a.probe_acc);
+  else
+    dedup_prepare_body(b, J.idx, J.counts, J.xyz, J.m, J.K, a.nB, J.perm, J.inv, J.perm_rows, J.idx_s, J.counts_s,
+                       J.xyz_s, J.ld_xyz_s, J.idx0, J.row_w, J.tile_valid, J.tile_list, J.n_tiles, J.nvalid,
+                       a.probe_acc);
+}
+
+static int prepare_args_ok(const pdr_prepare_job_t& q, int B) {
+  if (!q.idx || !q.counts || !q.perm || !q.inv || !q.idx_s || !q.counts_s || (q.xyz && !q.xyz_s) || !q.idx0 || !q.row_w ||
+      !q.tile_valid || !q.tile_list || !q.n_tiles || !q.nvalid || B < 0 || q.m <= 0)
+    return PDR_EINVAL;
+  if (q.ld_xyz_s != 3 && q.ld_xyz_s != 4) return PDR_EINVAL;
+  if (!(q.K == 8 || q.K == 16 || q.K == 32) || (static_cast<long>(q.m) * q.K) % 128 != 0) return PDR_EINVAL;
+  if (static_cast<long>(B) * q.m * q.K >= (1L << 31)) return PDR_EINVAL;
+  if (B > kMaxPrepareClouds || q.m > kMaxPrepareQueries) return PDR_EUNSUPPORTED;
+  if ((reinterpret_cast<uintptr_t>(q.idx) | reinterpret_cast<uintptr_t>(q.idx_s)) % 16 != 0) return PDR_EINVAL;
+  return PDR_OK;
+}
+
+extern "C" int pdr_dedup_prepare_ld(const int* idx, const int* counts, const float* xyz, int B, int m, int K, int* perm,
+                                    int* inv, int* perm_rows, int* idx_s, int* counts_s, float* xyz_s, int ld_xyz_s,
+                                    int* idx0, float* row_w, unsigned char* tile_valid, int* tile_list, int* n_tiles,
+                                    int* nvalid, int* probe_acc, pdr_stream_t stream) {
+  const pdr_prepare_job_t q{idx, counts, xyz, m, K, perm, inv, perm_rows, idx_s, counts_s, xyz_s, ld_xyz_s, 0, idx0,
+                            row_w, tile_valid, tile_list, n_tiles, nvalid};
+  const int rc = prepare_args_ok(q, B);
+  if (rc != PDR_OK) return rc;
+  if (B == 0) return PDR_OK;
+  hipLaunchKernelGGL(dedup_prepare_kernel, dim3(B), dim3(1024), 0, pdr::as_stream(stream), idx, counts, xyz, m, K, B,
+                     perm, inv, perm_rows, idx_s, counts_s, xyz_s, ld_xyz_s, idx0, row_w, tile_valid, tile_list, n_tiles,
+                     nvalid, probe_acc);
+  return pdr::check_launch();
+}
+
 extern "C" int pdr_dedup_prepare(const int* idx, const int* counts, const float* xyz, int B, int m, int K, int* perm,
                                  int* inv, int* perm_rows, int* idx_s, int* counts_s, float* xyz_s, int* idx0,
                                  float* row_w, unsigned char* tile_valid, int* tile_list, int* n_tiles, int* nvalid,
                                  int* probe_acc, pdr_stream_t stream) {
-  if (!idx || !counts || !perm || !inv || !idx_s || !counts_s || (xyz && !xyz_s) || !idx0 || !row_w || !tile_valid ||
-      !tile_list || !n_tiles || !nvalid || B < 0 || m <= 0)
-    return PDR_EINVAL;
-  if (!(K == 8 || K == 16 || K == 32) || (static_cast<long>(m) * K) % 128 != 0) return PDR_EINVAL;
-  if (static_cast<long>(B) * m * K >= (1L << 31)) return PDR_EINVAL;
-  if (B > kMaxPrepareClouds || m > kMaxPrepareQueries) return PDR_EUNSUPPORTED;
-  if ((reinterpret_cast<uintptr_t>(idx) | reinterpret_cast<uintptr_t>(idx_s)) % 16 != 0) return PDR_EINVAL;
-  if (B == 0) return PDR_OK;
-  hipLaunchKernelGGL(dedup_prepare_kernel, dim3(B), dim3(1024), 0, pdr::as_stream(stream), idx, counts, xyz, m, K, B,
-                     perm, inv, perm_rows, idx_s, counts_s, xyz_s, idx0, row_w, tile_valid, tile_list, n_tiles, nvalid,
-                     probe_acc);
+  return pdr_dedup_prepare_ld(idx, counts, xyz, B, m, K, perm, inv, perm_rows, idx_s, counts_s, xyz_s, 3, idx0, row_w,
+                              tile_valid, tile_list, n_tiles, nvalid, probe_acc, stream);
+}
+
+extern "C" int pdr_dedup_prepare_multi(const pdr_prepare_job_t* jobs, int njobs, int B, int* probe_acc,
+                                       pdr_stream_t stream) {
+  if (!jobs || njobs < 1 || njobs > PDR_MAX_JOBS || B < 0) return PDR_EINVAL;
+  for (int j = 0; j < njobs; ++j) {
+    const pdr_prepare_job_t& q = jobs[j];
+    if (q.probe_only) {
+      if (!q.counts || !probe_acc || q.m <= 0) return PDR_EINVAL;
+      if (!(q.K == 8 || q.K == 16 || q.K == 32) || (static_cast<long>(q.m) * q.K) % 128 != 0) return PDR_EINVAL;
+    } else {
+      const int rc = prepare_args_ok(q, B);
+      if (rc != PDR_OK) return rc;
+    }
+  }
+  if (B == 0) return PDR_OK;
+  PrepareMulti a;
+  long wgs[PDR_MAX_JOBS];
+  for (int j = 0; j < PDR_MAX_JOBS; ++j) {
+    a.job[j] = jobs[j < njobs ? j : 0];
+    wgs[j] = B;
+  }
+  a.nB = B;
+  a.probe_acc = probe_acc;
+  if (!pdr::fill_prefix(&a.pre, wgs, njobs)) return PDR_EINVAL;
+  hipLaunchKernelGGL(dedup_prepare_multi_kernel, dim3(a.pre.first[njobs]), dim3(1024), 0, pdr::as_stream(stream), a);
   return pdr::check_launch();
 }
 
diff --git a/point_diffusion_refinement_amd/csrc/fused_gather.hip b/point_diffusion_refinement_amd/csrc/fused_gather.hip
--- a/point_diffusion_refinement_amd/csrc/fused_gather.hip
+++ b/point_diffusion_refinement_amd/csrc/fused_gather.hip
@@ -219,13 +219,29 @@
   out[e] = c < C0 ? src0[row * C0 + c] : src1[row * C1 + (c - C0)];
 }
 
-__global__ __launch_bounds__(256) void pad_rows_kernel(const float* __restrict__ src, int C, int ldo, long total,
-                                                       float* __restrict__ out) {
-  const long e = static_cast<long>(blockIdx.x) * 256 + threadIdx.x;
+__device__ __forceinline__ void pad_rows_body(long bx, const float* __restrict__ src, int C, int ldo, long total,
+                                              float* __restrict__ out) {
+  const long e = bx * 256 + threadIdx.x;
   if (e >= total) return;
   const long r = e / ldo;
   const int c = static_cast<int>(e - r * ldo);
   out[e] = c < C ? src[r * C + c] : 0.0f;
+}
+
+__global__ __launch_bounds__(256) void pad_rows_kernel(const float* __restrict__ src, int C, int ldo, long total,
+                                                       float* __restrict__ out) {
+  pad_rows_body(blockIdx.x, src, C, ldo, total, out);
+}
+
+struct PadMulti {
+  pdr::JobPrefix pre;
+  pdr_pad_job_t job[PDR_MAX_JOBS];
+};
+
+__global__ __launch_bounds__(256) void pad_rows_multi_kernel(const PadMulti a) {
+  const int j = pdr::find_job(a.pre, blockIdx.x);
+  const pdr_pad_job_t& J = a.job[j];
+  pad_rows_body(blockIdx.x - a.pre.first[j], J.src, J.C, J.ldo, J.rows * J.ldo, J.out);
 }
 
 }
@@ -333,6 +349,21 @@
   const long total = rows * ldo;
   hipLaunchKernelGGL(pad_rows_kernel, dim3(pdr::blocks_for(total)), dim3(256), 0, pdr::as_stream(stream), src, C, ldo,
                      total, out);
+  return pdr::check_launch();
+}
+
+extern "C" int pdr_pad_rows_multi(const pdr_pad_job_t* jobs, int njobs, pdr_stream_t stream) {
+  if (!jobs || njobs < 1 || njobs > PDR_MAX_JOBS) return PDR_EINVAL;
+  PadMulti a;
+  long wgs[PDR_MAX_JOBS];
+  for (int j = 0; j < njobs; ++j) {
+    const pdr_pad_job_t& q = jobs[j];
+    if (q.rows <= 0 || q.C <= 0 || q.ldo < q.C || !q.src || !q.out) return PDR_EINVAL;
+    wgs[j] = pdr::blocks_for(q.rows * q.ldo);
+  }
+  for (int j = 0; j < PDR_MAX_JOBS; ++j) a.job[j] = jobs[j < njobs ? j : 0];
+  if (!pdr::fill_prefix(&a.pre, wgs, njobs)) return PDR_EINVAL;
+  hipLaunchKernelGGL(pad_rows_multi_kernel, dim3(a.pre.first[njobs]), dim3(256), 0, pdr::as_stream(stream), a);
   return pdr::check_launch();
 }
 
diff --git a/point_diffusion_refinement_amd/csrc/fused_layer.hip b/point_diffusion_refinement_amd/csrc/fused_layer.hip
--- a/point_diffusion_refinement_amd/csrc/fused_layer.hip
+++ b/point_diffusion_refinement_amd/csrc/fused_layer.hip
@@ -445,14 +445,14 @@
   }
 }
 
-__global__ __launch_bounds__(256) void fused_layer_thin_kernel(const float* __restrict__ X, int ldx, int shift,
-                                                               int Cin, const float* __restrict__ Wt, int ldw,
-                                                               const float* __restrict__ bias, int Cout,
-                                                               float* __restrict__ Y, int ldy, long P, int qshift) {
+__device__ __forceinline__ void fused_layer_thin_body(int bx, int by, const float* __restrict__ X, int ldx, int shift,
+                                                      int Cin, const float* __restrict__ Wt, int ldw,
+                                                      const float* __restrict__ bias, int Cout,
+                                                      float* __restrict__ Y, int ldy, long P, int qshift) {
   constexpr int kThinIters = 8;
   const int ql = 1 << qshift;
   const int cq = threadIdx.x & (ql - 1), rl = threadIdx.x >> qshift;
-  const int c0 = 4 * (static_cast<int>(blockIdx.y) * ql + cq);
+  const int c0 = 4 * (by * ql + cq);
   if (c0 >= Cout) return;
   const int rpp = 256 >> qshift;
   float4 w[4];
@@ -462,7 +462,7 @@
     w[k] = k < Cin ? *reinterpret_cast<const float4*>(Wt + static_cast<long>(k) * ldw + c0) : make_float4(0, 0, 0, 0);
 #pragma unroll
   for (int j = 0; j < 4; ++j) b4[j] = (bias && c0 + j < Cout) ? bias[c0 + j] : 0.0f;
-  const long r0 = static_cast<long>(blockIdx.x) * (rpp * kThinIters) + rl;
+  const long r0 = static_cast<long>(bx) * (rpp * kThinIters) + rl;
   float4 xr[kThinIters];
 #pragma unroll
   for (int it = 0; it < kThinIters; ++it) {
@@ -489,6 +489,44 @@
       *reinterpret_cast<float4*>(Y + row * ldy + c0) = make_float4(acc[0], acc[1], acc[2], acc[3]);
     }
   }
+}
+
+__global__ __launch_bounds__(256) void fused_layer_thin_kernel(const float* __restrict__ X, int ldx, int shift,
+                                                               int Cin, const float* __restrict__ Wt, int ldw,
+                                                               const float* __restrict__ bias, int Cout,
+                                                               float* __restrict__ Y, int ldy, long P, int qshift) {
+  fused_layer_thin_body(blockIdx.x, blockIdx.y, X, ldx, shift, Cin, Wt, ldw, bias, Cout, Y, ldy, P, qshift);
+}
+
+struct ThinJob {
+  const float* X;
+  const float* Wt;
+  const float* bias;
+  float* Y;
+  long P;
+  int ldx, shift, Cin, ldw, Cout, ldy, qshift, gx;
+};
+struct ThinMulti {
+  pdr::JobPrefix pre;
+  ThinJob job[PDR_MAX_JOBS];
+};
+
+__global__ __launch_bounds__(256) void fused_layer_thin_multi_kernel(const ThinMulti a) {
+  const int j = pdr::find_job(a.pre, blockIdx.x);
+  const ThinJob& J = a.job[j];
+  const int local = static_cast<int>(blockIdx.x - a.pre.first[j]);
+  const int by = local / J.gx, bx = local - by * J.gx;
+  fused_layer_thin_body(bx, by, J.X, J.ldx, J.shift, J.Cin, J.Wt, J.ldw, J.bias, J.Cout, J.Y, J.ldy, J.P, J.qshift);
+}
+
+inline void thin_grid(long P, int Cout, unsigned* gx, unsigned* gy, int* qshift_out) {
+  const int c4n = (Cout + 3) / 4;
+  int qshift = 3;
+  while (qshift < 6 && (1 << qshift) < c4n) ++qshift;
+  const int ql = 1 << qshift, rows_per_block = (256 >> qshift) * 8;
+  *gx = static_cast<unsigned>((P + rows_per_block - 1) / rows_per_block);
+  *gy = static_cast<unsigned>((c4n + ql - 1) / ql);
+  *qshift_out = qshift;
 }
 
 using pdr::LayerSource;
@@ -693,12 +731,10 @@
   };
   switch (pl.family) {
     case Family::Thin: {
-      const int c4n = (Cout + 3) / 4;
-      int qshift = 3;
-      while (qshift < 6 && (1 << qshift) < c4n) ++qshift;
-      const int ql = 1 << qshift, rows_per_block = (256 >> qshift) * 8;
-      const dim3 tgrid(static_cast<unsigned>((P + rows_per_block - 1) / rows_per_block),
-                       static_cast<unsigned>((c4n + ql - 1) / ql));
+      unsigned gx, gy;
+      int qshift;
+      thin_grid(P, Cout, &gx, &gy, &qshift);
+      const dim3 tgrid(gx, gy);
       hipLaunchKernelGGL(fused_layer_thin_kernel, tgrid, dim3(256), 0, s, in->seg[0].ptr, in->seg[0].ld,
                          __builtin_ctz(in->seg[0].row_div), Cin, Wt, ldw, bias, Cout, Y, ldy, P, qshift);
       break;
@@ -720,6 +756,34 @@
       pdr::with_tile(pl.id, [&](auto t) { launch_form<decltype(t)>(uniform_grid(pl.ntiles, pl.ncol), a, pl); });
       break;
   }
+  return pdr::check_launch();
+}
+
+extern "C" int pdr_thin_multi(const pdr_thin_job_t* jobs, int njobs, pdr_stream_t stream) {
+  if (!jobs || njobs < 1 || njobs > PDR_MAX_JOBS) return PDR_EINVAL;
+  ThinMulti a;
+  long wgs[PDR_MAX_JOBS];
+  for (int j = 0; j < njobs; ++j) {
+    const pdr_thin_job_t& q = jobs[j];
+    if (!q.X || !q.Wt || !q.Y || q.rows <= 0 || q.Cin <= 0 || q.Cout <= 0) return PDR_EINVAL;
+    pdr_layer_in_t li = {};
+    li.n_seg = 1;
+    li.seg[0].ptr = q.X, li.seg[0].C = q.Cin, li.seg[0].ld = q.ldx, li.seg[0].row_div = q.row_div;
+    li.rows_per_batch = static_cast<int>(q.rows < (1L << 30) ? q.rows : 0);
+    LayerPlan pl;
+    const int rc = plan_layer(&li, q.rows, q.Cin, q.Wt, q.ldw, q.Cout, q.Y, q.ldy, false, &pl);
+    if (rc != PDR_OK || pl.family != Family::Thin) return PDR_EINVAL;
+    ThinJob& J = a.job[j];
+    unsigned gx, gy;
+    thin_grid(q.rows, q.Cout, &gx, &gy, &J.qshift);
+    J.X = q.X, J.Wt = q.Wt, J.bias = q.bias, J.Y = q.Y, J.P = q.rows;
+    J.ldx = q.ldx, J.shift = __builtin_ctz(q.row_div), J.Cin = q.Cin, J.ldw = q.ldw, J.Cout = q.Cout, J.ldy = q.ldy;
+    J.gx = static_cast<int>(gx);
+    wgs[j] = static_cast<long>(gx) * gy;
+  }
+  for (int j = njobs; j < PDR_MAX_JOBS; ++j) a.job[j] = a.job[0];
+  if (!pdr::fill_prefix(&a.pre, wgs, njobs)) return PDR_EINVAL;
+  hipLaunchKernelGGL(fused_layer_thin_multi_kernel, dim3(a.pre.first[njobs]), dim3(256), 0, pdr::as_stream(stream), a);
   return pdr::check_launch();
 }
 
diff --git a/point_diffusion_refinement_amd/csrc/neighbors.hip b/point_diffusion_refinement_amd/csrc/neighbors.hip
--- a/point_diffusion_refinement_amd/csrc/neighbors.hip
+++ b/point_diffusion_refinement_amd/csrc/neighbors.hip
@@ -15,22 +15,16 @@
 }
 
 template <int K, int MODEL, typename IdxT, bool KNN_PAD, bool RAGGED = false>
-__global__ __launch_bounds__(256) void nn_search_kernel(const float* __restrict__ queries,
-                                                        const float* __restrict__ cloud, int nq,
-                                                        int nc, int Kout,
-                                                        float* __restrict__ dists,
-                                                        IdxT* __restrict__ idx,
-                                                        float* __restrict__ nn,
-                                                        float* __restrict__ wgt = nullptr,
-                                                        const int64_t* __restrict__ len_q = nullptr,
-                                                        const int64_t* __restrict__ len_c = nullptr) {
+__device__ __forceinline__ void nn_search_body(float4* tile, int bx, int b, const float* __restrict__ queries,
+                                               const float* __restrict__ cloud, int nq, int nc, int Kout,
+                                               float* __restrict__ dists, IdxT* __restrict__ idx,
+                                               float* __restrict__ nn, float* __restrict__ wgt,
+                                               const int64_t* __restrict__ len_q, const int64_t* __restrict__ len_c) {
   static_assert(KNN_PAD || !RAGGED, "the ragged search pads with (0, -1)");
-  __shared__ float4 tile[kTile];
-  const int b = blockIdx.y;
-  const int j = blockIdx.x * 256 + threadIdx.x;
+  const int j = bx * 256 + threadIdx.x;
   const bool active = j < nq;
   const int nqe = RAGGED ? cloud_len(len_q, b, nq) : nq;
-  const int nce = !RAGGED ? nc : (static_cast<int>(blockIdx.x) * 256 < nqe ? cloud_len(len_c, b, nc) : 0);
+  const int nce = !RAGGED ? nc : (bx * 256 < nqe ? cloud_len(len_c, b, nc) : 0);
   const bool searching = RAGGED ? j < nqe : active;
   const float* q = queries + (static_cast<size_t>(b) * nq + (active ? j : 0)) * 3;
   const float* c = cloud + static_cast<size_t>(b) * nc * 3;
@@ -104,18 +98,38 @@
   }
 }
 
+template <int K, int MODEL, typename IdxT, bool KNN_PAD, bool RAGGED = false>
+__global__ __launch_bounds__(256) void nn_search_kernel(const float* __restrict__ queries,
+                                                        const float* __restrict__ cloud, int nq,
+                                                        int nc, int Kout,
+                                                        float* __restrict__ dists,
+                                                        IdxT* __restrict__ idx,
+                                                        float* __restrict__ nn,
+                                                        float* __restrict__ wgt = nullptr,
+                                                        const int64_t* __restrict__ len_q = nullptr,
+                                                        const int64_t* __restrict__ len_c = nullptr) {
+  __shared__ float4 tile[kTile];
+  nn_search_body<K, MODEL, IdxT, KNN_PAD, RAGGED>(tile, blockIdx.x, blockIdx.y, queries, cloud, nq, nc, Kout, dists, idx,
+                                                  nn, wgt, len_q, len_c);
+}
+
+struct KnnWaveLds {
+  unsigned long long cand[4][64];
+  float outd[4][8];
+  int outi[4][8];
+  float outr[4][8];
+};
+
 template <int NCH, typename IdxT, bool RAGGED = false>
-__global__ __launch_bounds__(256) void knn_wave_kernel(const float* __restrict__ queries,
-                                                       const float* __restrict__ cloud, int nq, int nc, int K,
-                                                       int qpw, float* __restrict__ dists, IdxT* __restrict__ idx,
-                                                       float* __restrict__ nn, float* __restrict__ wgt,
-                                                       const int64_t* __restrict__ len_q = nullptr,
-                                                       const int64_t* __restrict__ len_c = nullptr) {
-  __shared__ unsigned long long cand[4][64];
-  __shared__ float outd[4][8];
-  __shared__ int outi[4][8];
-  __shared__ float outr[4][8];
-  const int b = blockIdx.y;
+__device__ __forceinline__ void knn_wave_body(KnnWaveLds& lds, int bx, int b, const float* __restrict__ queries,
+                                              const float* __restrict__ cloud, int nq, int nc, int K, int qpw,
+                                              float* __restrict__ dists, IdxT* __restrict__ idx,
+                                              float* __restrict__ nn, float* __restrict__ wgt,
+                                              const int64_t* __restrict__ len_q, const int64_t* __restrict__ len_c) {
+  auto& cand = lds.cand;
+  auto& outd = lds.outd;
+  auto& outi = lds.outi;
+  auto& outr = lds.outr;
   const int lane = threadIdx.x & 63;
   const int wave = __builtin_amdgcn_readfirstlane(threadIdx.x >> 6);
   const float* c = cloud + static_cast<size_t>(b) * nc * 3;
@@ -137,7 +151,7 @@
     py[ch] = ok ? py[ch] : __builtin_inff();
     pz[ch] = ok ? pz[ch] : __builtin_inff();
   }
-  const int j0 = (blockIdx.x * 4 + wave) * qpw;
+  const int j0 = (bx * 4 + wave) * qpw;
   __builtin_amdgcn_s_waitcnt(0x0F70);
   const int jf = min(j0, nq - 1);
   float nqx = q[jf * 3 + 0], nqy = q[jf * 3 + 1], nqz = q[jf * 3 + 2];
@@ -260,6 +274,71 @@
       }
     }
     __builtin_amdgcn_wave_barrier();
+  }
+}
+
+template <int NCH, typename IdxT, bool RAGGED = false>
+__global__ __launch_bounds__(256) void knn_wave_kernel(const float* __restrict__ queries,
+                                                       const float* __restrict__ cloud, int nq, int nc, int K,
+                                                       int qpw, float* __restrict__ dists, IdxT* __restrict__ idx,
+                                                       float* __restrict__ nn, float* __restrict__ wgt,
+                                                       const int64_t* __restrict__ len_q = nullptr,
+                                                       const int64_t* __restrict__ len_c = nullptr) {
+  __shared__ KnnWaveLds lds;
+  knn_wave_body<NCH, IdxT, RAGGED>(lds, blockIdx.x, blockIdx.y, queries, cloud, nq, nc, K, qpw, dists, idx, nn, wgt,
+                                   len_q, len_c);
+}
+
+struct KnnJob {
+  const float* x;
+  const float* y;
+  float* dists;
+  int* idx;
+  float* wgt;
+  int n1, n2, K, gx, kind, nch;
+};
+struct KnnMulti {
+  pdr::JobPrefix pre;
+  KnnJob job[PDR_MAX_JOBS];
+  int qpw;
+};
+
+__global__ __launch_bounds__(256) void knn_group_multi_kernel(const KnnMulti a) {
+  __shared__ float4 tile[kTile];
+  static_assert(sizeof(KnnWaveLds) <= sizeof(float4) * kTile, "the wave body's LDS fits the search tile");
+  const int j = pdr::find_job(a.pre, blockIdx.x);
+  const KnnJob& J = a.job[j];
+  const int local = static_cast<int>(blockIdx.x - a.pre.first[j]);
+  const int b = local / J.gx, bx = local - b * J.gx;
+  if (J.kind == 0) {
+    KnnWaveLds& lds = *reinterpret_cast<KnnWaveLds*>(tile);
+#define PDR_KWM(NCH)                                                                                                  \
+  case NCH:                                                                                                           \
+    knn_wave_body<NCH, int>(lds, bx, b, J.x, J.y, J.n1, J.n2, J.K, a.qpw, J.dists, J.idx, nullptr, J.wgt, nullptr,    \
+                            nullptr);                                                                                 \
+    break
+    switch (J.nch) {
+      PDR_KWM(1);
+      PDR_KWM(2);
+      PDR_KWM(4);
+      PDR_KWM(8);
+      default:
+      PDR_KWM(16);
+    }
+#undef PDR_KWM
+  } else {
+#define PDR_KGM(KK)                                                                                                   \
+  case KK:                                                                                                            \
+    nn_search_body<KK, kAcc3, int, false>(tile, bx, b, J.x, J.y, J.n1, J.n2, J.K, J.dists, J.idx, nullptr, J.wgt,     \
+                                          nullptr, nullptr);                                                          \
+    break
+    switch (J.kind) {
+      PDR_KGM(4);
+      PDR_KGM(8);
+      default:
+      PDR_KGM(16);
+    }
+#undef PDR_KGM
   }
 }
 
@@ -493,6 +572,53 @@
   else if (K <= 8) PDR_KG(8);
   else PDR_KG(16);
 #undef PDR_KG
+  return pdr::check_launch();
+}
+
+extern "C" int pdr_knn_group_multi(const pdr_knn_job_t* jobs, int njobs, int B, pdr_stream_t stream) {
+  if (!jobs || njobs < 1 || njobs > PDR_MAX_JOBS || B < 0) return PDR_EINVAL;
+  for (int j = 0; j < njobs; ++j) {
+    const pdr_knn_job_t& q = jobs[j];
+    if (q.n1 <= 0 || q.n2 <= 0 || q.K <= 0 || q.K > q.n2 || q.K > 16) return PDR_EINVAL;
+    if (!q.x || !q.y || !q.dists || !q.idx || !q.weights) return PDR_EINVAL;
+    if (static_cast<long>(B) * q.n1 * q.K >= (1L << 31)) return PDR_EINVAL;
+  }
+  if (B == 0) return PDR_OK;
+  KnnMulti a;
+  const bool wave_on = pdr::option(pdr::OPT_KNN_WAVE) != 0;
+  auto wave = [&](const pdr_knn_job_t& q) { return wave_on && q.K <= 8 && q.n2 >= 64 && q.n2 <= 1024; };
+  long fixed = 0;
+  for (int j = 0; j < njobs; ++j)
+    if (!wave(jobs[j])) fixed += static_cast<long>(B) * ((jobs[j].n1 + 255) / 256);
+  int qpw = 32;
+  long tot;
+  do {
+    qpw >>= 1;
+    tot = fixed;
+    for (int j = 0; j < njobs; ++j)
+      if (wave(jobs[j])) tot += static_cast<long>(B) * ((jobs[j].n1 + 4 * qpw - 1) / (4 * qpw));
+  } while (qpw > 1 && tot < 1024);
+  a.qpw = qpw;
+  long wgs[PDR_MAX_JOBS];
+  for (int j = 0; j < njobs; ++j) {
+    const pdr_knn_job_t& q = jobs[j];
+    KnnJob& J = a.job[j];
+    J.x = q.x, J.y = q.y, J.dists = q.dists, J.idx = q.idx, J.wgt = q.weights;
+    J.n1 = q.n1, J.n2 = q.n2, J.K = q.K;
+    if (wave(q)) {
+      J.kind = 0;
+      J.nch = q.n2 <= 64 ? 1 : q.n2 <= 128 ? 2 : q.n2 <= 256 ? 4 : q.n2 <= 512 ? 8 : 16;
+      J.gx = (q.n1 + 4 * qpw - 1) / (4 * qpw);
+    } else {
+      J.kind = q.K <= 4 ? 4 : q.K <= 8 ? 8 : 16;
+      J.nch = 0;
+      J.gx = (q.n1 + 255) / 256;
+    }
+    wgs[j] = static_cast<long>(B) * J.gx;
+  }
+  for (int j = njobs; j < PDR_MAX_JOBS; ++j) a.job[j] = a.job[0];
+  if (!pdr::fill_prefix(&a.pre, wgs, njobs)) return PDR_EINVAL;
+  hipLaunchKernelGGL(knn_group_multi_kernel, dim3(a.pre.first[njobs]), dim3(256), 0, pdr::as_stream(stream), a);
   return pdr::check_launch();
 }
 
diff --git a/point_diffusion_refinement_amd/csrc/pdr_common.h b/point_diffusion_refinement_amd/csrc/pdr_common.h
--- a/point_diffusion_refinement_amd/csrc/pdr_common.h
+++ b/point_diffusion_refinement_amd/csrc/pdr_common.h
@@ -31,6 +31,25 @@
   OPT_WS_XCD_ORDER, OPT_DEEP_CHUNKS, OPT_DEEP_KS, OPT_DEEP_JOBS32, OPT_DEEP_JOBS64, OPT_COUNT
 };
 int option(Opt o);
+
+struct JobPrefix {
+  unsigned first[PDR_MAX_JOBS + 1];
+};
+__device__ __forceinline__ int find_job(const JobPrefix& p, unsigned bid) {
+  int j = 0;
+#pragma unroll
+  for (int i = 1; i < PDR_MAX_JOBS; ++i) j += bid >= p.first[i] ? 1 : 0;
+  return __builtin_amdgcn_readfirstlane(j);
+}
+inline bool fill_prefix(JobPrefix* p, const long* wgs, int njobs) {
+  long tot = 0;
+  for (int j = 0; j <= PDR_MAX_JOBS; ++j) {
+    p->first[j] = static_cast<unsigned>(tot);
+    if (j < njobs) tot += wgs[j];
+    if (tot >= (1L << 31)) return false;
+  }
+  return true;
+}
 
 struct PoolArgs {
   const float* values;
diff --git a/point_diffusion_refinement_amd/pointnet2/fused_network.py b/point_diffusion_refinement_amd/pointnet2/fused_network.py
--- a/point_diffusion_refinement_amd/pointnet2/fused_network.py
+++ b/point_diffusion_refinement_amd/pointnet2/fused_network.py
@@ -218,10 +218,11 @@
 
 class SortedQueries:
 
-    def __init__(self, idx, counts, new_xyz):
+    def __init__(self, idx, counts, new_xyz, jobs=None):
         B, m, K = idx.shape
         dev = idx.device
         lib = _lib.load()
+        self.xyz4 = None
         self.perm = torch.empty((B, m), dtype=torch.int32, device=dev)
         self.inv = torch.empty((B, m), dtype=torch.int32, device=dev)
         self.perm_rows = torch.empty((B, m), dtype=torch.int32, device=dev)
@@ -230,17 +231,29 @@
             new_xyz = new_xyz.contiguous()
             self.idx = torch.empty_like(idx)
             self.counts = torch.empty_like(counts)
-            self.xyz = torch.empty_like(new_xyz)
+            if jobs is not None:
+                self.xyz4 = torch.empty((B, m, 4), dtype=torch.float32, device=dev)
+                self.xyz = self.xyz4[:, :, :3]
+            else:
+                self.xyz = torch.empty_like(new_xyz)
             nvalid = torch.empty((2, B), dtype=torch.int32, device=dev)
 
             def prepared(dd):
+                dd.nvalid = nvalid
+                if jobs is not None:
+                    job = _lib.PrepareJob(
+                        idx.data_ptr(), counts.data_ptr(), new_xyz.data_ptr(), m, K, self.perm.data_ptr(),
+                        self.inv.data_ptr(), self.perm_rows.data_ptr(), self.idx.data_ptr(), self.counts.data_ptr(),
+                        self.xyz4.data_ptr(), 4, 0, dd.idx0.data_ptr(), dd.row_w.data_ptr(), dd.tile_valid.data_ptr(),
+                        dd.tile_list.data_ptr(), dd.n_tiles.data_ptr(), nvalid.data_ptr())
+                    jobs.append((job, self, (idx, counts, new_xyz)))
+                    return
                 _lib.check(lib.pdr_dedup_prepare(
                     idx.data_ptr(), counts.data_ptr(), new_xyz.data_ptr(), B, m, K, self.perm.data_ptr(),
                     self.inv.data_ptr(), self.perm_rows.data_ptr(), self.idx.data_ptr(), self.counts.data_ptr(),
                     self.xyz.data_ptr(), dd.idx0.data_ptr(), dd.row_w.data_ptr(), dd.tile_valid.data_ptr(),
                     dd.tile_list.data_ptr(), dd.n_tiles.data_ptr(), nvalid.data_ptr(), _probe_ptr(), _stream()),
                     "dedup_prepare")
-                dd.nvalid = nvalid
             self.plan = Dedup(self.idx, self.counts, B, m, K, prepared=prepared)
             return
         _lib.check(lib.pdr_dedup_sort(counts.data_ptr(), B, m, self.perm.data_ptr(), self.inv.data_ptr(),
@@ -399,6 +412,79 @@
     return hit.padded
 
 
+def _xyz4_feed(entries):
+    if not entries:
+        return
+    cur = torch.cuda.current_stream(entries[0][0].device)
+    ev = torch.cuda.Event()
+    ev.record(cur)
+    for t, padded in entries:
+        _XYZ4[(t.data_ptr(), tuple(t.shape))] = Padded(t, padded, cur.cuda_stream, ev)
+
+
+def _batched(kind):
+    return GEOMETRY_BATCHED and kind in GEOMETRY_BATCHED_KINDS
+
+
+def _launch_jobs(fn, jobs, what, *args):
+    for i in range(0, len(jobs), _lib.MAX_JOBS):
+        part = jobs[i:i + _lib.MAX_JOBS]
+        _lib.check(fn(_lib.job_array(part), len(part), *args, _stream()), what)
+
+
+def xyz4_many(ts):
+    entries = []
+    for t in ts:
+        if t.shape[-1] % 4 == 0 or (t.data_ptr(), tuple(t.shape)) in _XYZ4 or \
+                any(t is e[0] for e in entries):
+            continue
+        if not (_batched("pad") and t.is_cuda and t.dtype == torch.float32 and t.is_contiguous()):
+            xyz4(t)
+            continue
+        entries.append((t, torch.empty(t.shape[:-1] + (_pad4(t.shape[-1]),), dtype=torch.float32, device=t.device)))
+    if entries:
+        jobs = [_lib.PadJob(t.data_ptr(), t.numel() // t.shape[-1], t.shape[-1], p.data_ptr(), p.shape[-1])
+                for t, p in entries]
+        _launch_jobs(_lib.load().pdr_pad_rows_multi, jobs, "pad_rows_multi")
+        _xyz4_feed(entries)
+
+
+def launch_plan_jobs(jobs, B):
+    if not jobs:
+        return
+    _launch_jobs(_lib.load().pdr_dedup_prepare_multi, [j[0] for j in jobs], "dedup_prepare_multi", B, _probe_ptr())
+    _xyz4_feed([(sq.xyz, sq.xyz4) for _, sq, _ in jobs if sq is not None])
+
+
+def query_tables_many(reqs):
+    lib = _lib.load()
+    out, jobs = [], []
+    for split, query_xyz, has_v0 in reqs:
+        if not _batched("thin"):
+            out.append(split.query_tables(query_xyz, has_v0))
+            continue
+        B, m, _ = query_xyz.shape
+        conv = split.VV0 if has_v0 else split.V
+        ld = _ldy(split.U.Cout)
+        X = xyz4(query_xyz).reshape(B * m, 4)
+        q_in = plain(X, B, m, C=3)
+        V2 = torch.empty((B * m, 2 * ld if has_v0 else ld), dtype=torch.float32, device=query_xyz.device)
+        out.append(V2)
+        plan = (ctypes.c_int * 8)()
+        li = q_in.struct()
+        rc = lib.pdr_fused_layer_plan(ctypes.byref(li), q_in.P, conv.Cin, conv.Wt.data_ptr(), conv.ldw, conv.Cout,
+                                      V2.data_ptr(), V2.shape[1], plan)
+        if rc != 0 or not plan[6]:
+            run_layer(q_in, conv, out=(V2, 0))
+            continue
+        jobs.append(_lib.ThinJob(X.data_ptr(), 4, 1, B * m, conv.Cin, conv.Wt.data_ptr(), conv.ldw,
+                                 conv.bias.data_ptr(), conv.Cout, V2.data_ptr(), V2.shape[1]))
+        _WALK[V2.data_ptr()] = li.walk_reverse
+    if jobs:
+        _launch_jobs(lib.pdr_thin_multi, jobs, "thin_multi")
+    return out
+
+
 def plain(t2d, B, rows_per_batch, row_div=1, C=None):
     rows, ld = t2d.shape
     C = ld if C is None else C
@@ -431,6 +517,8 @@
 
 SIDE_TABLES = True
 FPS_STREAM = True
+GEOMETRY_BATCHED = False
+GEOMETRY_BATCHED_KINDS = frozenset(("ball", "plan", "pad", "thin", "knn"))
 _PAR = {"stream": None}
 
 
@@ -1271,15 +1359,21 @@
         e = _geom(idx)
         return e.sorted if (e is not None and _dedup_on() and self.dedup) else None
 
-    def plan_ahead(self, neigh, new_xyz):
+    def plan_ahead(self, neigh, new_xyz, jobs=None):
         idx, counts = neigh
         B, m, K = idx.shape
         e = _geom(idx, create=True)
         if self._eligible(idx, m, K):
             if e.sorted is None:
-                e.sorted = SortedQueries(idx, counts, new_xyz)
+                e.sorted = SortedQueries(idx, counts, new_xyz, jobs)
         elif _PROBE[0] is not None and self._shape_ok(idx, m, K) and not e.probed:
-            _lib.check(_lib.load().pdr_dedup_probe(counts.data_ptr(), B, m, K, _probe_ptr(), _stream()), "dedup_probe")
+            if jobs is not None:
+                job = _lib.PrepareJob()
+                job.counts, job.m, job.K, job.probe_only = counts.data_ptr(), m, K, 1
+                jobs.append((job, None, (counts,)))
+            else:
+                _lib.check(_lib.load().pdr_dedup_probe(counts.data_ptr(), B, m, K, _probe_ptr(), _stream()),
+                           "dedup_probe")
             e.probed = True
         return neigh
 
@@ -1842,19 +1936,92 @@
                 mark("side:knn_done")
                 return event(side)
 
-        for k in range(nlev):
-            group_level(k)
-            lv = k + 1
-            transfer_level(lv, (self.enc_map[lv],) if lv < nlev else (self.dec_map[lv],))
-            if lv < nlev and hoist_enc:
-                hoist_map(self.enc_map[lv], enc_cl, lv)
-        if side_tables_on:
+        def batch_levels(ks, tail):
+            if not fps_on:
+                for k in ks:
+                    sample_level(k)
             with torch.cuda.stream(side):
-                for l in range(1, nlev):
-                    blk = self.dec_map[l]
-                    if blk.split is not None and id(blk) not in tables:
-                        tables[id(blk)] = blk.side_tables(fm_neigh[fm_key(l, blk)], l_xyz[l], True)
-        ev_knn = geometry_tail()
+                if fps_on and ks:
+                    side.wait_event(ev_fps[ks[-1]])
+                specs, owners, seen = [], [], set()
+                for k in ks:
+                    specs.append((l_xyz[k + 1], l_xyz[k], self.sa[k].radius, self.sa[k].nsample))
+                    owners.append((self.sa[k], k, None))
+                    lv = k + 1
+                    for blk in ([self.enc_map[lv]] if lv < nlev else []) + [self.dec_map[lv]]:
+                        key = fm_key(lv, blk)
+                        if key not in fm_neigh and key not in seen:
+                            seen.add(key)
+                            specs.append((l_xyz[lv], l_uvw[lv], blk.radius, blk.nsample))
+                            owners.append((blk, lv, key))
+                neighs = _ext.ball_query_multi(specs) if _batched("ball") else [_ext.ball_query(*sp) for sp in specs]
+                jobs = [] if _batched("plan") else None
+                for (blk, l, key), neigh in zip(owners, neighs):
+                    if key is None:
+                        sa_neigh[l] = blk.plan_ahead(neigh, l_xyz[l + 1], jobs)
+                    else:
+                        fm_neigh[key] = blk.plan_ahead(neigh, l_xyz[l], jobs)
+                launch_plan_jobs(jobs, B)
+                xyz4_many([l_xyz[k + 1] for k in ks])
+                reqs, sinks = [], []
+
+                def want(blk, neigh, new_xyz, has_v0):
+                    if side_tables_on and blk.split is not None and id(blk) not in tables and \
+                            all(id(blk) != bid for bid, _ in sinks):
+                        sq = blk._sorted(neigh[0]) if neigh is not None else None
+                        reqs.append((blk.split, sq.xyz if sq is not None else new_xyz, has_v0))
+                        sinks.append((id(blk), sq))
+                for k in ks:
+                    want(self.sa[k], sa_neigh[k], l_xyz[k + 1], False)
+                for k in ks:
+                    lv = k + 1
+                    blk = self.enc_map[lv] if lv < nlev else self.dec_map[lv]
+                    want(blk, fm_neigh[fm_key(lv, blk)], l_xyz[lv], True)
+                if tail:
+                    for l in list(range(1, nlev)) + [0]:
+                        want(self.dec_map[l], fm_neigh[fm_key(l, self.dec_map[l])], l_xyz[l], True)
+                    for i in range(-1, -(len(self.fp) + 1), -1):
+                        want(self.fp[i], None, l_xyz[i - 1], False)
+                for (bid, sq), V2 in zip(sinks, query_tables_many(reqs)):
+                    tables[bid] = QueryTables(V2, sq)
+                ev = event(side)
+                for k in ks:
+                    ev_sa[k] = ev_fm[k + 1] = ev
+
+        def knn_batch():
+            with torch.cuda.stream(side):
+                order = list(range(-1, -(len(self.fp) + 1), -1))
+                specs = [(l_xyz[i - 1], l_xyz[i], self.fp[i].K) for i in order]
+                found = _ext.knn_group_multi(specs) if _batched("knn") else [_ext.knn_group(*sp) for sp in specs]
+                knn.update(zip(order, found))
+                mark("side:knn_done")
+                return event(side)
+
+        if GEOMETRY_BATCHED:
+            groups = [g for g in ([[0], list(range(1, nlev))] if fps_on else [[k] for k in range(nlev)]) if g]
+            for ks in groups:
+                batch_levels(ks, tail=ks is groups[-1])
+                if ks is groups[-1]:
+                    with torch.cuda.stream(side):
+                        mark("side:encoder_geometry_done")
+                for k in ks:
+                    if k + 1 < nlev and hoist_enc:
+                        hoist_map(self.enc_map[k + 1], enc_cl, k + 1)
+            ev_knn = knn_batch()
+        else:
+            for k in range(nlev):
+                group_level(k)
+                lv = k + 1
+                transfer_level(lv, (self.enc_map[lv],) if lv < nlev else (self.dec_map[lv],))
+                if lv < nlev and hoist_enc:
+                    hoist_map(self.enc_map[lv], enc_cl, lv)
+            if side_tables_on:
+                with torch.cuda.stream(side):
+                    for l in range(1, nlev):
+                        blk = self.dec_map[l]
+                        if blk.split is not None and id(blk) not in tables:
+                            tables[id(blk)] = blk.side_tables(fm_neigh[fm_key(l, blk)], l_xyz[l], True)
+            ev_knn = geometry_tail()
         if hoist:
             for l in range(nlev, 0 if hoist0_main else -1, -1):
                 hoist_map(self.dec_map[l], dec_cl, l)
diff --git a/point_diffusion_refinement_amd/pointnet2_ops/_ext.py b/point_diffusion_refinement_amd/pointnet2_ops/_ext.py
--- a/point_diffusion_refinement_amd/pointnet2_ops/_ext.py
+++ b/point_diffusion_refinement_amd/pointnet2_ops/_ext.py
@@ -87,6 +87,35 @@
                                               int(nsample), idx.data_ptr(), counts.data_ptr(), _stream()),
                    "ball_query")
     return idx, counts
+
+
+def ball_query_multi(specs):
+    out, jobs = [None] * len(specs), []
+    for k, (new_xyz, xyz, radius, nsample) in enumerate(specs):
+        if xyz.shape[1] > 1024 or new_xyz.shape[0] != specs[0][0].shape[0]:
+            out[k] = ball_query(new_xyz, xyz, radius, nsample)
+            continue
+        _req(new_xyz, "new_xyz", torch.float32)
+        _req(xyz, "xyz", torch.float32)
+        _req_xyz(new_xyz, "new_xyz")
+        _req_xyz(xyz, "xyz")
+        _same_device(new_xyz, xyz)
+        if new_xyz.shape[0] != xyz.shape[0]:
+            raise RuntimeError("new_xyz and xyz must have the same batch size")
+        B, m, _ = new_xyz.shape
+        idx = torch.empty((B, m, nsample), dtype=torch.int32, device=xyz.device)
+        counts = torch.empty((B, m), dtype=torch.int32, device=xyz.device)
+        out[k] = (idx, counts)
+        jobs.append(_lib.BallJob(new_xyz.data_ptr(), xyz.data_ptr(), xyz.shape[1], m, float(radius), int(nsample),
+                                 idx.data_ptr(), counts.data_ptr()))
+    if jobs:
+        B, dev = specs[0][0].shape[0], specs[0][0].device
+        with torch.cuda.device(dev):
+            for i in range(0, len(jobs), _lib.MAX_JOBS):
+                part = jobs[i:i + _lib.MAX_JOBS]
+                _lib.check(_lib.load().pdr_ball_query_multi(_lib.job_array(part), len(part), B, _stream()),
+                           "ball_query_multi")
+    return out
 
 
 def group_points(points, idx):
@@ -239,6 +268,36 @@
     return d, i, w
 
 
+def knn_group_multi(specs):
+    out, jobs = [None] * len(specs), []
+    for k, (x, y, K) in enumerate(specs):
+        K = int(K)
+        if K > min(y.shape[1], 16) or x.shape[0] != specs[0][0].shape[0]:
+            out[k] = knn_group(x, y, K)
+            continue
+        _req(x, "x", torch.float32)
+        _req(y, "y", torch.float32)
+        _same_device(x, y)
+        if x.dim() != 3 or y.dim() != 3 or x.shape[2] != 3 or y.shape[2] != 3 or x.shape[0] != y.shape[0]:
+            raise RuntimeError("knn_group: x (B,n1,3) and y (B,n2,3) with equal batch size required, got %s and %s"
+                               % (tuple(x.shape), tuple(y.shape)))
+        B, n1, _ = x.shape
+        d = torch.empty((B, n1, K), dtype=torch.float32, device=x.device)
+        w = torch.empty((B, n1, K), dtype=torch.float32, device=x.device)
+        i = torch.empty((B, n1, K), dtype=torch.int32, device=x.device)
+        out[k] = (d, i, w)
+        jobs.append(_lib.KnnJob(x.data_ptr(), y.data_ptr(), n1, y.shape[1], K, d.data_ptr(), i.data_ptr(),
+                                w.data_ptr()))
+    if jobs:
+        B, dev = specs[0][0].shape[0], specs[0][0].device
+        with torch.cuda.device(dev):
+            for i0 in range(0, len(jobs), _lib.MAX_JOBS):
+                part = jobs[i0:i0 + _lib.MAX_JOBS]
+                _lib.check(_lib.load().pdr_knn_group_multi(_lib.job_array(part), len(part), B, _stream()),
+                           "knn_group_multi")
+    return out
+
+
 class _KnnDists(torch.autograd.Function):
 
     @staticmethod
```

New measurement: 5949 cloud-steps/s. 0.989x the previous value.
